# sangminwoo/SVOL

Measured on AMD Instinct MI355X. Metric: frames/sec (fwd+matcher+bwd), T=32·P=196·d=256, higher is better.
Workload: dtype bf16

## Files before the change

include/svol_hip.h:

```cpp
#ifndef SVOL_HIP_H
#define SVOL_HIP_H

#include <stdint.h>

#ifdef __cplusplus
extern "C" {
#endif

#define SVOL_F32 0
#define SVOL_BF16 1
#define SVOL_F16 2

#define SVOL_OK 0
#define SVOL_E_INVALID (-1)
#define SVOL_E_UNSUPPORTED (-2)
#define SVOL_E_LAUNCH (-3)

#define SVOL_ACT_NONE 0
#define SVOL_ACT_RELU 1
#define SVOL_ACT_GELU 2
#define SVOL_ACT_SIGMOID 3
#define SVOL_ACT_GELU_D 5
#define SVOL_ACT_RELU_RES 4

// ... 24 lines not shown
                   float weight_decay, int64_t step, float grad_scale, void* stream);
int svol_adam_flat_zero(float* p, float* g, float* m, float* v, int64_t n, float lr, float beta1, float beta2, float eps,
                        float weight_decay, int64_t step, float grad_scale, void* stream);
int svol_adam_flat_scaled(float* p, const float* g, float* m, float* v, int64_t n, float lr, float beta1, float beta2, float eps,
                          float weight_decay, float grad_mul, const float* scaler_state, void* stream);
int64_t svol_grad_sqnorm_ws_bytes(int64_t n);
int svol_grad_sqnorm(const float* g, int64_t n, float* ws, float* out, void* stream);
int svol_grad_clip_state(const float* sq, int32_t nb, float grad_mul, float max_norm, float loss_scale, int64_t steps_taken,
                         float* scaler_state, float* state_out, void* stream);
int svol_sgd_flat_grouped(float* p, float* g, float* buf, int64_t n, const int32_t* seg_end, const int32_t* seg_group, int32_t nseg,
                          const float* hyper, int32_t ngroups, const float* state, float grad_mul, int zero, void* stream);
int svol_adam_flat_grouped(float* p, float* g, float* m, float* v, int64_t n, const int32_t* seg_end, const int32_t* seg_group,
                           int32_t nseg, const float* hyper, int32_t ngroups, const float* state, const float* step_count,
                           float grad_mul, int zero, void* stream);
int svol_adamw_flat_grouped(float* p, float* g, float* m, float* v, int64_t n, const int32_t* seg_end, const int32_t* seg_group,
                            int32_t nseg, const float* hyper, int32_t ngroups, const float* state, const float* step_count,
                            float grad_mul, int zero, void* stream);
int svol_flat_step_advance(float* step_count, const float* state, void* stream);

int svol_gemm_nt(const void* A, int64_t lda, const void* A2, int64_t n_split, const void* B, int64_t ldb,
                 void* C, int64_t ldc, const float* bias, const float* colscale, int act, void* pre_act_out,
                 int64_t ldp, const void* residual, int64_t ldr, int out_f32, int64_t M, int64_t N, int64_t K,
                 int dtype, void* stream);
int svol_gemm_nt_split(const void* A, int64_t lda, const void* W_hilo, int64_t ldw, void* C, int64_t ldc, const float* bias,
                       int64_t M, int64_t N, int64_t K, void* stream);
int svol_gemm_nt_dgelu(const void* A, int64_t lda, const void* B, int64_t ldb, void* C, int64_t ldc,
                       const void* pre, int64_t ldp, float* colsum, int64_t M, int64_t N, int64_t K, int dtype,
                       void* stream);
int svol_gemm_nt_dact(const void* A, int64_t lda, const void* B, int64_t ldb, void* C, int64_t ldc,
                      const void* aux, int64_t ldaux, int act, float* colsum, int64_t M, int64_t N, int64_t K,
                      int dtype, void* stream);

int svol_gemm_tn(const void* A, int64_t lda, const void* B, int64_t ldb, float* C, int64_t ldc, float* colsum,
                 int64_t Mc, int64_t N, int64_t K, int dtype, void* stream);
#define SVOL_TN_GROUP_MAX 6
typedef struct svol_tn_problem {
    const void* A; int64_t lda;
    const void* B; int64_t ldb;
    float* C; int64_t ldc;
    float* colsum;
    int64_t Mc, N, K;
} svol_tn_problem;
int svol_gemm_tn_grouped(const svol_tn_problem* problems, int32_t n, int dtype, void* stream);
int svol_colsum(const void* X, int64_t ldx, float* out, int64_t M, int64_t N, int dtype, void* stream);
int svol_act_bwd(const void* dy, const void* aux, void* dpre, int act, int64_t n, int dtype, void* stream);

int svol_layernorm_fwd(const void* x, int x_f32, const float* gamma, const float* beta, float* y32, void* y,
                       void* ypos, const void* pos, int64_t pos_rows, float* mean, float* rstd, int64_t M, int64_t D,
                       float dropout_p, uint64_t seed, const int64_t* seed_offset_dev, int dtype, void* stream);
int svol_layernorm_bwd(const float* dy32, const void* dy, const void* dy2, const void* x, int x_f32,
                       const float* gamma, const float* mean, const float* rstd, float* dx32, void* dx,
                       float* dgamma, float* dbeta, float* dx_colsum, int64_t M, int64_t D, float dropout_p,
                       uint64_t seed, const int64_t* seed_offset_dev, int dtype, void* stream);

int svol_dropout(const void* x, void* y, int64_t n, int64_t row_len, float p, uint64_t seed, int dtype, void* stream);
int svol_dropout_add(const float* t32, const float* res32, float* out32, int64_t n, int64_t row_len, float p, uint64_t seed, void* stream);

int svol_posenc_sine(const float* mask, void* pos, int64_t B, int64_t L, int64_t D, int dtype, void* stream);

int64_t svol_attn_ws_bytes(int64_t B, int64_t H, int64_t Lq, int64_t Lk, int64_t dh);
int svol_attn_fwd(const void* q, int64_t ldq, const void* k, int64_t ldk, const void* v, int64_t ldv, void* o,
                  int64_t ldo, float* lse2, const float* kbias, int64_t B, int64_t H, int64_t Lq, int64_t Lk,
                  int64_t dh, float scale, float q_premul, void* ws, int64_t ws_bytes, int dtype, void* stream);
int svol_attn_bwd(const void* q, int64_t ldq, const void* k, int64_t ldk, const void* v, int64_t ldv, const void* o,
                  int64_t ldo, const void* d_o, int64_t lddo, const float* lse2, float* delta, const float* kbias,
                  void* dq, int64_t lddq, void* dk, int64_t lddk, void* dv, int64_t lddv, int64_t B, int64_t H,
                  int64_t Lq, int64_t Lk, int64_t dh, float scale, float q_premul, void* ws, int64_t ws_bytes,
                  int dtype, void* stream);

#define SVOL_ATTN_DQ_PREZEROED 1
int64_t svol_attn_bwd_sp_image_bytes(int64_t B, int64_t H, int64_t Lq, int64_t Lk, int64_t dh, int64_t ws_bytes, int dtype);
int svol_attn_bwd_zero_ws(void* ws, int64_t ws_bytes, int64_t B, int64_t H, int64_t Lq, int64_t Lk, int64_t dh, int dtype, void* stream);
int svol_attn_bwd_ex(const void* q, int64_t ldq, const void* k, int64_t ldk, const void* v, int64_t ldv, const void* o,
                     int64_t ldo, const void* d_o, int64_t lddo, const float* lse2, float* delta, const float* kbias,
                     void* dq, int64_t lddq, void* dk, int64_t lddk, void* dv, int64_t lddv, int64_t B, int64_t H,
                     int64_t Lq, int64_t Lk, int64_t dh, float scale, float q_premul, void* ws, int64_t ws_bytes,
                     int dtype, int flags, void* ev_prep, void* stream);

int svol_attn_fwd_dropout(const void* q, int64_t ldq, const void* k, int64_t ldk, const void* v, int64_t ldv, void* o,
                          int64_t ldo, float* lse2, const float* kbias, int64_t B, int64_t H, int64_t Lq, int64_t Lk,
                          int64_t dh, float scale, float q_premul, void* ws, int64_t ws_bytes, float dropout_p, uint64_t seed,
                          int dtype, void* stream);
int svol_attn_bwd_dropout(const void* q, int64_t ldq, const void* k, int64_t ldk, const void* v, int64_t ldv, const void* o,
                          int64_t ldo, const void* d_o, int64_t lddo, const float* lse2, float* delta, const float* kbias,
                          void* dq, int64_t lddq, void* dk, int64_t lddk, void* dv, int64_t lddv, int64_t B, int64_t H,
                          int64_t Lq, int64_t Lk, int64_t dh, float scale, float q_premul, void* ws, int64_t ws_bytes,
                          float dropout_p, uint64_t seed, int dtype, void* stream);

int svol_gate_fwd(const float* x32, const void* pos, const float* u, const float* gamma, const float* beta,
                  float* y32, void* y, void* ypos, float* a, float* mean, float* rstd, float* ws, int64_t B,
                  int64_t L, int64_t D, int64_t H, int dtype, void* stream);
int svol_gate_bwd(const float* dy32, const void* dy, const void* dy2, const float* x32, const void* pos,
                  const float* u, const float* gamma, const float* a, const float* mean, const float* rstd,
                  const float* ws, float* ws2, float* dx32, float* du, float* dgamma, float* dbeta, int64_t B,
                  int64_t L, int64_t D, int64_t H, int dtype, void* stream);

int svol_layernorm_gate_scores_fwd(const float* x32, const float* gamma, const float* beta, float* y32, void* y, void* ypos,
                                   const void* pos, float* mean, float* rstd, const float* u_next, float* scores_next,
                                   int64_t B, int64_t L, int64_t D, int64_t H, int dtype, void* stream);
int svol_gate_fwd_scored(const float* x32, const void* pos, const float* u, const float* gamma, const float* beta,
                         float* y32, void* y, void* ypos, float* a, float* mean, float* rstd, float* ws, int64_t B,
                         int64_t L, int64_t D, int64_t H, int dtype, void* stream);

int svol_gate_vectors_fwd(const float* skch, const float* W_in, const float* b_in, float* q_out, float* u_out, int64_t B, int64_t D,
                          int64_t H, void* stream);
int svol_gate_vectors_bwd(const float* du, const float* skch, const float* W_in, const float* q, float* dq_ws, float* dskch,
                          float* dW_in, float* db_in, int64_t B, int64_t D, int64_t H, void* stream);
#define SVOL_GATE_VEC_MAX_LAYERS 8
int svol_gate_vectors_fwd_multi(const float* skch, const float* const* W_in, const float* const* b_in, float* const* q_out,
                                float* const* u_out, int64_t n_layers, int64_t B, int64_t D, int64_t H, void* stream);
int svol_gate_vectors_bwd_multi(const float* const* du, const float* skch, const float* const* W_in, const float* const* q,
                                float* const* dq_ws, float* const* dskch, float* const* dW_in, float* const* db_in, int64_t n_layers,
                                int64_t B, int64_t D, int64_t H, void* stream);

int svol_match_cost(const float* logits, const float* boxes, const float* tgt_boxes, const int32_t* pred_off,
                    const int32_t* pred_cnt, const int32_t* tgt_off, const int32_t* tgt_cnt,
                    const int64_t* cost_off, float* cost, int32_t n_problems, float w_bbox, float w_giou,
                    float w_class, int32_t* box_status, void* stream);
int svol_lsap_batched(const float* cost, const int64_t* cost_off, const int32_t* pred_off, const int32_t* pred_cnt,
                      const int32_t* tgt_off, const int32_t* tgt_cnt, int32_t* match, int32_t* status,
                      int32_t n_problems, int32_t max_dim, void* stream);
int svol_heads_fwd(const float* hs, const float* Wc, const float* bc, const float* W0, const float* b0, const float* W1, const float* b1,
                   const float* W2, const float* b2, float* logits, float* h1, float* h2, float* boxes, int64_t R, int64_t D, void* stream);
int svol_heads_bwd(const float* dlogits, const float* dboxes, const float* hs, const float* h1, const float* h2, const float* boxes,
                   const float* Wc, const float* W0, const float* W1, const float* W2, float* dhs, float* gp0, float* gp1, float* dWc,
                   float* dbc, float* dW2, float* db2, int64_t R, int64_t D, void* stream);
int svol_set_loss_bwd(const float* g_label, const float* g_bbox, const float* g_giou, const float* dl, float* dlogits, float* dboxes,
                      int64_t n_layers, int64_t rows_per_layer, void* stream);
int svol_weighted_total(const float* x, const float* w, int64_t n, float* out, void* stream);
int svol_weighted_total_bwd(const float* w, const float* dout, int64_t n, float* dx, void* stream);
int svol_lsap_solve(const double* cost, int64_t nr, int64_t nc, int64_t* rows, int64_t* cols);
int svol_set_loss(const float* logits, const float* boxes, const float* tgt_boxes, const int32_t* match,
                  float* losses, float* g_label, float* g_bbox, float* g_giou, int32_t n_layers,
                  int32_t rows_per_layer, float eos_coef, const int32_t* rebase_vid_off, int32_t rows_per_video,
                  const int32_t* status, const int32_t* box_status, int32_t problems_per_layer, void* stream);

int svol_postprocess(const float* logits, const float* boxes, float* out, int64_t B, int64_t N, int64_t chunk, void* stream);
int svol_eval_max_iou(const double* pred_box, const int32_t* pred_off, const double* gt_box, const int32_t* gt_off,
                      const int32_t* gt_rec, double* out, int64_t n_gt, int32_t k, void* stream);
int svol_eval_ap(const double* pred_box, const double* pred_score, const int32_t* pred_frame, const int32_t* grp_pred_off,
                 const double* gt_box, const int32_t* gt_frame, const int32_t* grp_gt_off, const double* thresholds,
                 int32_t n_thresholds, int32_t* ws_order, unsigned char* ws_u8, double* ws_f64, double* ap, int64_t n_pred,
                 int64_t n_gt, int64_t n_groups, void* stream);

int svol_ingest_resize(const uint8_t* src, int64_t n, int64_t H, int64_t W, int64_t s_n, int64_t s_h, int64_t s_w,
                       const int32_t* xtab, int64_t kx, const int32_t* ytab, int64_t ky, const float* lut, const uint8_t* flip,
                       void* out, int64_t o_n, int64_t o_c, int64_t o_h, int64_t o_w, int64_t OH, int64_t OW, int out_dtype,
                       void* stream);
// ... 9 lines not shown
                   int64_t N, int64_t H, int64_t W, int64_t C, int64_t Cout, int64_t kh, int64_t kw, int64_t stride,
                   int64_t pad, int dtype, void* stream);
int svol_maxpool_nhwc(const void* x, void* y, int64_t N, int64_t H, int64_t W, int64_t C, int64_t k, int64_t stride,
                      int64_t pad, int dtype, void* stream);
int svol_avgpool_nhwc(const void* x, float* y, int64_t N, int64_t HW, int64_t C, int dtype, void* stream);
int svol_bn_colstats(const void* z, const float* shift, float shift_scale, float* sum, float* sumsq, int64_t M, int64_t C, int dtype,
                     void* stream);
int svol_bn_finalize(const float* sum, const float* sumsq_centered, const float* pivot, const float* gamma, const float* beta,
                     float* running_mean, float* running_var, float momentum, float eps, int64_t M, int64_t C, float* mean, float* rstd,
                     float* scale, float* shift, void* stream);
int svol_conv_weight_pack(const float* w, void* out, int64_t Cout, int64_t Cin, int64_t kh, int64_t kw, int64_t Kp, int flip, int dtype,
                          void* stream);
int svol_conv_weight_unpack_add(const float* dwp, float* grad, int64_t Cout, int64_t Cin, int64_t kh, int64_t kw, int64_t Kp, void* stream);
int svol_conv_wgrad_nhwc(const void* dz, const void* x, float* dwp, int64_t N, int64_t H, int64_t W, int64_t C, int64_t Cout, int64_t kh, int64_t kw,
                         int64_t stride, int64_t pad, int64_t Kp, int dtype, void* stream);
int svol_bn_apply(const void* z, const float* scale, const float* shift, const void* residual, int relu, void* y, int64_t M, int64_t C,
                  int dtype, void* stream);
int svol_bn_bwd_reduce(const void* dy, const void* y, const void* z, const float* mean, const float* rstd, float* sum_g, float* sum_gx,
                       int64_t M, int64_t C, int dtype, void* stream);
int svol_bn_bwd_apply(const void* dy, const void* y, const void* z, const float* mean, const float* rstd, const float* gamma,
                      const float* sum_g, const float* sum_gx, void* dz, void* dres, int64_t M, int64_t C, int dtype, void* stream);
int svol_col2im_nhwc(const void* dcols, int64_t ldcols, void* dx, int64_t N, int64_t H, int64_t W, int64_t C, int64_t kh, int64_t kw,
                     int64_t stride, int64_t pad, int dtype, void* stream);
int svol_maxpool_idx_nhwc(const void* x, void* y, uint8_t* idx, int64_t N, int64_t H, int64_t W, int64_t C, int64_t k, int64_t stride,
                          int64_t pad, int dtype, void* stream);
int svol_maxpool_bwd_nhwc(const void* dy, const uint8_t* idx, void* dx, int64_t N, int64_t H, int64_t W, int64_t C, int64_t k,
                          int64_t stride, int64_t pad, int dtype, void* stream);
int svol_attn_weights_mean(const void* q, int64_t ldq, const void* k, int64_t ldk, const float* lse2, const float* kbias,
                           float* att, int64_t B, int64_t H, int64_t Lq, int64_t Lk, int64_t dh, float scale,
                           float q_premul, int dtype, void* stream);
int svol_attn_small_fwd(const void* q, int64_t ldq, const void* k, int64_t ldk, const void* v, int64_t ldv, void* o, int64_t ldo,
                        int64_t n_seq, int64_t H, int64_t L, int64_t dh, float scale, int dtype, void* stream);
int svol_attn_small_fwd_lse(const void* q, int64_t ldq, const void* k, int64_t ldk, const void* v, int64_t ldv, void* o, int64_t ldo,
                            float* lse2, int64_t n_seq, int64_t H, int64_t L, int64_t dh, float scale, int dtype, void* stream);
int svol_attn_small_bwd(const void* q, int64_t ldq, const void* k, int64_t ldk, const void* v, int64_t ldv, const void* o, int64_t ldo,
                        const void* dout, int64_t lddo, const float* lse2, void* dq, int64_t lddq, void* dk, int64_t lddk, void* dv,
                        int64_t lddv, int64_t n_seq, int64_t H, int64_t L, int64_t dh, float scale, int dtype, void* stream);


#define SVOL_DIM_B 0
#define SVOL_DIM_L 1
#define SVOL_DIM_N 2
#define SVOL_DIM_D 3
#define SVOL_DIM_H 4
#define SVOL_DIM_F 5
#define SVOL_DIM_DTYPE 6
#define SVOL_DIM_QDTYPE 7
#define SVOL_DIM_ATTN_WS_BYTES 8
#define SVOL_DIM_COUNT 9

#define SVOL_BLK_VIDEO_HALF 0
#define SVOL_BLK_QUERY_SELF 1
#define SVOL_BLK_QUERY_CROSS 2
const char* svol_block_slot_names(int block);
int svol_block_trace_dump(char* buf, int64_t cap);
int svol_clock_probe(uint64_t* samples, int32_t* count, int32_t max_samples, const int32_t* stop, int64_t period_us,
                     int64_t max_ms, int32_t* wall_khz, void* stream);


#define SVOL_VH_SLOTS(X) \
    X(X32) X(POS) X(U) X(G1) X(BT1) X(G2) X(BT2) X(G3) X(BT3) X(B_IN) X(B_O) X(B_FC1) X(B_FC2) X(QSCALE) \
    X(W_IN) X(WV_HILO) X(W_O) X(W_FC1) X(W_FC2) X(W_IN_T) X(W_O_T) X(W_FC1_T) X(W_FC2_T) \
    X(Y1) X(Y1POS) X(A) X(MEAN1) X(RSTD1) X(GATE_WS) X(GATE_PRE) X(U_NEXT) X(GATE_WS_NEXT) \
    X(QKV) X(O) X(LSE) X(S2) X(Y2) X(MEAN2) X(RSTD2) X(PRE) X(HID) X(S3) \
    X(MEAN3) X(RSTD3) X(M32) X(M) X(MPOS) X(Y1_32) X(Y2_32) X(ATTN_WS) \
    X(DM32) X(DM) X(DMPOS) X(DS32_3) X(DS3) X(DPRE) X(DY2) X(DS32_2) X(G2D) X(DO) X(DQKV) X(DELTA) X(DXQP) X(DXQ) X(GATE_WS2) \
    X(DX32) X(DU) \
    X(DG1) X(DBT1) X(DG2) X(DBT2) X(DG3) X(DBT3) X(DW_IN) X(DB_IN) X(DW_O) X(DB_O) X(DW_FC1) X(DB_FC1) X(DW_FC2) X(DB_FC2) \
    X(EV_A0) X(EV_A1) X(EV_CLEAN_IN) X(EV_PREP) X(ATTN_WS_NEXT) X(ZERO_STREAM) X(EV_CLEAN_OUT)
#define SVOL_QS_SLOTS(X) \
    X(O32) X(O) X(OPOS) X(QPOS) X(B_IN) X(B_O) X(G4) X(BT4) X(QSCALE) X(W_IN) X(WV_HILO) X(W_O) X(W_IN_T) X(W_O_T) \
    X(QKV) X(OA) X(LSE) X(S4) X(MEAN4) X(RSTD4) X(Y32) X(Y) X(YPOS) X(ATTN_WS) \
    X(DY32) X(DY) X(DYPOS) X(G) X(DOA) X(DQKV) X(DELTA) X(DO32) X(DXQ) X(DXQP) X(DQPOS) \
    X(DW_IN) X(DB_IN) X(DW_O) X(DB_O) X(DG4) X(DBT4)
#define SVOL_QC_SLOTS(X) \
    X(O32) X(O) X(OPOS) X(MV) X(MPOS) X(KBIAS) X(QPOS) X(B_IN) X(B_O) X(G5) X(BT5) X(B_FC1) X(B_FC2) X(G6) X(BT6) X(QSCALE) \
    X(W_INQ) X(W_INQ_T) X(W_KV) X(W_KV_T) X(WV_HILO) X(W_O) X(W_O_T) X(W_FC1) X(W_FC1_T) X(W_FC2) X(W_FC2_T) \
    X(Q) X(QC) X(KV) X(OA) X(OAQ) X(LSE) X(S5) X(Y5_32) X(Y5) X(MEAN5) X(RSTD5) X(PRE) X(HID) X(S6) X(MEAN6) X(RSTD6) \
    X(Y32) X(Y) X(YPOS) X(ATTN_WS) \
    X(DY32) X(DY) X(DYPOS) X(DS32_6) X(DS6) X(DPRE) X(DY5) X(DS32_5) X(G5D) X(DOAQ) X(DOA) X(DQC) X(DQ) X(DKV) X(DELTA) \
    X(DO32) X(DXQP) X(DMPOS) X(DMV) X(DQPOS) \
    X(DW_IN) X(DB_IN) X(DW_O) X(DB_O) X(DG5) X(DBT5) X(DW_FC1) X(DB_FC1) X(DW_FC2) X(DB_FC2) X(DG6) X(DBT6)
#define SVOL_SLOT_ENUM_VH(n) SVOL_VH_##n,
#define SVOL_SLOT_ENUM_QS(n) SVOL_QS_##n,
#define SVOL_SLOT_ENUM_QC(n) SVOL_QC_##n,
enum { SVOL_VH_SLOTS(SVOL_SLOT_ENUM_VH) SVOL_VH_COUNT };
enum { SVOL_QS_SLOTS(SVOL_SLOT_ENUM_QS) SVOL_QS_COUNT };
enum { SVOL_QC_SLOTS(SVOL_SLOT_ENUM_QC) SVOL_QC_COUNT };

int svol_video_half_fwd(const int64_t* dims, void* const* slots, void* stream);
int svol_video_half_bwd(const int64_t* dims, void* const* slots, int phase, void* stream);
int svol_video_half_wgrad(const int64_t* dims, void* const* slots, void* stream);
int svol_video_half_wgrad_part(const int64_t* dims, void* const* slots, int part, void* stream);
int svol_query_self_fwd(const int64_t* dims, void* const* slots, void* stream);
int svol_query_self_bwd(const int64_t* dims, void* const* slots, void* stream);
int svol_query_self_wgrad(const int64_t* dims, void* const* slots, void* stream);
int svol_query_cross_fwd(const int64_t* dims, void* const* slots, void* stream);
int svol_query_cross_bwd(const int64_t* dims, void* const* slots, void* stream);
int svol_query_cross_wgrad(const int64_t* dims, void* const* slots, void* stream);

#ifdef __cplusplus
}
#endif
#endif
```

svol_amd/_lib.py:

```python
from __future__ import annotations

import ctypes
import os

_HERE = os.path.dirname(os.path.abspath(__file__))
LIB_PATH = os.path.join(_HERE, 'libsvol_hip.so')

_p = ctypes.c_void_p
_i64 = ctypes.c_int64
_i32 = ctypes.c_int32
_int = ctypes.c_int
_f32 = ctypes.c_float
_u64 = ctypes.c_uint64

SIGNATURES = {
    'svol_block_trace_dump': [ctypes.c_char_p, _i64],
    'svol_lsap_solve': [_p, _i64, _i64, _p, _p],
    'svol_heads_fwd': [_p] * 13 + [_i64, _i64, _p],
    'svol_heads_bwd': [_p] * 17 + [_i64, _i64, _p],
    'svol_set_loss_bwd': [_p] * 6 + [_i64, _i64, _p],
    'svol_weighted_total': [_p, _p, _i64, _p, _p],
    'svol_weighted_total_bwd': [_p, _p, _i64, _p, _p],
    'svol_cast': [_p, _int, _p, _int, _i64, _p],
    'svol_cast_transpose': [_p, _p, _p, _int, _i64, _i64, _p],
    'svol_cast_split': [_p, _i64, _p, _i64, _i64, _p],
    'svol_gemm_nt_split': [_p, _i64, _p, _i64, _p, _i64, _p, _i64, _i64, _i64, _p],
    'svol_gemm_nt': [_p, _i64, _p, _i64, _p, _i64, _p, _i64, _p, _p, _int, _p, _i64, _p, _i64, _int, _i64, _i64, _i64,
                     _int, _p],
    'svol_gemm_nt_dgelu': [_p, _i64, _p, _i64, _p, _i64, _p, _i64, _p, _i64, _i64, _i64, _int, _p],
    'svol_gemm_nt_dact': [_p, _i64, _p, _i64, _p, _i64, _p, _i64, _int, _p, _i64, _i64, _i64, _int, _p],
    'svol_gemm_tn': [_p, _i64, _p, _i64, _p, _i64, _p, _i64, _i64, _i64, _int, _p],
    'svol_gemm_tn_grouped': [_p, _i32, _int, _p],
    'svol_colsum': [_p, _i64, _p, _i64, _i64, _int, _p],
    'svol_act_bwd': [_p, _p, _p, _int, _i64, _int, _p],
    'svol_layernorm_fwd': [_p, _int, _p, _p, _p, _p, _p, _p, _i64, _p, _p, _i64, _i64, _f32, _u64, _p, _int, _p],
    'svol_layernorm_bwd': [_p, _p, _p, _p, _int, _p, _p, _p, _p, _p, _p, _p, _p, _i64, _i64, _f32, _u64, _p, _int, _p],
    'svol_cast_transpose_multi': [_p, _int, _i64, _int, _p],
    'svol_postprocess': [_p, _p, _p, _i64, _i64, _i64, _p],
    'svol_eval_max_iou': [_p, _p, _p, _p, _p, _p, _i64, _int, _p],
    'svol_eval_ap': [_p, _p, _p, _p, _p, _p, _p, _p, _int, _p, _p, _p, _p, _i64, _i64, _i64, _p],
    'svol_patchify': [_p, _p, _i64, _i64, _i64, _i64, _i64, _int, _p],
    'svol_vit_embed': [_p, _p, _p, _p, _p, _i64, _i64, _i64, _int, _p],
    'svol_ingest_resize': [_p, _i64, _i64, _i64, _i64, _i64, _i64, _p, _i64, _p, _i64, _p, _p, _p, _i64, _i64, _i64, _i64, _i64, _i64, _int, _p],
    'svol_adamw_flat': [_p, _p, _p, _p, _i64, _f32, _f32, _f32, _f32, _f32, _i64, _f32, _p],
    'svol_adamw_flat_zero': [_p, _p, _p, _p, _i64, _f32, _f32, _f32, _f32, _f32, _i64, _f32, _p],
    'svol_grad_finite': [_p, _i64, _p, _p],
    'svol_adamw_flat_scaled': [_p, _p, _p, _p, _i64, _f32, _f32, _f32, _f32, _f32, _f32, _p, _p],
    'svol_loss_scaler_update': [_p, _f32, _f32, _i64, _f32, _f32, _p],
    'svol_sgd_flat': [_p, _p, _p, _i64, _f32, _f32, _f32, _f32, _p],
    'svol_sgd_flat_zero': [_p, _p, _p, _i64, _f32, _f32, _f32, _f32, _p],
    'svol_sgd_flat_scaled': [_p, _p, _p, _i64, _f32, _f32, _f32, _f32, _p, _p],
    'svol_adam_flat': [_p, _p, _p, _p, _i64, _f32, _f32, _f32, _f32, _f32, _i64, _f32, _p],
    'svol_adam_flat_zero': [_p, _p, _p, _p, _i64, _f32, _f32, _f32, _f32, _f32, _i64, _f32, _p],
    'svol_adam_flat_scaled': [_p, _p, _p, _p, _i64, _f32, _f32, _f32, _f32, _f32, _f32, _p, _p],
    'svol_grad_sqnorm_ws_bytes': [_i64],
    'svol_grad_sqnorm': [_p, _i64, _p, _p, _p],
    'svol_grad_clip_state': [_p, _i32, _f32, _f32, _f32, _i64, _p, _p, _p],
    'svol_sgd_flat_grouped': [_p, _p, _p, _i64, _p, _p, _i32, _p, _i32, _p, _f32, _int, _p],
    'svol_adam_flat_grouped': [_p, _p, _p, _p, _i64, _p, _p, _i32, _p, _i32, _p, _p, _f32, _int, _p],
    'svol_adamw_flat_grouped': [_p, _p, _p, _p, _i64, _p, _p, _i32, _p, _i32, _p, _p, _f32, _int, _p],
    'svol_flat_step_advance': [_p, _p, _p],
    'svol_conv_nhwc': [_p, _p, _i64, _p, _p, _int, _p, _i64, _i64, _i64, _i64, _i64, _i64, _i64, _i64, _i64, _int, _p],
    'svol_im2col': [_p, _i64, _i64, _i64, _i64, _int, _p, _i64, _i64, _i64, _i64, _i64, _i64, _i64, _i64, _i64, _int, _p],
    'svol_maxpool_nhwc': [_p, _p, _i64, _i64, _i64, _i64, _i64, _i64, _i64, _int, _p],
    'svol_avgpool_nhwc': [_p, _p, _i64, _i64, _i64, _int, _p],
    'svol_bn_colstats': [_p, _p, _f32, _p, _p, _i64, _i64, _int, _p],
    'svol_bn_finalize': [_p, _p, _p, _p, _p, _p, _p, _f32, _f32, _i64, _i64, _p, _p, _p, _p, _p],
    'svol_conv_weight_pack': [_p, _p, _i64, _i64, _i64, _i64, _i64, _int, _int, _p],
    'svol_conv_weight_unpack_add': [_p, _p, _i64, _i64, _i64, _i64, _i64, _p],
    'svol_conv_wgrad_nhwc': [_p, _p, _p, _i64, _i64, _i64, _i64, _i64, _i64, _i64, _i64, _i64, _i64, _int, _p],
    'svol_bn_apply': [_p, _p, _p, _p, _int, _p, _i64, _i64, _int, _p],
    'svol_bn_bwd_reduce': [_p, _p, _p, _p, _p, _p, _p, _i64, _i64, _int, _p],
    'svol_bn_bwd_apply': [_p, _p, _p, _p, _p, _p, _p, _p, _p, _p, _i64, _i64, _int, _p],
    'svol_col2im_nhwc': [_p, _i64, _p, _i64, _i64, _i64, _i64, _i64, _i64, _i64, _i64, _int, _p],
    'svol_maxpool_idx_nhwc': [_p, _p, _p, _i64, _i64, _i64, _i64, _i64, _i64, _i64, _int, _p],
    'svol_maxpool_bwd_nhwc': [_p, _p, _p, _i64, _i64, _i64, _i64, _i64, _i64, _i64, _int, _p],
    'svol_attn_weights_mean': [_p, _i64, _p, _i64, _p, _p, _p, _i64, _i64, _i64, _i64, _i64, _f32, _f32, _int, _p],
    'svol_attn_small_fwd': [_p, _i64, _p, _i64, _p, _i64, _p, _i64, _i64, _i64, _i64, _i64, _f32, _int, _p],
    'svol_attn_small_fwd_lse': [_p, _i64, _p, _i64, _p, _i64, _p, _i64, _p, _i64, _i64, _i64, _i64, _f32, _int, _p],
    'svol_attn_small_bwd': [_p, _i64, _p, _i64, _p, _i64, _p, _i64, _p, _i64, _p, _p, _i64, _p, _i64, _p, _i64, _i64, _i64, _i64,
                            _i64, _f32, _int, _p],
    'svol_posenc_sine': [_p, _p, _i64, _i64, _i64, _int, _p],
    'svol_attn_ws_bytes': [_i64, _i64, _i64, _i64, _i64],
    'svol_attn_fwd': [_p, _i64, _p, _i64, _p, _i64, _p, _i64, _p, _p, _i64, _i64, _i64, _i64, _i64, _f32, _f32, _p, _i64,
                      _int, _p],
    'svol_attn_bwd': [_p, _i64, _p, _i64, _p, _i64, _p, _i64, _p, _i64, _p, _p, _p, _p, _i64, _p, _i64, _p, _i64,
                      _i64, _i64, _i64, _i64, _i64, _f32, _f32, _p, _i64, _int, _p],
    'svol_attn_bwd_ex': [_p, _i64, _p, _i64, _p, _i64, _p, _i64, _p, _i64, _p, _p, _p, _p, _i64, _p, _i64, _p, _i64,
                         _i64, _i64, _i64, _i64, _i64, _f32, _f32, _p, _i64, _int, _int, _p, _p],
    'svol_attn_bwd_sp_image_bytes': [_i64, _i64, _i64, _i64, _i64, _i64, _int],
    'svol_attn_bwd_zero_ws': [_p, _i64, _i64, _i64, _i64, _i64, _i64, _int, _p],
    'svol_attn_fwd_dropout': [_p, _i64, _p, _i64, _p, _i64, _p, _i64, _p, _p, _i64, _i64, _i64, _i64, _i64, _f32, _f32, _p, _i64,
                              _f32, _u64, _int, _p],
    'svol_attn_bwd_dropout': [_p, _i64, _p, _i64, _p, _i64, _p, _i64, _p, _i64, _p, _p, _p, _p, _i64, _p, _i64, _p, _i64,
                              _i64, _i64, _i64, _i64, _i64, _f32, _f32, _p, _i64, _f32, _u64, _int, _p],
    'svol_dropout': [_p, _p, _i64, _i64, _f32, _u64, _int, _p],
    'svol_dropout_add': [_p, _p, _p, _i64, _i64, _f32, _u64, _p],
    'svol_gate_fwd': [_p, _p, _p, _p, _p, _p, _p, _p, _p, _p, _p, _p, _i64, _i64, _i64, _i64, _int, _p],
    'svol_gate_bwd': [_p, _p, _p, _p, _p, _p, _p, _p, _p, _p, _p, _p, _p, _p, _p, _p, _i64, _i64, _i64, _i64, _int,
                      _p],
    'svol_clock_probe': [_p, _p, _int, _p, _i64, _i64, _p, _p],
    'svol_gate_fwd_scored': [_p, _p, _p, _p, _p, _p, _p, _p, _p, _p, _p, _p, _i64, _i64, _i64, _i64, _int, _p],
    'svol_layernorm_gate_scores_fwd': [_p, _p, _p, _p, _p, _p, _p, _p, _p, _p, _p, _i64, _i64, _i64, _i64, _int, _p],
    'svol_gate_vectors_fwd': [_p, _p, _p, _p, _p, _i64, _i64, _i64, _p],
    'svol_gate_vectors_bwd': [_p, _p, _p, _p, _p, _p, _p, _p, _i64, _i64, _i64, _p],
    'svol_gate_vectors_fwd_multi': [_p, _p, _p, _p, _p, _i64, _i64, _i64, _i64, _p],
    'svol_gate_vectors_bwd_multi': [_p, _p, _p, _p, _p, _p, _p, _p, _i64, _i64, _i64, _i64, _p],
    'svol_match_cost': [_p, _p, _p, _p, _p, _p, _p, _p, _p, _i32, _f32, _f32, _f32, _p, _p],
    'svol_lsap_batched': [_p, _p, _p, _p, _p, _p, _p, _p, _i32, _i32, _p],
    'svol_set_loss': [_p, _p, _p, _p, _p, _p, _p, _p, _i32, _i32, _f32, _p, _i32, _p, _p, _i32, _p],
    'svol_video_half_fwd': [_p, _p, _p],
    'svol_video_half_bwd': [_p, _p, _int, _p],
    'svol_video_half_wgrad': [_p, _p, _p],
    'svol_video_half_wgrad_part': [_p, _p, _int, _p],
    'svol_query_self_fwd': [_p, _p, _p],
    'svol_query_self_bwd': [_p, _p, _p],
    'svol_query_self_wgrad': [_p, _p, _p],
    'svol_query_cross_fwd': [_p, _p, _p],
    'svol_query_cross_bwd': [_p, _p, _p],
    'svol_query_cross_wgrad': [_p, _p, _p],
}



class TnProblem(ctypes.Structure):
    _fields_ = [('A', _p), ('lda', _i64), ('B', _p), ('ldb', _i64), ('C', _p), ('ldc', _i64), ('colsum', _p),
                ('Mc', _i64), ('N', _i64), ('K', _i64)]


_LIB = None


class SvolHipError(RuntimeError):
    pass


def lib():
    global _LIB
    if _LIB is None:
        if not os.path.exists(LIB_PATH):
            raise SvolHipError(
                f'{LIB_PATH} not found: the SVOL hot path has no CPU fallback. '
                'Build it with `python -m svol_amd.build` (hipcc, gfx950).')
        L = ctypes.CDLL(LIB_PATH)
        L.svol_abi_version.restype = _int
        L.svol_abi_version.argtypes = []
        L.svol_strerror.restype = ctypes.c_char_p
        L.svol_strerror.argtypes = [_int]
        for name, at in SIGNATURES.items():
            f = getattr(L, name)
            f.restype = _int
            f.argtypes = at
        L.svol_attn_ws_bytes.restype = _i64
        L.svol_attn_bwd_sp_image_bytes.restype = _i64
        L.svol_grad_sqnorm_ws_bytes.restype = _i64
        L.svol_block_slot_names.restype = ctypes.c_char_p
        L.svol_block_slot_names.argtypes = [_int]
        _LIB = L
    return _LIB


def check(rc: int, name: str):
    if rc != 0:
        msg = lib().svol_strerror(rc).decode()
        raise SvolHipError(f'{name} failed: {msg} (code {rc})')
```

svol_amd/blocks.py:

```python
from __future__ import annotations

import ctypes
import math
import os
import weakref

import torch

from . import _lib, ops

WGRAD_SPLIT = os.environ.get('SVOL_WGRAD_SPLIT') is not None
ENABLED = os.environ.get('SVOL_NO_BLOCKS') is None
GATE_SCORES_FUSE = os.environ.get('SVOL_GATE_SCORES_FUSE') is not None
VH, QS, QC = 0, 1, 2
_F32, _BF16 = 0, 1
_ESZ = {torch.float32: 4, torch.bfloat16: 2, torch.float16: 2}
_SLOTS = {}


def _slots(block):
    m = _SLOTS.get(block)
    if m is None:
        names = _lib.lib().svol_block_slot_names(block).decode().rstrip(',').split(',')
        m = _SLOTS[block] = {n: i for i, n in enumerate(names)}
    return m


class _Table:

    __slots__ = ('arr', 'idx', 'n')

    def __init__(self, block, template=None):
        self.idx = _slots(block)
        self.n = len(self.idx)
        self.arr = (ctypes.c_void_p * self.n)()
        if template is not None:
            ctypes.memmove(self.arr, template.arr, self.n * 8)

    def set(self, name, ptr):
        self.arr[self.idx[name]] = ptr

    def set_t(self, name, t):
        self.arr[self.idx[name]] = t.data_ptr() if t is not None else None


def _align(n, a=256):
    return (n + a - 1) // a * a


class _Layout:

    def __init__(self, items):
        self.off = {}
        n = 0
        for name, nbytes in items:
            self.off[name] = (n, nbytes)
            n += _align(nbytes)
        self.total = max(n, 256)

    def fill(self, tbl, base):
        for name, (o, _) in self.off.items():
            tbl.arr[tbl.idx[name]] = base + o

    def view(self, arena, name, dtype, shape):
        o, nb = self.off[name]
        return arena[o:o + nb].view(dtype).view(shape)


_LAYOUTS = {}


def _layout(key, make):
    lay = _LAYOUTS.get(key)
    if lay is None:
        lay = _LAYOUTS[key] = _Layout(make())
    return lay


_SCRATCH = {}


def _scratch(dev, nbytes):
    key = (dev, ops._stream())
    t = _SCRATCH.get(key)
    if t is None or t.numel() < nbytes:
        t = _SCRATCH[key] = torch.empty((_align(nbytes, 1 << 20),), dtype=torch.uint8, device=dev)
    return t


def _dims(B, L, N, D, H, F, dt, qdt, ws_bytes):
    return (ctypes.c_int64 * 9)(B, L, N, D, H, F, ops._DT[dt], ops._DT[qdt], ws_bytes)


def _attn_ws_bytes(B, H, Lq, Lk, dh, dt):
    n = _lib.lib().svol_attn_ws_bytes(B, H, Lq, Lk, dh) if dt != torch.float32 else 0
    return max(int(n), 0)


_VH_PARAMS = [
    ('DG1', lambda l: l.norm1.weight), ('DBT1', lambda l: l.norm1.bias),
    ('DW_IN', lambda l: l.content_self_attn.in_proj_weight), ('DB_IN', lambda l: l.content_self_attn.in_proj_bias),
    ('DW_O', lambda l: l.content_self_attn.out_proj.weight), ('DB_O', lambda l: l.content_self_attn.out_proj.bias),
    ('DG2', lambda l: l.norm2.weight), ('DBT2', lambda l: l.norm2.bias),
    ('DW_FC1', lambda l: l.mlp1.fc1.weight), ('DB_FC1', lambda l: l.mlp1.fc1.bias),
    ('DW_FC2', lambda l: l.mlp1.fc2.weight), ('DB_FC2', lambda l: l.mlp1.fc2.bias),
    ('DG3', lambda l: l.norm3.weight), ('DBT3', lambda l: l.norm3.bias)]
_QS_PARAMS = [
    ('DW_IN', lambda l: l.token_self_attn.in_proj_weight), ('DB_IN', lambda l: l.token_self_attn.in_proj_bias),
    ('DW_O', lambda l: l.token_self_attn.out_proj.weight), ('DB_O', lambda l: l.token_self_attn.out_proj.bias),
    ('DG4', lambda l: l.norm4.weight), ('DBT4', lambda l: l.norm4.bias)]
_QC_PARAMS = [
    ('DW_IN', lambda l: l.content_token_cross_attn.in_proj_weight), ('DB_IN', lambda l: l.content_token_cross_attn.in_proj_bias),
    ('DW_O', lambda l: l.content_token_cross_attn.out_proj.weight), ('DB_O', lambda l: l.content_token_cross_attn.out_proj.bias),
    ('DG5', lambda l: l.norm5.weight), ('DBT5', lambda l: l.norm5.bias),
    ('DW_FC1', lambda l: l.mlp2.fc1.weight), ('DB_FC1', lambda l: l.mlp2.fc1.bias),
    ('DW_FC2', lambda l: l.mlp2.fc2.weight), ('DB_FC2', lambda l: l.mlp2.fc2.bias),
    ('DG6', lambda l: l.norm6.weight), ('DBT6', lambda l: l.norm6.bias)]
_PARAMS = {VH: _VH_PARAMS, QS: _QS_PARAMS, QC: _QC_PARAMS}


class BlockPlan:

    def __init__(self, block, layer, dt, qdt):
        self.block, self.dt, self.qdt = block, dt, qdt
        self.layer = weakref.ref(layer)
        self.params = [g(layer) for _, g in _PARAMS[block]]
        self.grad_slots = [n for n, _ in _PARAMS[block]]
        self.tpl = _Table(block)
        self.keep = []
        D = layer.d_model
        self.split_v = ops.SPLIT_V and D % 32 == 0
        t = self.tpl
        W = ops.weights
        dev = self.params[0].device

        self.casts = []
        self.epoch = W.epoch

        def both(name, w, dtype, name_t=None):
            wc, wt = W.get(w, dtype)
            t.set_t(name, wc)
            t.set_t(name_t or (name + '_T'), wt)
            self.keep += [wc, wt]
            self.casts.append((w, dtype, wc, wt))

        def qscale(dtype, n):
            if dtype == torch.float32:
                return None
            q = ops._qscale(D, ops.LOG2E / math.sqrt(D // layer.nhead), dev)
            self.keep.append(q)
            return q

        if block == VH:
            m, mlp = layer.content_self_attn, layer.mlp1
            for n_, p_ in (('G1', layer.norm1.weight), ('BT1', layer.norm1.bias), ('G2', layer.norm2.weight), ('BT2', layer.norm2.bias),
                           ('G3', layer.norm3.weight), ('BT3', layer.norm3.bias), ('B_IN', m.in_proj_bias), ('B_O', m.out_proj.bias),
                           ('B_FC1', mlp.fc1.bias), ('B_FC2', mlp.fc2.bias)):
                t.set_t(n_, p_)
            both('W_IN', m.in_proj_weight, dt)
            both('W_O', m.out_proj.weight, dt)
            both('W_FC1', mlp.fc1.weight, dt)
            both('W_FC2', mlp.fc2.weight, dt)
            if dt == torch.bfloat16 and self.split_v:
                hl = W.get_split(m.in_proj_weight, 2 * D, D)
                t.set_t('WV_HILO', hl)
                self.keep.append(hl)
                self.casts.append((m.in_proj_weight, 2 * D, D, hl))
            t.set_t('QSCALE', qscale(dt, 2 * D))
        elif block == QS:
            m = layer.token_self_attn
            for n_, p_ in (('G4', layer.norm4.weight), ('BT4', layer.norm4.bias), ('B_IN', m.in_proj_bias), ('B_O', m.out_proj.bias)):
                t.set_t(n_, p_)
            both('W_IN', m.in_proj_weight, qdt)
            both('W_O', m.out_proj.weight, qdt)
            if qdt == torch.bfloat16 and self.split_v:
                hl = W.get_split(m.in_proj_weight, 2 * D, D)
                t.set_t('WV_HILO', hl)
                self.keep.append(hl)
                self.casts.append((m.in_proj_weight, 2 * D, D, hl))
            t.set_t('QSCALE', qscale(qdt, 2 * D))
        else:
            m, mlp = layer.content_token_cross_attn, layer.mlp2
            for n_, p_ in (('G5', layer.norm5.weight), ('BT5', layer.norm5.bias), ('G6', layer.norm6.weight), ('BT6', layer.norm6.bias),
                           ('B_IN', m.in_proj_bias), ('B_O', m.out_proj.bias), ('B_FC1', mlp.fc1.bias), ('B_FC2', mlp.fc2.bias)):
                t.set_t(n_, p_)
            both('W_INQ', m.in_proj_weight, qdt)
            both('W_KV', m.in_proj_weight, dt)
            both('W_O', m.out_proj.weight, qdt)
            both('W_FC1', mlp.fc1.weight, qdt)
            both('W_FC2', mlp.fc2.weight, qdt)
            if dt == torch.bfloat16 and self.split_v:
                hl = W.get_split(m.in_proj_weight, 2 * D, D)
                t.set_t('WV_HILO', hl)
                self.keep.append(hl)
                self.casts.append((m.in_proj_weight, 2 * D, D, hl))
            t.set_t('QSCALE', qscale(dt, D))
        self.sinks = [ops._claim(p, p.requires_grad) for p in self.params]
        self.nosink = [(i, p.numel()) for i, (p, s) in enumerate(zip(self.params, self.sinks)) if s is None]
        for name, s in zip(self.grad_slots, self.sinks):
            if s is not None:
                t.set_t(name, s.view)
        self.graph_params = self.params if (self.nosink or any(s.owner is None for s in self.sinks)) else []
        cnt = {}
        for s in self.sinks:
            if s is not None and s.owner is not None:
                cnt[(id(s.owner), s.bucket)] = (s.owner, s.bucket, cnt.get((id(s.owner), s.bucket), (None, None, 0))[2] + 1)
        self.notify = list(cnt.values())
        self.key = self._key()

    def _key(self):
        k = []
        for p in self.params:
            g = p.grad
            s = getattr(p, '_svol_sink', None)
            k.append((p.data_ptr(), g.data_ptr() if (g is not None and s is not None) else 0, p.requires_grad))
        return (ops.SPLIT_V, tuple(k))

    def valid(self):
        return self.layer() is not None and self._key() == self.key

    def fresh_copies(self):
        W = ops.weights
        for c in self.casts:
            if len(c) == 4 and isinstance(c[1], torch.dtype):
                wc, wt = W.get(c[0], c[1])
                if wc is not c[2] or wt is not c[3]:
                    return False
            else:
                if W.get_split(c[0], c[1], c[2]) is not c[3]:
                    return False
        return True

    def grad_buffers(self, tbl, dev):
        if not self.nosink:
            return None
        offs, n = [], 0
        for _, numel in self.nosink:
            offs.append(n)
            n += (numel + 3) // 4 * 4
        flat = torch.zeros((n,), dtype=torch.float32, device=dev)
        out = {}
        base = flat.data_ptr()
        for (i, numel), o in zip(self.nosink, offs):
            tbl.set(self.grad_slots[i], base + o * 4)
            out[i] = flat[o:o + numel].view_as(self.params[i])
        return out

    def inputs(self, *tensors):
        if self.graph_params or not any(t_.requires_grad for t_ in tensors):
            return self.params
        return ()

    def done(self, in_graph):
        if not in_graph:
            for owner, bi, n in self.notify:
                owner.params_done(bi, n)

    def grads_out(self, bufs, needs, in_graph):
        res = []
        if not in_graph:
            return res
# ... 56 lines not shown
    e0, e1 = torch.cuda.Event(enable_timing=True), torch.cuda.Event(enable_timing=True)
    e0.record()
    e1.record()
    tm.records.setdefault((name, meta), []).append((e0, e1))
    return e0, e1


DQ_PREZERO = os.environ.get('SVOL_DQ_PREZERO') is not None and os.environ.get('SVOL_NO_DQ_PREZERO') is None
_DQ_PREZERO = {}


class _DqPrezero:
    __slots__ = ('bufs', 'side', 'ev_prep', 'clean_ev', 'clean', 'nxt')

    def __init__(self, dev, wsb):
        self.bufs = [torch.empty((_align(wsb, 1 << 20),), dtype=torch.uint8, device=dev) for _ in range(2)]
        self.side = torch.cuda.Stream(device=dev)
        self.ev_prep = torch.cuda.Event()
        self.clean_ev = [torch.cuda.Event(), torch.cuda.Event()]
        for e_ in [self.ev_prep] + self.clean_ev:
            e_.record()
        self.clean = [False, False]
        self.nxt = 0

    def bind(self, tbl):
        i = self.nxt
        tbl.set('ATTN_WS', self.bufs[i].data_ptr())
        tbl.set('EV_CLEAN_IN', self.clean_ev[i].cuda_event if self.clean[i] else None)
        tbl.set('EV_PREP', self.ev_prep.cuda_event)
        tbl.set('ATTN_WS_NEXT', self.bufs[1 - i].data_ptr())
        tbl.set('ZERO_STREAM', self.side.cuda_stream)
        tbl.set('EV_CLEAN_OUT', self.clean_ev[1 - i].cuda_event)
        self.clean[i] = False

    def advance(self, tbl):
        i = self.nxt
        self.clean[1 - i] = True
        self.nxt = 1 - i
        for n_ in ('EV_CLEAN_IN', 'EV_PREP', 'ATTN_WS_NEXT', 'ZERO_STREAM', 'EV_CLEAN_OUT'):
            tbl.set(n_, None)


def _dq_prezero(dev, B, H, L, dh, dt, wsb):
    if not DQ_PREZERO or dt == torch.float32 or torch.cuda.is_current_stream_capturing():
        return None
    key = (dev, ops._stream(), B, H, L, dh, dt, wsb)
    st = _DQ_PREZERO.get(key)
    if st is None:
        img = _lib.lib().svol_attn_bwd_sp_image_bytes(B, H, L, L, dh, wsb, ops._DT[dt])
        st = _DQ_PREZERO[key] = _DqPrezero(dev, wsb) if img > 0 else False
    return st or None


def _vh_fwd_layout(B, L, D, H, F, e):
    M = B * L
    return [('Y1', M * D * e), ('Y1POS', M * D * e), ('A', M * 4), ('MEAN1', M * 4), ('RSTD1', M * 4), ('GATE_WS', B * H * (L + 2) * 4),
            ('QKV', M * 3 * D * e), ('O', M * D * e), ('LSE', B * H * L * 4), ('S2', M * D * 4), ('Y2', M * D * e), ('MEAN2', M * 4),
            ('RSTD2', M * 4), ('PRE', M * F * e), ('HID', M * F * e), ('S3', M * D * 4), ('MEAN3', M * 4), ('RSTD3', M * 4),
            ('M32', M * D * 4), ('M', M * D * e), ('MPOS', M * D * e)]


def _vh_bwd_layout(B, L, D, H, F, e):
    M = B * L
    return [('DS32_3', M * D * 4), ('DS3', M * D * e), ('DPRE', M * F * e), ('DY2', M * D * e), ('DS32_2', M * D * 4), ('G2D', M * D * e),
            ('DO', M * D * e), ('DQKV', M * 3 * D * e), ('DELTA', 3 * B * H * L * 4), ('DXQP', M * D * e), ('DXQ', M * D * e),
            ('GATE_WS2', (B * L + B * H) * 4), ('DX32', M * D * 4)]


class VideoHalfFn(torch.autograd.Function):

    @staticmethod
    def forward(ctx, pl, x32, pos, u, u_next, sc_in, *params):
        ctx.set_materialize_grads(False)
        B, L, D = x32.shape
        layer = pl.layer()
        H, F = layer.nhead, layer.mlp1.fc1.weight.shape[0]
        dt = pl.dt
        e = _ESZ[dt]
        dev = x32.device
        M = B * L
        x2 = x32.reshape(M, D)
        x2 = x2 if x2.is_contiguous() else x2.contiguous()
        pos2 = pos.reshape(M, D)
        pos2 = pos2 if pos2.is_contiguous() else pos2.contiguous()
        u = u.contiguous()
        assert x2.dtype == torch.float32 and pos2.dtype == dt and u.dtype == torch.float32
        wsb = _attn_ws_bytes(B, H, L, L, D // H, dt)
        key = (VH, B, L, D, H, F, dt)
        lay = _layout(('f',) + key, lambda: _vh_fwd_layout(B, L, D, H, F, e))
        slay = _layout(('s',) + key, lambda: [('Y1_32', M * D * 4), ('Y2_32', M * D * 4), ('ATTN_WS', max(wsb, 16))])
        arena = torch.empty((lay.total,), dtype=torch.uint8, device=dev)
        scr = _scratch(dev, slay.total)
        tbl = _Table(VH, pl.tpl)
        lay.fill(tbl, arena.data_ptr())
        slay.fill(tbl, scr.data_ptr())
        tbl.set('X32', x2.data_ptr())
        tbl.set('POS', pos2.data_ptr())
        tbl.set('U', u.data_ptr())
        if sc_in is not None:
            assert sc_in.dtype == torch.float32 and sc_in.numel() == B * H * (L + 2) and sc_in.is_contiguous()
            tbl.set('GATE_WS', sc_in.data_ptr())
            tbl.set('GATE_PRE', sc_in.data_ptr())
        if u_next is not None:
            u_next = u_next.contiguous()
            assert u_next.dtype == torch.float32 and u_next.shape == u.shape and L % 4 == 0
            sc_next = torch.empty((B * H * (L + 2),), dtype=torch.float32, device=dev)
            tbl.set('U_NEXT', u_next.data_ptr())
            tbl.set('GATE_WS_NEXT', sc_next.data_ptr())
        else:
            sc_next = torch.empty((0,), dtype=torch.float32, device=dev)
        dims = _dims(B, L, 0, D, H, F, dt, dt, wsb)
        big = B * H * L * L >= ops._WGRAD_FLUSH_MIN_SCORES
        if big:
            ops._BIG_ATTN['left'] += 1
        ev = _maybe_events('attn_fwd', (B, H, L, L, D // H))
        if ev:
            tbl.set('EV_A0', ev[0].cuda_event)
            tbl.set('EV_A1', ev[1].cuda_event)
        _lib.check(_lib.lib().svol_video_half_fwd(dims, tbl.arr, ops._stream()), 'svol_video_half_fwd')
        tbl.set('EV_A0', None)
        tbl.set('EV_A1', None)
        tbl.set('U_NEXT', None)
        tbl.set('GATE_WS_NEXT', None)
        ctx.pl, ctx.tbl, ctx.dims, ctx.arena, ctx.shape, ctx.big = pl, tbl, dims, arena, (B, L, D, H, F), big
        ctx.n_par = len(params)
        ctx.sc_in = sc_in
        ctx.save_for_backward(x2, pos2, u)
        ctx.mark_non_differentiable(sc_next)
        return (lay.view(arena, 'M32', torch.float32, (B, L, D)), lay.view(arena, 'M', dt, (B, L, D)),
                lay.view(arena, 'MPOS', dt, (B, L, D)), sc_next)

    @staticmethod
    def backward(ctx, dm32, dm, dmpos, _dsc=None):
        pl, tbl, dims = ctx.pl, ctx.tbl, ctx.dims
        B, L, D, H, F = ctx.shape
        x2, pos2, u = ctx.saved_tensors
        n_par = ctx.n_par
        if dm32 is None and dm is None and dmpos is None:
            pl.done(n_par > 0)
            return (None,) * (6 + n_par)
        dt = pl.dt
        e = _ESZ[dt]
        dev = x2.device
        M = B * L
        cont = lambda t_: None if t_ is None else (t_.reshape(M, D) if t_.is_contiguous() else t_.reshape(M, D).contiguous())
        dm32, dm, dmpos = cont(dm32), cont(dm), cont(dmpos)
        lay = _layout(('b', VH, B, L, D, H, F, dt), lambda: _vh_bwd_layout(B, L, D, H, F, e))
        tmp = torch.empty((lay.total,), dtype=torch.uint8, device=dev)
        lay.fill(tbl, tmp.data_ptr())
        du = torch.zeros((B, H, D), dtype=torch.float32, device=dev)
        tbl.set('DU', du.data_ptr())
        tbl.set_t('DM32', dm32)
        tbl.set_t('DM', dm)
        tbl.set_t('DMPOS', dmpos)
        slay = _layout(('s', VH, B, L, D, H, F, dt), None)
        scr = _scratch(dev, slay.total)
        slay.fill(tbl, scr.data_ptr())
        bufs = pl.grad_buffers(tbl, dev)
        L_ = _lib.lib()
        s = ops._stream()
        _lib.check(L_.svol_video_half_bwd(dims, tbl.arr, 1, s), 'svol_video_half_bwd')
        keep = [t_ for t_ in (ctx.arena, tmp, dm32, dm, dmpos) if t_ is not None]
        split = bufs is None and ctx.big and WGRAD_SPLIT
        if ctx.big:
            ops._BIG_ATTN['left'] -= 1
            if split:
                _issue_wgrad('svol_video_half_wgrad_part', dims, tbl, keep, dev, part=1)
            ops.flush_wgrad(gate=True)
        ev = _maybe_events('attn_bwd', (B, H, L, L, D // H))
        if ev:
            tbl.set('EV_A0', ev[0].cuda_event)
            tbl.set('EV_A1', ev[1].cuda_event)
        pz = _dq_prezero(dev, B, H, L, D // H, dt, dims[8]) if ctx.big else None
        if pz is not None:
            pz.bind(tbl)
        _lib.check(L_.svol_video_half_bwd(dims, tbl.arr, 2, s), 'svol_video_half_bwd')
        if pz is not None:
            pz.advance(tbl)
        tbl.set('EV_A0', None)
        tbl.set('EV_A1', None)
        if split:
            _issue_wgrad('svol_video_half_wgrad_part', dims, tbl, keep, dev, part=2)
        elif bufs is None:
            _issue_wgrad('svol_video_half_wgrad', dims, tbl, keep, dev)
        else:
            _lib.check(L_.svol_video_half_wgrad(dims, tbl.arr, s), 'svol_video_half_wgrad')
        pl.done(n_par > 0)
        dx32 = lay.view(tmp, 'DX32', torch.float32, (B, L, D))
        needs = ctx.needs_input_grad
        return (None, dx32, None, du if needs[3] else None, None, None) + tuple(pl.grads_out(bufs, needs[6:], n_par > 0))


def gate_scores_fusable(L, D, H):
    return GATE_SCORES_FUSE and L % 4 == 0 and D % 4 == 0 and D <= 256 and H <= 8


def video_half(layer, x32, pos, u, dt, u_next=None, sc_in=None):
    pl = plan(layer, VH, dt, dt)
    if u_next is not None and not gate_scores_fusable(x32.shape[1], x32.shape[2], layer.nhead):
        u_next = None
    m32, m, mpos, sc = VideoHalfFn.apply(pl, x32, pos, u, u_next, sc_in, *pl.inputs(x32, u))
    return m32, m, mpos, (sc if u_next is not None else None)


def _qpos_target(pl, qpos, tbl, dev, N, D):
    if not qpos.requires_grad:
        tbl.set('DQPOS', None)
        return None, False
    s = ops._claim(qpos, True) if (qpos.is_leaf and qpos.dtype == torch.float32) else None
    if s is not None:
        tbl.set_t('DQPOS', s.view)
        return None, True
    g = torch.zeros((N, D), dtype=torch.float32, device=dev)
    tbl.set('DQPOS', g.data_ptr())
    return g, False


class QuerySelfFn(torch.autograd.Function):

    @staticmethod
    def forward(ctx, pl, o32, o, opos, qpos, *params):
        ctx.set_materialize_grads(False)
        B, N, D = o.shape
        layer = pl.layer()
        H = layer.nhead
        qdt = pl.qdt
        e = _ESZ[qdt]
        dev = o.device
        R = B * N
        c = lambda t_: t_ if t_.is_contiguous() else t_.contiguous()
        o32_, o_, opos_, qpos_ = c(o32), c(o), c(opos), c(qpos)
        assert o32_.dtype == torch.float32 and o_.dtype == qdt and opos_.dtype == qdt and qpos_.dtype == qdt
        wsb = _attn_ws_bytes(B, H, N, N, D // H, qdt)
        key = (QS, B, N, D, H, qdt)
        lay = _layout(('f',) + key, lambda: [('QKV', R * 3 * D * e), ('OA', R * D * e), ('LSE', B * H * N * 4), ('S4', R * D * 4),
                                              ('MEAN4', R * 4), ('RSTD4', R * 4), ('Y32', R * D * 4), ('Y', R * D * e), ('YPOS', R * D * e)])
        slay = _layout(('s',) + key, lambda: [('ATTN_WS', max(wsb, 16))])
        arena = torch.empty((lay.total,), dtype=torch.uint8, device=dev)
        scr = _scratch(dev, slay.total)
        tbl = _Table(QS, pl.tpl)
        lay.fill(tbl, arena.data_ptr())
        slay.fill(tbl, scr.data_ptr())
        tbl.set('O32', o32_.data_ptr())
        tbl.set('O', o_.data_ptr())
        tbl.set('OPOS', opos_.data_ptr())
        tbl.set('QPOS', qpos_.data_ptr())
        dims = _dims(B, 0, N, D, H, 0, qdt, qdt, wsb)
        _lib.check(_lib.lib().svol_query_self_fwd(dims, tbl.arr, ops._stream()), 'svol_query_self_fwd')
        ctx.pl, ctx.tbl, ctx.dims, ctx.arena, ctx.shape = pl, tbl, dims, arena, (B, N, D, H)
        ctx.n_par = len(params)
        ctx.save_for_backward(o32_, o_, opos_, qpos)
        return (lay.view(arena, 'Y32', torch.float32, (B, N, D)), lay.view(arena, 'Y', qdt, (B, N, D)),
                lay.view(arena, 'YPOS', qdt, (B, N, D)))

    @staticmethod
# ... 6 lines not shown
            pl.done(n_par > 0)
            return (None,) * (5 + n_par)
        qdt = pl.qdt
        e = _ESZ[qdt]
        dev = o_.device
        R = B * N
        cont = lambda t_: None if t_ is None else (t_ if t_.is_contiguous() else t_.contiguous())
        dy32, dy, dypos = cont(dy32), cont(dy), cont(dypos)
        lay = _layout(('b', QS, B, N, D, H, qdt), lambda: [('G', R * D * e), ('DOA', R * D * e), ('DQKV', R * 3 * D * e),
                                                            ('DELTA', 3 * B * H * N * 4), ('DO32', R * D * 4), ('DXQ', R * D * e),
                                                            ('DXQP', R * D * e)])
        tmp = torch.empty((lay.total,), dtype=torch.uint8, device=dev)
        lay.fill(tbl, tmp.data_ptr())
        tbl.set_t('DY32', dy32)
        tbl.set_t('DY', dy)
        tbl.set_t('DYPOS', dypos)
        slay = _layout(('s', QS, B, N, D, H, qdt), None)
        scr = _scratch(dev, slay.total)
        slay.fill(tbl, scr.data_ptr())
        needs = ctx.needs_input_grad
        gq, _ = _qpos_target(pl, qpos, tbl, dev, N, D) if needs[4] else (None, False)
        if not needs[4]:
            tbl.set('DQPOS', None)
        bufs = pl.grad_buffers(tbl, dev)
        L_ = _lib.lib()
        s = ops._stream()
        _lib.check(L_.svol_query_self_bwd(dims, tbl.arr, s), 'svol_query_self_bwd')
        keep = (ctx.arena, tmp, o_, opos_)
        if bufs is None:
            _issue_wgrad('svol_query_self_wgrad', dims, tbl, list(keep), dev)
        else:
            _lib.check(L_.svol_query_self_wgrad(dims, tbl.arr, s), 'svol_query_self_wgrad')
        pl.done(n_par > 0)
        if gq is not None and qdt != torch.float32:
            gq = ops.cast(gq, qdt)
        v = lambda n_, dt_: lay.view(tmp, n_, dt_, (B, N, D))
        return (None, v('DO32', torch.float32), v('DXQ', qdt), v('DXQP', qdt), gq) + tuple(pl.grads_out(bufs, needs[5:], n_par > 0))


def query_self(layer, out, qpos, dt, qdt):
    pl = plan(layer, QS, dt, qdt)
    o32, o, opos = out
    return QuerySelfFn.apply(pl, o32, o, opos, qpos, *pl.inputs(o32, o, opos))


def _qc_fwd_layout(B, N, L, D, H, F, e, qe):
    R, M = B * N, B * L
    return [('Q', R * D * qe), ('QC', R * D * e), ('KV', M * 2 * D * e), ('OA', R * D * e), ('OAQ', R * D * qe), ('LSE', B * H * N * 4),
            ('S5', R * D * 4), ('Y5_32', R * D * 4), ('Y5', R * D * qe), ('MEAN5', R * 4), ('RSTD5', R * 4), ('PRE', R * F * qe),
            ('HID', R * F * qe), ('S6', R * D * 4), ('MEAN6', R * 4), ('RSTD6', R * 4), ('Y32', R * D * 4), ('Y', R * D * qe),
            ('YPOS', R * D * qe)]


def _qc_bwd_layout(B, N, L, D, H, F, e, qe):
    R, M = B * N, B * L
    return [('DS32_6', R * D * 4), ('DS6', R * D * qe), ('DPRE', R * F * qe), ('DY5', R * D * qe), ('G5D', R * D * qe), ('DOAQ', R * D * qe),
            ('DOA', R * D * e), ('DQC', R * D * e), ('DQ', R * D * qe), ('DKV', M * 2 * D * e), ('DELTA', 3 * B * H * N * 4),
            ('DO32', R * D * 4), ('DXQP', R * D * qe), ('DMPOS', M * D * e), ('DMV', M * D * e)]


class QueryCrossFn(torch.autograd.Function):

    @staticmethod
    def forward(ctx, pl, o32, o, opos, mv, mpos, kbias, qpos, *params):
        ctx.set_materialize_grads(False)
        B, N, D = o.shape
        L = mv.shape[1]
        layer = pl.layer()
        H, F = layer.nhead, layer.mlp2.fc1.weight.shape[0]
        dt, qdt = pl.dt, pl.qdt
        e, qe = _ESZ[dt], _ESZ[qdt]
        dev = o.device
        c = lambda t_: t_ if t_.is_contiguous() else t_.contiguous()
        o32_, o_, opos_, mv_, mpos_, kb_, qpos_ = c(o32), c(o), c(opos), c(mv), c(mpos), c(kbias), c(qpos)
        assert o32_.dtype == torch.float32 and o_.dtype == qdt and opos_.dtype == qdt and qpos_.dtype == qdt
        assert mv_.dtype == dt and mpos_.dtype == dt and kb_.dtype == torch.float32
        wsb = _attn_ws_bytes(B, H, N, L, D // H, dt)
        key = (QC, B, N, L, D, H, F, dt, qdt)
        lay = _layout(('f',) + key, lambda: _qc_fwd_layout(B, N, L, D, H, F, e, qe))
        slay = _layout(('s',) + key, lambda: [('ATTN_WS', max(wsb, 16))])
        arena = torch.empty((lay.total,), dtype=torch.uint8, device=dev)
        scr = _scratch(dev, slay.total)
        tbl = _Table(QC, pl.tpl)
        lay.fill(tbl, arena.data_ptr())
        slay.fill(tbl, scr.data_ptr())
        for n_, t_ in (('O32', o32_), ('O', o_), ('OPOS', opos_), ('MV', mv_), ('MPOS', mpos_), ('KBIAS', kb_), ('QPOS', qpos_)):
            tbl.set(n_, t_.data_ptr())
        dims = _dims(B, L, N, D, H, F, dt, qdt, wsb)
        _lib.check(_lib.lib().svol_query_cross_fwd(dims, tbl.arr, ops._stream()), 'svol_query_cross_fwd')
        ctx.pl, ctx.tbl, ctx.dims, ctx.arena, ctx.shape = pl, tbl, dims, arena, (B, N, L, D, H, F)
        ctx.n_par = len(params)
        ctx.save_for_backward(o32_, o_, opos_, mv_, mpos_, kb_, qpos)
        return (lay.view(arena, 'Y32', torch.float32, (B, N, D)), lay.view(arena, 'Y', qdt, (B, N, D)),
                lay.view(arena, 'YPOS', qdt, (B, N, D)))

    @staticmethod
    def backward(ctx, dy32, dy, dypos):
        pl, tbl, dims = ctx.pl, ctx.tbl, ctx.dims
        B, N, L, D, H, F = ctx.shape
        o32_, o_, opos_, mv_, mpos_, kb_, qpos = ctx.saved_tensors
        n_par = ctx.n_par
        if dy32 is None and dy is None and dypos is None:
            pl.done(n_par > 0)
            return (None,) * (8 + n_par)
        dt, qdt = pl.dt, pl.qdt
        e, qe = _ESZ[dt], _ESZ[qdt]
        dev = o_.device
        cont = lambda t_: None if t_ is None else (t_ if t_.is_contiguous() else t_.contiguous())
        dy32, dy, dypos = cont(dy32), cont(dy), cont(dypos)
        lay = _layout(('b', QC, B, N, L, D, H, F, dt, qdt), lambda: _qc_bwd_layout(B, N, L, D, H, F, e, qe))
        tmp = torch.empty((lay.total,), dtype=torch.uint8, device=dev)
        lay.fill(tbl, tmp.data_ptr())
        tbl.set_t('DY32', dy32)
        tbl.set_t('DY', dy)
        tbl.set_t('DYPOS', dypos)
        slay = _layout(('s', QC, B, N, L, D, H, F, dt, qdt), None)
        scr = _scratch(dev, slay.total)
        slay.fill(tbl, scr.data_ptr())
        needs = ctx.needs_input_grad
        gq = None
        if needs[7]:
            gq, _ = _qpos_target(pl, qpos, tbl, dev, N, D)
        else:
            tbl.set('DQPOS', None)
        bufs = pl.grad_buffers(tbl, dev)
        L_ = _lib.lib()
        s = ops._stream()
        _lib.check(L_.svol_query_cross_bwd(dims, tbl.arr, s), 'svol_query_cross_bwd')
        keep = (ctx.arena, tmp, opos_, mv_, mpos_)
        if bufs is None:
            _issue_wgrad('svol_query_cross_wgrad', dims, tbl, list(keep), dev)
        else:
            _lib.check(L_.svol_query_cross_wgrad(dims, tbl.arr, s), 'svol_query_cross_wgrad')
        pl.done(n_par > 0)
        if gq is not None and qdt != torch.float32:
            gq = ops.cast(gq, qdt)
        vq = lambda n_, dt_: lay.view(tmp, n_, dt_, (B, N, D))
        vm = lambda n_: lay.view(tmp, n_, dt, (B, L, D))
        return (None, vq('DO32', torch.float32), None, vq('DXQP', qdt), vm('DMV'), vm('DMPOS'), None, gq) + \
            tuple(pl.grads_out(bufs, needs[8:], n_par > 0))


def query_cross(layer, out, mv, mpos, kbias, qpos, dt, qdt):
    pl = plan(layer, QC, dt, qdt)
    o32, o, opos = out
    return QueryCrossFn.apply(pl, o32, o, opos, mv, mpos, kbias, qpos, *pl.inputs(o32, opos, mv, mpos))


def trace_dump() -> str:
    buf = ctypes.create_string_buffer(1 << 20)
    _lib.check(_lib.lib().svol_block_trace_dump(buf, len(buf)), 'svol_block_trace_dump')
    return buf.value.decode()
```

svol_amd/csrc/blocks.hip:

```cpp
#include <math.h>
#include <stdio.h>
#include <stdlib.h>
#include <string.h>

#include <map>
#include <mutex>
#include <string>
#include <vector>

#include "common.h"

namespace {

const bool kTrace = getenv("SVOL_BLOCK_TRACE") != nullptr;
struct TraceRec { const char* prog; const char* site; hipEvent_t e0, e1; };
std::mutex g_trace_mu;
std::vector<TraceRec> g_trace_log;
struct Trace {
    const char* prog;
    hipStream_t s;
    hipEvent_t last = nullptr;
    Trace* prev;
    static thread_local Trace* cur;
    Trace(const char* prog_, void* s_) : prog(prog_), s(static_cast<hipStream_t>(s_)), prev(cur) {
// ... 4 lines not shown
    void mark(const char* site) {
        if (!kTrace || !last) return;
        hipEvent_t e;
        if (hipEventCreate(&e) != hipSuccess) return;
        (void)hipEventRecord(e, s);
        std::lock_guard<std::mutex> lk(g_trace_mu);
        g_trace_log.push_back({prog, site, last, e});
        last = e;
    }
};
thread_local Trace* Trace::cur = nullptr;

struct Dims {
    int64_t B, L, N, D, H, F, ws_bytes;
    int dt, qdt;
    explicit Dims(const int64_t* d)
        : B(d[SVOL_DIM_B]), L(d[SVOL_DIM_L]), N(d[SVOL_DIM_N]), D(d[SVOL_DIM_D]), H(d[SVOL_DIM_H]), F(d[SVOL_DIM_F]),
          ws_bytes(d[SVOL_DIM_ATTN_WS_BYTES]), dt((int)d[SVOL_DIM_DTYPE]), qdt((int)d[SVOL_DIM_QDTYPE]) {}
    bool ok() const {
        return B > 0 && D > 0 && H > 0 && D % H == 0 && (dt == SVOL_F32 || svol_is16(dt)) && (qdt == SVOL_F32 || svol_is16(qdt));
    }
};

inline int esz(int dtype) { return svol_is16(dtype) ? 2 : 4; }
inline void* at(void* p, int64_t elems, int dtype) { return p ? static_cast<char*>(p) + elems * esz(dtype) : nullptr; }
inline const void* at(const void* p, int64_t elems, int dtype) { return p ? static_cast<const char*>(p) + elems * esz(dtype) : nullptr; }
inline float* f32(void* p) { return static_cast<float*>(p); }

inline float attn_scale(int64_t dh) { return (float)(1.0 / sqrt((double)dh)); }
inline float attn_premul(int64_t dh, int dtype) { return svol_is16(dtype) ? (float)(1.4426950408889634 / sqrt((double)dh)) : 0.f; }

inline int nt(const void* A, int64_t lda, const void* W, int64_t ldw, void* C, int64_t ldc, const void* bias, const void* colscale,
              int64_t M, int64_t N, int64_t K, int dtype, void* s) {
    return svol_gemm_nt(A, lda, nullptr, 0, W, ldw, C, ldc, static_cast<const float*>(bias), static_cast<const float*>(colscale),
                        SVOL_ACT_NONE, nullptr, 0, nullptr, 0, 0, M, N, K, dtype, s);
}
inline int nt_res(const void* A, int64_t lda, const void* W, int64_t ldw, void* C32, const void* bias, const void* res32, int64_t M,
                  int64_t N, int64_t K, int dtype, void* s) {
    return svol_gemm_nt(A, lda, nullptr, 0, W, ldw, C32, N, static_cast<const float*>(bias), nullptr, SVOL_ACT_NONE, nullptr, 0, res32, N,
                        1, M, N, K, dtype, s);
}

#define RUN(expr)                                 \
    do {                                          \
        const int rc_ = (expr);                   \
        if (rc_) return rc_;                      \
        if (kTrace && Trace::cur) Trace::cur->mark(#expr); \
    } while (0)

#define SLOT_NAME(n) #n ","
const char* const kVhNames = SVOL_VH_SLOTS(SLOT_NAME);
const char* const kQsNames = SVOL_QS_SLOTS(SLOT_NAME);
const char* const kQcNames = SVOL_QC_SLOTS(SLOT_NAME);

inline void record(void* ev, void* stream) {
    if (ev) (void)hipEventRecord(static_cast<hipEvent_t>(ev), static_cast<hipStream_t>(stream));
}

}


extern "C" {

int svol_block_trace_dump(char* buf, int64_t cap) {
    if (!buf || cap <= 0) return SVOL_E_INVALID;
    buf[0] = 0;
    if (!kTrace) return SVOL_OK;
    if (hipDeviceSynchronize() != hipSuccess) return SVOL_E_LAUNCH;
    std::lock_guard<std::mutex> lk(g_trace_mu);
    static const bool timeline = getenv("SVOL_BLOCK_TRACE") && atoi(getenv("SVOL_BLOCK_TRACE")) == 2;
    if (timeline && !g_trace_log.empty()) {
        std::string out;
        char line[256];
        const hipEvent_t ref = g_trace_log.front().e0;
        for (const TraceRec& r : g_trace_log) {
            float t0 = 0.f, t1 = 0.f;
            if (hipEventElapsedTime(&t0, ref, r.e0) != hipSuccess || hipEventElapsedTime(&t1, ref, r.e1) != hipSuccess) continue;
            std::string site(r.site);
            const size_t c = site.find(',');
            if (c != std::string::npos) site.resize(c);
            snprintf(line, sizeof line, "%9.3f %9.3f  %-20s %s\n", t0, t1, r.prog, site.c_str());
            out += line;
        }
        std::map<hipEvent_t, int> seen_;
        for (const TraceRec& r : g_trace_log) { seen_[r.e0] = 1; seen_[r.e1] = 1; }
        for (auto& kv : seen_) (void)hipEventDestroy(kv.first);
        g_trace_log.clear();
        strncpy(buf, out.c_str(), (size_t)cap - 1);
        buf[cap - 1] = 0;
        return SVOL_OK;
    }
    std::map<std::string, std::pair<double, int>> acc;
    std::vector<std::string> order;
    std::map<hipEvent_t, int> seen;
    for (const TraceRec& r : g_trace_log) {
        float ms = 0.f;
        if (hipEventElapsedTime(&ms, r.e0, r.e1) != hipSuccess) continue;
        std::string site(r.site);
        const size_t c = site.find(',');
        if (c != std::string::npos) site.resize(c);
        const std::string key = std::string(r.prog) + " | " + site;
        if (!acc.count(key)) order.push_back(key);
        acc[key].first += ms;
        acc[key].second += 1;
    }
    for (const TraceRec& r : g_trace_log) { seen[r.e0] = 1; seen[r.e1] = 1; }
    for (auto& kv : seen) (void)hipEventDestroy(kv.first);
    g_trace_log.clear();
    std::string out;
    char line[256];
    for (const std::string& k : order) {
        snprintf(line, sizeof line, "%-110s calls %6d  avg_us %9.1f  total_ms %9.3f\n", k.c_str(), acc[k].second,
                 acc[k].first / acc[k].second * 1e3, acc[k].first);
        out += line;
    }
    strncpy(buf, out.c_str(), (size_t)cap - 1);
    buf[cap - 1] = 0;
    return SVOL_OK;
}

const char* svol_block_slot_names(int block) {
    switch (block) {
        case SVOL_BLK_VIDEO_HALF: return kVhNames;
        case SVOL_BLK_QUERY_SELF: return kQsNames;
        case SVOL_BLK_QUERY_CROSS: return kQcNames;
        default: return "";
    }
}

int svol_video_half_fwd(const int64_t* dims, void* const* p, void* s) {
    if (!dims || !p) return SVOL_E_INVALID;
    Trace tr_("video_half_fwd", s);
    const Dims d(dims);
    if (!d.ok() || d.L <= 0 || d.F <= 0) return SVOL_E_INVALID;
    const int64_t M = d.B * d.L, D = d.D, F = d.F, dh = D / d.H;
    const int dt = d.dt, xf = dt != SVOL_F32;
#define P(n) p[SVOL_VH_##n]
    if (P(GATE_PRE))
        RUN(svol_gate_fwd_scored(f32(P(X32)), P(POS), f32(P(U)), f32(P(G1)), f32(P(BT1)), f32(P(Y1_32)), P(Y1), P(Y1POS), f32(P(A)),
                                 f32(P(MEAN1)), f32(P(RSTD1)), f32(P(GATE_WS)), d.B, d.L, D, d.H, dt, s));
    else
        RUN(svol_gate_fwd(f32(P(X32)), P(POS), f32(P(U)), f32(P(G1)), f32(P(BT1)), f32(P(Y1_32)), P(Y1), P(Y1POS), f32(P(A)), f32(P(MEAN1)),
                          f32(P(RSTD1)), f32(P(GATE_WS)), d.B, d.L, D, d.H, dt, s));
    RUN(nt(P(Y1POS), D, P(W_IN), D, P(QKV), 3 * D, P(B_IN), P(QSCALE), M, 2 * D, D, dt, s));
    if (P(WV_HILO))
        RUN(svol_gemm_nt_split(P(Y1), D, P(WV_HILO), 2 * D, at(P(QKV), 2 * D, dt), 3 * D, f32(P(B_IN)) + 2 * D, M, D, D, s));
    else
        RUN(nt(P(Y1), D, at(P(W_IN), 2 * D * D, dt), D, at(P(QKV), 2 * D, dt), 3 * D, f32(P(B_IN)) + 2 * D, nullptr, M, D, D, dt, s));
    record(P(EV_A0), s);
    RUN(svol_attn_fwd(P(QKV), 3 * D, at(P(QKV), D, dt), 3 * D, at(P(QKV), 2 * D, dt), 3 * D, P(O), D, f32(P(LSE)), nullptr, d.B, d.H, d.L,
                      d.L, dh, attn_scale(dh), attn_premul(dh, dt), P(ATTN_WS), d.ws_bytes, dt, s));
    record(P(EV_A1), s);
    RUN(nt_res(P(O), D, P(W_O), D, P(S2), P(B_O), P(Y1_32), M, D, D, dt, s));
    RUN(svol_layernorm_fwd(P(S2), xf, f32(P(G2)), f32(P(BT2)), f32(P(Y2_32)), P(Y2), nullptr, nullptr, 0, f32(P(MEAN2)), f32(P(RSTD2)), M,
                           D, 0.f, 0, nullptr, dt, s));
    RUN(svol_gemm_nt(P(Y2), D, nullptr, 0, P(W_FC1), D, P(HID), F, f32(P(B_FC1)), nullptr, SVOL_ACT_GELU_D, P(PRE), F, nullptr, 0, 0, M, F, D, dt, s));
    RUN(nt_res(P(HID), F, P(W_FC2), F, P(S3), P(B_FC2), P(Y2_32), M, D, F, dt, s));
    if (P(U_NEXT) && P(GATE_WS_NEXT))
        RUN(svol_layernorm_gate_scores_fwd(f32(P(S3)), f32(P(G3)), f32(P(BT3)), f32(P(M32)), P(M), P(MPOS), P(POS), f32(P(MEAN3)),
                                           f32(P(RSTD3)), f32(P(U_NEXT)), f32(P(GATE_WS_NEXT)), d.B, d.L, D, d.H, dt, s));
    else
        RUN(svol_layernorm_fwd(P(S3), xf, f32(P(G3)), f32(P(BT3)), f32(P(M32)), P(M), P(MPOS), P(POS), M, f32(P(MEAN3)), f32(P(RSTD3)), M, D,
                               0.f, 0, nullptr, dt, s));
    return SVOL_OK;
}

int svol_video_half_bwd(const int64_t* dims, void* const* p, int phase, void* s) {
    if (!dims || !p || phase < 0 || phase > 2) return SVOL_E_INVALID;
    Trace tr_(phase == 2 ? "video_half_bwd.2" : "video_half_bwd.1", s);
    const Dims d(dims);
    if (!d.ok() || d.L <= 0 || d.F <= 0) return SVOL_E_INVALID;
    const int64_t M = d.B * d.L, D = d.D, F = d.F, dh = D / d.H;
    const int dt = d.dt, xf = dt != SVOL_F32;
    if (phase != 2) {
        RUN(svol_layernorm_bwd(f32(P(DM32)), P(DM), P(DMPOS), P(S3), xf, f32(P(G3)), f32(P(MEAN3)), f32(P(RSTD3)), f32(P(DS32_3)), P(DS3),
                               f32(P(DG3)), f32(P(DBT3)), f32(P(DB_FC2)), M, D, 0.f, 0, nullptr, dt, s));
        RUN(svol_gemm_nt_dact(P(DS3), D, P(W_FC2_T), D, P(DPRE), F, P(PRE), F, SVOL_ACT_GELU_D, f32(P(DB_FC1)), M, F, D, dt, s));
        RUN(nt(P(DPRE), F, P(W_FC1_T), F, P(DY2), D, nullptr, nullptr, M, D, F, dt, s));
        RUN(svol_layernorm_bwd(f32(P(DS32_3)), P(DY2), nullptr, P(S2), xf, f32(P(G2)), f32(P(MEAN2)), f32(P(RSTD2)), f32(P(DS32_2)), P(G2D),
                               f32(P(DG2)), f32(P(DBT2)), f32(P(DB_O)), M, D, 0.f, 0, nullptr, dt, s));
        RUN(nt(P(G2D), D, P(W_O_T), D, P(DO), D, nullptr, nullptr, M, D, D, dt, s));
    }
    if (phase != 1) {
        int aflags = 0;
        if (P(EV_CLEAN_IN)) {
            if (hipStreamWaitEvent(static_cast<hipStream_t>(s), static_cast<hipEvent_t>(P(EV_CLEAN_IN)), 0) != hipSuccess) return SVOL_E_LAUNCH;
            aflags = SVOL_ATTN_DQ_PREZEROED;
        }
        record(P(EV_A0), s);
        RUN(svol_attn_bwd_ex(P(QKV), 3 * D, at(P(QKV), D, dt), 3 * D, at(P(QKV), 2 * D, dt), 3 * D, P(O), D, P(DO), D, f32(P(LSE)),
                             f32(P(DELTA)), nullptr, P(DQKV), 3 * D, at(P(DQKV), D, dt), 3 * D, at(P(DQKV), 2 * D, dt), 3 * D, d.B, d.H, d.L,
                             d.L, dh, attn_scale(dh), attn_premul(dh, dt), P(ATTN_WS), d.ws_bytes, dt, aflags, P(EV_PREP), s));
        record(P(EV_A1), s);
        if (P(ATTN_WS_NEXT) && P(ZERO_STREAM) && P(EV_PREP) && P(EV_CLEAN_OUT)) {
            hipStream_t zs = static_cast<hipStream_t>(P(ZERO_STREAM));
            if (hipStreamWaitEvent(zs, static_cast<hipEvent_t>(P(EV_PREP)), 0) != hipSuccess) return SVOL_E_LAUNCH;
            const int zrc = svol_attn_bwd_zero_ws(P(ATTN_WS_NEXT), d.ws_bytes, d.B, d.H, d.L, d.L, dh, dt, zs);
            if (zrc) return zrc;
            record(P(EV_CLEAN_OUT), zs);
        }
        RUN(nt(P(DQKV), 3 * D, P(W_IN_T), 3 * D, P(DXQP), D, nullptr, nullptr, M, D, 2 * D, dt, s));
        RUN(nt(at(P(DQKV), 2 * D, dt), 3 * D, at(P(W_IN_T), 2 * D, dt), 3 * D, P(DXQ), D, nullptr, nullptr, M, D, D, dt, s));
        RUN(svol_gate_bwd(f32(P(DS32_2)), P(DXQ), P(DXQP), f32(P(X32)), P(POS), f32(P(U)), f32(P(G1)), f32(P(A)), f32(P(MEAN1)),
                          f32(P(RSTD1)), f32(P(GATE_WS)), f32(P(GATE_WS2)), f32(P(DX32)), f32(P(DU)), f32(P(DG1)), f32(P(DBT1)), d.B, d.L,
                          D, d.H, dt, s));
    }
    return SVOL_OK;
}

int svol_video_half_wgrad_part(const int64_t* dims, void* const* p, int part, void* s) {
    if (!dims || !p || part < 0 || part > 2) return SVOL_E_INVALID;
    Trace tr_(part == 1 ? "video_half_wgrad.1" : part == 2 ? "video_half_wgrad.2" : "video_half_wgrad", s);
    const Dims d(dims);
    if (!d.ok()) return SVOL_E_INVALID;
    const int64_t M = d.B * d.L, D = d.D, F = d.F;
    const int dt = d.dt;
    const svol_tn_problem pr[5] = {
        {P(DS3), D, P(HID), F, f32(P(DW_FC2)), F, nullptr, M, D, F},
        {P(DPRE), F, P(Y2), D, f32(P(DW_FC1)), D, nullptr, M, F, D},
        {P(G2D), D, P(O), D, f32(P(DW_O)), D, nullptr, M, D, D},
        {P(DQKV), 3 * D, P(Y1POS), D, f32(P(DW_IN)), D, f32(P(DB_IN)), M, 2 * D, D},
        {at(P(DQKV), 2 * D, dt), 3 * D, P(Y1), D, f32(P(DW_IN)) + 2 * D * D, D, f32(P(DB_IN)) + 2 * D, M, D, D}};
    if (part == 1) RUN(svol_gemm_tn_grouped(pr, 3, dt, s));
    else if (part == 2) RUN(svol_gemm_tn_grouped(pr + 3, 2, dt, s));
    else RUN(svol_gemm_tn_grouped(pr, 5, dt, s));
    return SVOL_OK;
}

int svol_video_half_wgrad(const int64_t* dims, void* const* p, void* s) { return svol_video_half_wgrad_part(dims, p, 0, s); }
#undef P

int svol_query_self_fwd(const int64_t* dims, void* const* p, void* s) {
    if (!dims || !p) return SVOL_E_INVALID;
    Trace tr_("query_self_fwd", s);
    const Dims d(dims);
    if (!d.ok() || d.N <= 0) return SVOL_E_INVALID;
    const int64_t R = d.B * d.N, D = d.D, dh = D / d.H;
    const int qdt = d.qdt, xf = qdt != SVOL_F32;
#define P(n) p[SVOL_QS_##n]
    RUN(nt(P(OPOS), D, P(W_IN), D, P(QKV), 3 * D, P(B_IN), P(QSCALE), R, 2 * D, D, qdt, s));
    if (P(WV_HILO))
        RUN(svol_gemm_nt_split(P(O), D, P(WV_HILO), 2 * D, at(P(QKV), 2 * D, qdt), 3 * D, f32(P(B_IN)) + 2 * D, R, D, D, s));
    else
        RUN(nt(P(O), D, at(P(W_IN), 2 * D * D, qdt), D, at(P(QKV), 2 * D, qdt), 3 * D, f32(P(B_IN)) + 2 * D, nullptr, R, D, D, qdt, s));
    RUN(svol_attn_fwd(P(QKV), 3 * D, at(P(QKV), D, qdt), 3 * D, at(P(QKV), 2 * D, qdt), 3 * D, P(OA), D, f32(P(LSE)), nullptr, d.B, d.H,
                      d.N, d.N, dh, attn_scale(dh), attn_premul(dh, qdt), P(ATTN_WS), d.ws_bytes, qdt, s));
    RUN(nt_res(P(OA), D, P(W_O), D, P(S4), P(B_O), P(O32), R, D, D, qdt, s));
    RUN(svol_layernorm_fwd(P(S4), xf, f32(P(G4)), f32(P(BT4)), f32(P(Y32)), P(Y), P(YPOS), P(QPOS), d.N, f32(P(MEAN4)), f32(P(RSTD4)), R, D,
                           0.f, 0, nullptr, qdt, s));
    return SVOL_OK;
}

int svol_query_self_bwd(const int64_t* dims, void* const* p, void* s) {
    if (!dims || !p) return SVOL_E_INVALID;
    Trace tr_("query_self_bwd", s);
    const Dims d(dims);
    if (!d.ok() || d.N <= 0) return SVOL_E_INVALID;
    const int64_t R = d.B * d.N, D = d.D, dh = D / d.H;
// ... 39 lines not shown
    if (mixed) {
        RUN(nt(P(OPOS), D, P(W_INQ), D, P(Q), D, P(B_IN), P(QSCALE), R, D, D, qdt, s));
        RUN(svol_cast(P(Q), qdt, P(QC), dt, R * D, s));
    } else {
        RUN(nt(P(OPOS), D, P(W_KV), D, P(QC), D, P(B_IN), P(QSCALE), R, D, D, dt, s));
    }
    RUN(nt(P(MPOS), D, at(P(W_KV), D * D, dt), D, P(KV), 2 * D, f32(P(B_IN)) + D, nullptr, M, D, D, dt, s));
    if (P(WV_HILO))
        RUN(svol_gemm_nt_split(P(MV), D, P(WV_HILO), 2 * D, at(P(KV), D, dt), 2 * D, f32(P(B_IN)) + 2 * D, M, D, D, s));
    else
        RUN(nt(P(MV), D, at(P(W_KV), 2 * D * D, dt), D, at(P(KV), D, dt), 2 * D, f32(P(B_IN)) + 2 * D, nullptr, M, D, D, dt, s));
    RUN(svol_attn_fwd(P(QC), D, P(KV), 2 * D, at(P(KV), D, dt), 2 * D, P(OA), D, f32(P(LSE)), f32(P(KBIAS)), d.B, d.H, d.N, d.L, dh,
                      attn_scale(dh), attn_premul(dh, dt), P(ATTN_WS), d.ws_bytes, dt, s));
    const void* oq = P(OA);
    if (mixed) {
        RUN(svol_cast(P(OA), dt, P(OAQ), qdt, R * D, s));
        oq = P(OAQ);
    }
    RUN(nt_res(oq, D, P(W_O), D, P(S5), P(B_O), P(O32), R, D, D, qdt, s));
    RUN(svol_layernorm_fwd(P(S5), xf, f32(P(G5)), f32(P(BT5)), f32(P(Y5_32)), P(Y5), nullptr, nullptr, 0, f32(P(MEAN5)), f32(P(RSTD5)), R,
                           D, 0.f, 0, nullptr, qdt, s));
    RUN(svol_gemm_nt(P(Y5), D, nullptr, 0, P(W_FC1), D, P(HID), F, f32(P(B_FC1)), nullptr, SVOL_ACT_GELU, P(PRE), F, nullptr, 0, 0, R, F, D,
                     qdt, s));
    RUN(nt_res(P(HID), F, P(W_FC2), F, P(S6), P(B_FC2), P(Y5_32), R, D, F, qdt, s));
    RUN(svol_layernorm_fwd(P(S6), xf, f32(P(G6)), f32(P(BT6)), f32(P(Y32)), P(Y), P(YPOS), P(QPOS), d.N, f32(P(MEAN6)), f32(P(RSTD6)), R, D,
                           0.f, 0, nullptr, qdt, s));
    return SVOL_OK;
}

int svol_query_cross_bwd(const int64_t* dims, void* const* p, void* s) {
    if (!dims || !p) return SVOL_E_INVALID;
    Trace tr_("query_cross_bwd", s);
    const Dims d(dims);
    if (!d.ok() || d.N <= 0 || d.L <= 0 || d.F <= 0) return SVOL_E_INVALID;
    const int64_t R = d.B * d.N, M = d.B * d.L, D = d.D, F = d.F, dh = D / d.H;
    const int dt = d.dt, qdt = d.qdt, xf = qdt != SVOL_F32;
    const bool mixed = qdt != dt;
    RUN(svol_layernorm_bwd(f32(P(DY32)), P(DY), P(DYPOS), P(S6), xf, f32(P(G6)), f32(P(MEAN6)), f32(P(RSTD6)), f32(P(DS32_6)), P(DS6),
                           f32(P(DG6)), f32(P(DBT6)), f32(P(DB_FC2)), R, D, 0.f, 0, nullptr, qdt, s));
    if (P(DQPOS) && P(DYPOS)) RUN(svol_colsum(P(DYPOS), d.N * D, f32(P(DQPOS)), d.B, d.N * D, qdt, s));
    RUN(svol_gemm_nt_dact(P(DS6), D, P(W_FC2_T), D, P(DPRE), F, P(PRE), F, SVOL_ACT_GELU, f32(P(DB_FC1)), R, F, D, qdt, s));
    RUN(nt(P(DPRE), F, P(W_FC1_T), F, P(DY5), D, nullptr, nullptr, R, D, F, qdt, s));
    RUN(svol_layernorm_bwd(f32(P(DS32_6)), P(DY5), nullptr, P(S5), xf, f32(P(G5)), f32(P(MEAN5)), f32(P(RSTD5)), f32(P(DO32)), P(G5D),
                           f32(P(DG5)), f32(P(DBT5)), f32(P(DB_O)), R, D, 0.f, 0, nullptr, qdt, s));
    RUN(nt(P(G5D), D, P(W_O_T), D, P(DOAQ), D, nullptr, nullptr, R, D, D, qdt, s));
    const void* d_o = P(DOAQ);
    if (mixed) {
        RUN(svol_cast(P(DOAQ), qdt, P(DOA), dt, R * D, s));
        d_o = P(DOA);
    }
    RUN(svol_attn_bwd(P(QC), D, P(KV), 2 * D, at(P(KV), D, dt), 2 * D, P(OA), D, d_o, D, f32(P(LSE)), f32(P(DELTA)), f32(P(KBIAS)), P(DQC), D,
                      P(DKV), 2 * D, at(P(DKV), D, dt), 2 * D, d.B, d.H, d.N, d.L, dh, attn_scale(dh), attn_premul(dh, dt), P(ATTN_WS),
                      d.ws_bytes, dt, s));
    RUN(nt(P(DKV), 2 * D, at(P(W_KV_T), D, dt), 3 * D, P(DMPOS), D, nullptr, nullptr, M, D, D, dt, s));
    RUN(nt(at(P(DKV), D, dt), 2 * D, at(P(W_KV_T), 2 * D, dt), 3 * D, P(DMV), D, nullptr, nullptr, M, D, D, dt, s));
    const void* dq = P(DQC);
    if (mixed) {
        RUN(svol_cast(P(DQC), dt, P(DQ), qdt, R * D, s));
        dq = P(DQ);
    }
    RUN(nt(dq, D, mixed ? P(W_INQ_T) : P(W_KV_T), 3 * D, P(DXQP), D, nullptr, nullptr, R, D, D, qdt, s));
    return SVOL_OK;
}

int svol_query_cross_wgrad(const int64_t* dims, void* const* p, void* s) {
    if (!dims || !p) return SVOL_E_INVALID;
    Trace tr_("query_cross_wgrad", s);
    const Dims d(dims);
    if (!d.ok()) return SVOL_E_INVALID;
    const int64_t R = d.B * d.N, M = d.B * d.L, D = d.D, F = d.F;
    const int dt = d.dt, qdt = d.qdt;
    const bool mixed = qdt != dt;
    const svol_tn_problem pv[2] = {
        {P(DKV), 2 * D, P(MPOS), D, f32(P(DW_IN)) + D * D, D, f32(P(DB_IN)) + D, M, D, D},
        {at(P(DKV), D, dt), 2 * D, P(MV), D, f32(P(DW_IN)) + 2 * D * D, D, f32(P(DB_IN)) + 2 * D, M, D, D}};
    RUN(svol_gemm_tn_grouped(pv, 2, dt, s));
    const svol_tn_problem pq[4] = {
        {P(DS6), D, P(HID), F, f32(P(DW_FC2)), F, nullptr, R, D, F},
        {P(DPRE), F, P(Y5), D, f32(P(DW_FC1)), D, nullptr, R, F, D},
        {P(G5D), D, mixed ? P(OAQ) : P(OA), D, f32(P(DW_O)), D, nullptr, R, D, D},
        {mixed ? P(DQ) : P(DQC), D, P(OPOS), D, f32(P(DW_IN)), D, f32(P(DB_IN)), R, D, D}};
    RUN(svol_gemm_tn_grouped(pq, 4, qdt, s));
    return SVOL_OK;
#undef P
}

}
```

svol_amd/csrc/gate.hip:

```cpp
#include <cstdlib>

#include "common.h"

namespace {

constexpr int GP = 4;
constexpr int GH = 8;

__device__ __forceinline__ void store_head_sums(const float (&part)[GH], float* __restrict__ scores, int b, int l, int L, int H, int lane) {
    const bool b0 = lane & 1, b1 = lane & 2;
    float h4[4], h2[2];
#pragma unroll
    for (int i = 0; i < 4; ++i) {
        const float send = b0 ? part[i] : part[4 + i], keep = b0 ? part[4 + i] : part[i];
        h4[i] = keep + dpp_f32<0xB1>(send);
    }
#pragma unroll
    for (int i = 0; i < 2; ++i) {
        const float send = b1 ? h4[i] : h4[2 + i], keep = b1 ? h4[2 + i] : h4[i];
        h2[i] = keep + dpp_f32<0x4E>(send);
    }
#pragma unroll
    for (int i = 0; i < 2; ++i) {
        float v = h2[i];
// ... 352 lines not shown
                o.store(dx + row * D + c);
            }
        }
        dacc = wave_sum(dacc);
        if (lane == 0) da[row] = dacc;
        cacc += __expf(cur.sc - mxl) * isl * dacc;
        if (bn != bcur || row + 1 == rend) {
            if (lane < H) {
                if (det_cc) det_cc[(((int64_t)blockIdx.x * 4 + (threadIdx.x >> 6)) * (M / L) + bcur) * H + lane] = cacc / (float)H;
                else atomicAdd(cc + bcur * H + lane, cacc / (float)H);
                cacc = 0.f;
                if (row + 1 < rend) { mxl = mx[bn * H + lane]; isl = 1.f / sm[bn * H + lane]; }
            }
        }
        bcur = bn;
        lcur = ln;
        cur = nxt;
    }
    __shared__ float red[2][NP * 256];
    const int wave = threadIdx.x >> 6;
    for (int w = 0; w < 4; ++w) {
        if (wave == w) {
#pragma unroll
            for (int j = 0; j < NP; ++j) {
                const int c = (lane + 64 * j) * 4;
                if (c < D) {
#pragma unroll
                    for (int e = 0; e < 4; ++e) {
                        if (w == 0) { red[0][c + e] = dg[j][e]; red[1][c + e] = db[j][e]; }
                        else { red[0][c + e] += dg[j][e]; red[1][c + e] += db[j][e]; }
                    }
                }
            }
        }
        __syncthreads();
    }
    if (det_gb) {
        float* row = det_gb + (int64_t)blockIdx.x * 2 * D;
        for (int c = threadIdx.x; c < D; c += 256) { row[c] = red[0][c]; row[D + c] = red[1][c]; }
        return;
    }
    for (int c = threadIdx.x; c < D; c += 256) {
        atomicAdd(dgamma + c, red[0][c]);
        atomicAdd(dbeta + c, red[1][c]);
    }
}

template <typename T, int NP>
__global__ __launch_bounds__(256) void gate_bwd_apply_kernel(const float* __restrict__ x, const T* __restrict__ pos,
                                                             const float* __restrict__ u, const float* __restrict__ scores,
                                                             const float* __restrict__ mx, const float* __restrict__ sm,
                                                             const float* __restrict__ da, const float* __restrict__ cc,
                                                             float* __restrict__ dx, float* __restrict__ du, int L, int D,
                                                             int H, int rpw, float* __restrict__ det_du) {
    const int lane = threadIdx.x & 63, wave = threadIdx.x >> 6;
    const int b = blockIdx.y;
    const int l0 = (blockIdx.x * 4 + wave) * rpw;
    float ur[GH][NP][4], dur[GH][NP][4];
#pragma unroll
    for (int hh = 0; hh < GH; ++hh)
#pragma unroll
        for (int j = 0; j < NP; ++j) {
            const int c = (lane + 64 * j) * 4;
#pragma unroll
            for (int e = 0; e < 4; ++e) {
                ur[hh][j][e] = (hh < H && c < D) ? u[((int64_t)b * H + hh) * D + c + e] : 0.f;
                dur[hh][j][e] = 0.f;
            }
        }
    const int lend = min(l0 + rpw, L);
    Vec4<float> xv[NP], dv[NP], nxv[NP], ndv[NP];
    Vec4<T> pv[NP], npv[NP];
    float mxr[GH], isr[GH], ccr[GH], sc[GH], nsc[GH], dar = 0.f, ndar = 0.f;
#pragma unroll
    for (int hh = 0; hh < GH; ++hh) {
        mxr[hh] = hh < H ? mx[b * H + hh] : 0.f;
        isr[hh] = hh < H ? 1.f / sm[b * H + hh] : 0.f;
        ccr[hh] = hh < H ? cc[b * H + hh] : 0.f;
        sc[hh] = nsc[hh] = 0.f;
    }
    auto fetch = [&](int l, Vec4<float> (&xr)[NP], Vec4<T> (&pr)[NP], Vec4<float> (&dr)[NP], float (&sr)[GH], float& dr1) {
        const int64_t row = (int64_t)b * L + l;
#pragma unroll
        for (int j = 0; j < NP; ++j) {
            const int c = (lane + 64 * j) * 4;
            if (c < D) {
                xr[j].load(x + row * D + c);
                pr[j].load(pos + row * D + c);
                dr[j].load(dx + row * D + c);
            }
        }
#pragma unroll
        for (int hh = 0; hh < GH; ++hh)
            if (hh < H) sr[hh] = scores[((int64_t)b * H + hh) * L + l];
        dr1 = da[row];
    };
    if (l0 < lend) fetch(l0, xv, pv, dv, sc, dar);
    for (int l = l0; l < lend; ++l) {
        const int64_t row = (int64_t)b * L + l;
        if (l + 1 < lend) fetch(l + 1, nxv, npv, ndv, nsc, ndar);
        float ds[GH];
        const float dal = dar / (float)H;
#pragma unroll
        for (int hh = 0; hh < GH; ++hh) {
            if (hh < H) {
                const float pp = __expf(sc[hh] - mxr[hh]) * isr[hh];
                ds[hh] = pp * (dal - ccr[hh]);
            } else ds[hh] = 0.f;
        }
#pragma unroll
        for (int j = 0; j < NP; ++j) {
            const int c = (lane + 64 * j) * 4;
            if (c < D) {
#pragma unroll
                for (int e = 0; e < 4; ++e) {
                    const float t = xv[j].get(e) + pv[j].get(e);
                    float add = 0.f;
#pragma unroll
                    for (int hh = 0; hh < GH; ++hh) {
                        add += ds[hh] * ur[hh][j][e];
                        dur[hh][j][e] += ds[hh] * t;
                    }
                    dv[j].set(e, dv[j].get(e) + add);
                }
                dv[j].store(dx + row * D + c);
            }
        }
#pragma unroll
        for (int j = 0; j < NP; ++j) { xv[j] = nxv[j]; pv[j] = npv[j]; dv[j] = ndv[j]; }
#pragma unroll
        for (int hh = 0; hh < GH; ++hh) sc[hh] = nsc[hh];
        dar = ndar;
    }
    __shared__ float red[GH * NP * 256];
    for (int w = 0; w < 4; ++w) {
        if (wave == w) {
#pragma unroll
            for (int hh = 0; hh < GH; ++hh)
#pragma unroll
                for (int j = 0; j < NP; ++j) {
                    const int c = (lane + 64 * j) * 4;
#pragma unroll
                    for (int e = 0; e < 4; ++e) {
                        float* r = red + hh * NP * 256 + c + e;
                        if (w == 0) *r = dur[hh][j][e];
                        else *r += dur[hh][j][e];
                    }
                }
        }
        __syncthreads();
    }
    for (int i = threadIdx.x; i < GH * NP * 256; i += 256) {
        const int hh = i / (NP * 256), c = i % (NP * 256);
        if (hh < H && c < D) {
            if (det_du) det_du[(((int64_t)b * gridDim.x + blockIdx.x) * H + hh) * D + c] = red[i];
            else atomicAdd(du + ((int64_t)b * H + hh) * D + c, red[i]);
        }
    }
}

__device__ __forceinline__ void gate_vec_fwd_body(const float* __restrict__ skch, const float* __restrict__ W,
                                                  const float* __restrict__ bias, float* __restrict__ q_out,
                                                  float* __restrict__ u_out, int D, int H) {
    __shared__ float s_q[GP * 256];
    const int hh = blockIdx.x, b = blockIdx.y, tid = threadIdx.x, lane = tid & 63, wave = tid >> 6, dh = D / H;
    float sv[GP][4];
#pragma unroll
    for (int j = 0; j < GP; ++j) {
        const int c = (lane + 64 * j) * 4;
#pragma unroll
        for (int e = 0; e < 4; ++e) sv[j][e] = c < D ? skch[(int64_t)b * D + c + e] : 0.f;
    }
    for (int e = wave; e < dh; e += 4) {
        const int row = hh * dh + e;
        const float* w = W + (int64_t)row * D;
        float acc = 0.f;
#pragma unroll
        for (int j = 0; j < GP; ++j) {
// ... 162 lines not shown
#define SVOL_GATE_FWD(TT)                                                                                                   \
    do {                                                                                                                    \
        if (scored) { }                                                                                                      \
        else if (np_ == 1) hipLaunchKernelGGL((gate_scores_kernel<TT, 1>), g1, dim3(256), 0, s, x32, (const TT*)pos, u, scores, (int)L, (int)D, (int)H, rpw); \
        else if (np_ == 2) hipLaunchKernelGGL((gate_scores_kernel<TT, 2>), g1, dim3(256), 0, s, x32, (const TT*)pos, u, scores, (int)L, (int)D, (int)H, rpw); \
        else hipLaunchKernelGGL((gate_scores_kernel<TT, 4>), g1, dim3(256), 0, s, x32, (const TT*)pos, u, scores, (int)L, (int)D, (int)H, rpw); \
        hipLaunchKernelGGL(gate_stats_kernel, dim3((unsigned)(B * H)), dim3(256), 0, s, scores, mx, sm, (int)L);            \
        if (np_ == 1) hipLaunchKernelGGL((gate_apply_kernel<TT, 1>), dim3(g3), dim3(256), 0, s, x32, (const TT*)pos, scores, mx, sm, gamma, beta, y32, (TT*)y, (TT*)ypos, a, mean, rstd, (int)L, (int)D, (int)H, M); \
        else if (np_ == 2) hipLaunchKernelGGL((gate_apply_kernel<TT, 2>), dim3(g3), dim3(256), 0, s, x32, (const TT*)pos, scores, mx, sm, gamma, beta, y32, (TT*)y, (TT*)ypos, a, mean, rstd, (int)L, (int)D, (int)H, M); \
        else hipLaunchKernelGGL((gate_apply_kernel<TT, 4>), dim3(g3), dim3(256), 0, s, x32, (const TT*)pos, scores, mx, sm, gamma, beta, y32, (TT*)y, (TT*)ypos, a, mean, rstd, (int)L, (int)D, (int)H, M); \
    } while (0)
    if (dtype == SVOL_BF16) SVOL_GATE_FWD(bf16_t);
    else if (dtype == SVOL_F16) SVOL_GATE_FWD(f16_t);
    else SVOL_GATE_FWD(float);
#undef SVOL_GATE_FWD
    SVOL_CHECK_LAUNCH();
    return SVOL_OK;
}

int svol_gate_fwd(const float* x32, const void* pos, const float* u, const float* gamma, const float* beta, float* y32,
                  void* y, void* ypos, float* a, float* mean, float* rstd, float* ws, int64_t B, int64_t L, int64_t D, int64_t H,
                  int dtype, void* stream) {
    return gate_fwd_impl(x32, pos, u, gamma, beta, y32, y, ypos, a, mean, rstd, ws, B, L, D, H, dtype, stream, false);
}

int svol_gate_fwd_scored(const float* x32, const void* pos, const float* u, const float* gamma, const float* beta, float* y32,
                         void* y, void* ypos, float* a, float* mean, float* rstd, float* ws, int64_t B, int64_t L, int64_t D,
                         int64_t H, int dtype, void* stream) {
    return gate_fwd_impl(x32, pos, u, gamma, beta, y32, y, ypos, a, mean, rstd, ws, B, L, D, H, dtype, stream, true);
}

int svol_layernorm_gate_scores_fwd(const float* x32, const float* gamma, const float* beta, float* y32, void* y, void* ypos,
                                   const void* pos, float* mean, float* rstd, const float* u_next, float* scores_next, int64_t B,
                                   int64_t L, int64_t D, int64_t H, int dtype, void* stream) {
    if (!x32 || !gamma || !beta || (!y && !y32 && !ypos) || !pos || !mean || !rstd || !u_next || !scores_next) return SVOL_E_INVALID;
    if (!aligned16(gamma) || !aligned16(beta) || !aligned16(u_next)) return SVOL_E_INVALID;
    if (B <= 0 || L <= 0 || D <= 0 || H <= 0) return SVOL_E_INVALID;
    if (D % 4 || D > 256 || H > GH || L % 4 || L > (1 << 24) || B > 65535) return SVOL_E_UNSUPPORTED;
    if (!svol_is16(dtype) && dtype != SVOL_F32) return SVOL_E_INVALID;
    hipStream_t s = reinterpret_cast<hipStream_t>(stream);
    const dim3 grid((unsigned)(L / 4), (unsigned)B);
    const size_t lds = (size_t)GH * D * sizeof(float);
#define SVOL_LNS(TT)                                                                                                          \
    hipLaunchKernelGGL((ln_scores_kernel<TT, 1>), grid, dim3(256), lds, s, x32, gamma, beta, y32, (TT*)y, (TT*)ypos,               \
                       (const TT*)pos, mean, rstd, u_next, scores_next, (int)L, (int)D, (int)H)
    if (dtype == SVOL_BF16) SVOL_LNS(bf16_t);
    else if (dtype == SVOL_F16) SVOL_LNS(f16_t);
    else SVOL_LNS(float);
#undef SVOL_LNS
    SVOL_CHECK_LAUNCH();
    return SVOL_OK;
}

int svol_gate_bwd(const float* dy32, const void* dy, const void* dy2, const float* x32, const void* pos, const float* u,
                  const float* gamma, const float* a, const float* mean, const float* rstd, const float* ws, float* ws2,
                  float* dx32, float* du, float* dgamma, float* dbeta, int64_t B, int64_t L, int64_t D, int64_t H, int dtype,
                  void* stream) {
    if ((!dy32 && !dy && !dy2) || !x32 || !pos || !u || !gamma || !a || !mean || !rstd || !ws || !ws2 || !dx32 || !du ||
        !dgamma || !dbeta)
        return SVOL_E_INVALID;
    if (B <= 0 || L <= 0 || D <= 0 || H <= 0) return SVOL_E_INVALID;
    if (D % 4 || D > GP * 256 || H > GH || B > 65535 || L > (1 << 24)) return SVOL_E_UNSUPPORTED;
    if (!svol_is16(dtype) && dtype != SVOL_F32) return SVOL_E_INVALID;
    hipStream_t s = reinterpret_cast<hipStream_t>(stream);
    const int np_ = D <= 256 ? 1 : (D <= 512 ? 2 : 4);
    const float* scores = ws;
    const float* mx = ws + B * H * L;
    const float* sm = mx + B * H;
    float* da = ws2;
    float* cc = ws2 + B * L;
    const int64_t M = B * L;
    const int rpw1 = rows_per_wave(M, gate_waves(1));
    const unsigned g1 = (unsigned)(((M + rpw1 - 1) / rpw1 + 3) / 4);
    const int rpw3 = rows_per_wave(L, gate_waves(2) / B + 1);
    dim3 g3((unsigned)((L + 4 * rpw3 - 1) / (4 * rpw3)), (unsigned)B);
    if (hipMemsetAsync(cc, 0, sizeof(float) * (size_t)(B * H), s) != hipSuccess) return SVOL_E_LAUNCH;
    const bool det_mode = svol_deterministic();
    const size_t n_cc = (size_t)g1 * 4 * (size_t)(B * H), n_gb = (size_t)g1 * 2 * (size_t)D, n_du = (size_t)B * g3.x * (size_t)(H * D);
    DetScratch det(det_mode ? n_cc + n_gb + n_du : 0, s, true);
    if (det_mode && !det.p) return SVOL_E_LAUNCH;
    float* det_cc = det_mode ? det.p : nullptr;
    float* det_gb = det_mode ? det.p + n_cc : nullptr;
    float* det_du = det_mode ? det.p + n_cc + n_gb : nullptr;
#define SVOL_GATE_BWD(TT)                                                                                                   \
    do {                                                                                                                    \
        if (np_ == 1) hipLaunchKernelGGL((gate_bwd_ln_kernel<TT, 1>), dim3(g1), dim3(256), 0, s, dy32, (const TT*)dy, (const TT*)dy2, x32, a, gamma, mean, rstd, dx32, da, dgamma, dbeta, scores, mx, sm, cc, (int)L, (int)H, M, (int)D, rpw1, det_cc, det_gb); \
        else if (np_ == 2) hipLaunchKernelGGL((gate_bwd_ln_kernel<TT, 2>), dim3(g1), dim3(256), 0, s, dy32, (const TT*)dy, (const TT*)dy2, x32, a, gamma, mean, rstd, dx32, da, dgamma, dbeta, scores, mx, sm, cc, (int)L, (int)H, M, (int)D, rpw1, det_cc, det_gb); \
        else hipLaunchKernelGGL((gate_bwd_ln_kernel<TT, 4>), dim3(g1), dim3(256), 0, s, dy32, (const TT*)dy, (const TT*)dy2, x32, a, gamma, mean, rstd, dx32, da, dgamma, dbeta, scores, mx, sm, cc, (int)L, (int)H, M, (int)D, rpw1, det_cc, det_gb); \
        if (det_mode) {                                                                                                     \
            det_fold(det_cc, (int)(g1 * 4), B * H, cc, B * H, s);                                                           \
            det_fold(det_gb, (int)g1, 2 * D, dgamma, D, s);                                                                 \
            det_fold(det_gb + D, (int)g1, 2 * D, dbeta, D, s);                                                              \
        }                                                                                                                   \
        if (np_ == 1) hipLaunchKernelGGL((gate_bwd_apply_kernel<TT, 1>), g3, dim3(256), 0, s, x32, (const TT*)pos, u, scores, mx, sm, da, cc, dx32, du, (int)L, (int)D, (int)H, rpw3, det_du); \
        else if (np_ == 2) hipLaunchKernelGGL((gate_bwd_apply_kernel<TT, 2>), g3, dim3(256), 0, s, x32, (const TT*)pos, u, scores, mx, sm, da, cc, dx32, du, (int)L, (int)D, (int)H, rpw3, det_du); \
        else hipLaunchKernelGGL((gate_bwd_apply_kernel<TT, 4>), g3, dim3(256), 0, s, x32, (const TT*)pos, u, scores, mx, sm, da, cc, dx32, du, (int)L, (int)D, (int)H, rpw3, det_du); \
    } while (0)
    if (dtype == SVOL_BF16) SVOL_GATE_BWD(bf16_t);
    else if (dtype == SVOL_F16) SVOL_GATE_BWD(f16_t);
    else SVOL_GATE_BWD(float);
#undef SVOL_GATE_BWD
    if (det_mode) det_fold(det_du, (int)g3.x, H * D, du, H * D, s, (int)B, (int64_t)g3.x * H * D, H * D);
    SVOL_CHECK_LAUNCH();
    return SVOL_OK;
}

int svol_gate_vectors_fwd(const float* skch, const float* W_in, const float* b_in, float* q_out, float* u_out, int64_t B, int64_t D,
                          int64_t H, void* stream) {
    if (!skch || !W_in || !b_in || !q_out || !u_out || B <= 0 || D <= 0 || H <= 0) return SVOL_E_INVALID;
    if (D % 4 || D > GP * 256 || H > GH || D % H || B > 65535) return SVOL_E_UNSUPPORTED;
    if (!aligned16(W_in)) return SVOL_E_INVALID;
    hipLaunchKernelGGL(gate_vec_fwd_kernel, dim3((unsigned)H, (unsigned)B), dim3(256), 0, reinterpret_cast<hipStream_t>(stream), skch,
                       W_in, b_in, q_out, u_out, (int)D, (int)H);
    SVOL_CHECK_LAUNCH();
    return SVOL_OK;
}

int svol_gate_vectors_bwd(const float* du, const float* skch, const float* W_in, const float* q, float* dq_ws, float* dskch,
                          float* dW_in, float* db_in, int64_t B, int64_t D, int64_t H, void* stream) {
    if (!du || !skch || !W_in || !q || !dq_ws || !dW_in || !db_in || B <= 0 || D <= 0 || H <= 0) return SVOL_E_INVALID;
    if (D % 4 || D > GP * 256 || H > GH || D % H || B > 65535) return SVOL_E_UNSUPPORTED;
    if (!aligned16(W_in)) return SVOL_E_INVALID;
    hipStream_t s = reinterpret_cast<hipStream_t>(stream);
    hipLaunchKernelGGL(gate_vec_bwd_a_kernel, dim3((unsigned)H, (unsigned)B), dim3(256), 0, s, du, W_in, dq_ws, (int)D, (int)H);
    hipLaunchKernelGGL(gate_vec_bwd_b_kernel, dim3((unsigned)(D + B)), dim3(256), 0, s, du, skch, q, dq_ws, W_in, dW_in, db_in, dskch,
                       (int)B, (int)D, (int)H);
    SVOL_CHECK_LAUNCH();
    return SVOL_OK;
}

int svol_gate_vectors_fwd_multi(const float* skch, const float* const* W_in, const float* const* b_in, float* const* q_out,
                                float* const* u_out, int64_t n_layers, int64_t B, int64_t D, int64_t H, void* stream) {
    if (!skch || !W_in || !b_in || !q_out || !u_out || B <= 0 || D <= 0 || H <= 0 || n_layers <= 0) return SVOL_E_INVALID;
    if (D % 4 || D > GP * 256 || H > GH || D % H || B > 65535 || n_layers > SVOL_GATE_VEC_MAX_LAYERS) return SVOL_E_UNSUPPORTED;
    GateVecMulti g{};
    for (int l = 0; l < n_layers; ++l) {
        if (!W_in[l] || !b_in[l] || !q_out[l] || !u_out[l] || !aligned16(W_in[l])) return SVOL_E_INVALID;
        g.W[l] = W_in[l]; g.bias[l] = b_in[l]; g.q[l] = q_out[l]; g.u[l] = u_out[l];
    }
    hipLaunchKernelGGL(gate_vec_fwd_multi_kernel, dim3((unsigned)H, (unsigned)B, (unsigned)n_layers), dim3(256), 0,
                       reinterpret_cast<hipStream_t>(stream), skch, g, (int)D, (int)H);
    SVOL_CHECK_LAUNCH();
    return SVOL_OK;
}

int svol_gate_vectors_bwd_multi(const float* const* du, const float* skch, const float* const* W_in, const float* const* q,
                                float* const* dq_ws, float* const* dskch, float* const* dW_in, float* const* db_in, int64_t n_layers,
                                int64_t B, int64_t D, int64_t H, void* stream) {
    if (!du || !skch || !W_in || !q || !dq_ws || !dW_in || !db_in || B <= 0 || D <= 0 || H <= 0 || n_layers <= 0) return SVOL_E_INVALID;
    if (D % 4 || D > GP * 256 || H > GH || D % H || B > 65535 || n_layers > SVOL_GATE_VEC_MAX_LAYERS) return SVOL_E_UNSUPPORTED;
    GateVecMulti g{};
    for (int l = 0; l < n_layers; ++l) {
        if (!du[l] || !W_in[l] || !q[l] || !dq_ws[l] || !dW_in[l] || !db_in[l] || !aligned16(W_in[l])) return SVOL_E_INVALID;
        g.du[l] = du[l]; g.W[l] = W_in[l]; g.q[l] = const_cast<float*>(q[l]); g.dq[l] = dq_ws[l]; g.dW[l] = dW_in[l]; g.db[l] = db_in[l];
        g.dskch[l] = dskch ? dskch[l] : nullptr;
    }
    hipStream_t s = reinterpret_cast<hipStream_t>(stream);
// ... 9 lines not shown
```

svol_amd/csrc/norm.hip:

```cpp
#include "common.h"

namespace {

constexpr int LN_MAX_PASSES = 4;

template <typename T, typename TX, int NP>
__global__ __launch_bounds__(256) void ln_fwd_kernel(const TX* __restrict__ x, const float* __restrict__ gamma,
                                                     const float* __restrict__ beta, float* __restrict__ y32,
                                                     T* __restrict__ y, T* __restrict__ ypos, const T* __restrict__ pos,
                                                     int64_t pos_rows, float* __restrict__ mean, float* __restrict__ rstd,
                                                     int64_t M, int D, float p, float inv_keep, uint64_t seed0,
                                                     const int64_t* __restrict__ soff) {
    const uint64_t seed = seed0 + (soff ? ((uint64_t)soff[0] << 8) : 0ull);
    const int lane = threadIdx.x & 63;
    const int64_t row = (int64_t)blockIdx.x * 4 + (threadIdx.x >> 6);
    if (row >= M) return;
    const TX* xr = x + row * D;
    float v[NP][4];
    float s = 0.f;
    const T* pr = pos ? pos + (row % pos_rows) * D : nullptr;
    Vec4<TX> t[NP];
    Vec4<T> pv[NP];
    Vec4<float> gv[NP], bv[NP];
#pragma unroll
// ... 6 lines not shown
            bv[j].load(beta + c);
        }
    }
#pragma unroll
    for (int j = 0; j < NP; ++j) {
        const int c = (lane + 64 * j) * 4;
#pragma unroll
        for (int e = 0; e < 4; ++e) {
            v[j][e] = c < D ? t[j].get(e) : 0.f;
            s += v[j][e];
        }
    }
    const float mu = wave_sum(s) / (float)D;
    float q = 0.f;
#pragma unroll
    for (int j = 0; j < NP; ++j) {
        const int c = (lane + 64 * j) * 4;
        if (c < D) {
#pragma unroll
            for (int e = 0; e < 4; ++e) { const float d = v[j][e] - mu; q += d * d; }
        }
    }
    const float rs = rsqrtf(wave_sum(q) / (float)D + 1e-5f);
    if (lane == 0) { mean[row] = mu; rstd[row] = rs; }
#pragma unroll
    for (int j = 0; j < NP; ++j) {
        const int c = (lane + 64 * j) * 4;
        if (c < D) {
            Vec4<T> o, op;
            Vec4<float> o32;
#pragma unroll
            for (int e = 0; e < 4; ++e) {
                float r = (v[j][e] - mu) * rs * gv[j].get(e) + bv[j].get(e);
                if (p > 0.f) r *= dropout_scale(seed, (uint64_t)row, (uint32_t)(c + e), p, inv_keep);
                o.set(e, r);
                o32.set(e, r);
                if (pr) op.set(e, r + pv[j].get(e));
            }
            if (y32) o32.store(y32 + row * D + c);
            if (y) o.store(y + row * D + c);
            if (ypos) op.store(ypos + row * D + c);
        }
    }
}

template <typename T, typename TX, int NP>
__global__ __launch_bounds__(256) void ln_bwd_kernel(const float* __restrict__ dy32, const T* __restrict__ dy,
                                                     const T* __restrict__ dy2, const TX* __restrict__ x,
                                                     const float* __restrict__ gamma, const float* __restrict__ mean,
                                                     const float* __restrict__ rstd, float* __restrict__ dx32,
                                                     T* __restrict__ dx, float* __restrict__ dgamma,
                                                     float* __restrict__ dbeta, float* __restrict__ dxsum, int64_t M, int D,
                                                     float p, float inv_keep, uint64_t seed0, const int64_t* __restrict__ soff, int rows_per_wave,
                                                     float* __restrict__ det_part) {
    const uint64_t seed = seed0 + (soff ? ((uint64_t)soff[0] << 8) : 0ull);
    const int lane = threadIdx.x & 63;
    const int64_t wave_id = (int64_t)blockIdx.x * 4 + (threadIdx.x >> 6);
    const int64_t r0 = wave_id * rows_per_wave;
    float dg[NP][4], db[NP][4], dxs[NP][4], gm[NP][4];
#pragma unroll
    for (int j = 0; j < NP; ++j) {
        const int c = (lane + 64 * j) * 4;
#pragma unroll
        for (int e = 0; e < 4; ++e) { dg[j][e] = 0.f; db[j][e] = 0.f; dxs[j][e] = 0.f; gm[j][e] = c < D ? gamma[c + e] : 0.f; }
    }
    struct Row { Vec4<float> a32[NP]; Vec4<T> a[NP], b[NP]; Vec4<TX> xv[NP]; float mu, rs; };
    auto fetch = [&](int64_t row, Row& r) {
#pragma unroll
        for (int j = 0; j < NP; ++j) {
            const int c = (lane + 64 * j) * 4;
            if (c < D) {
                if (dy32) r.a32[j].load(dy32 + row * D + c);
                if (dy) r.a[j].load(dy + row * D + c);
                if (dy2) r.b[j].load(dy2 + row * D + c);
                r.xv[j].load(x + row * D + c);
            }
        }
        r.mu = mean[row];
        r.rs = rstd[row];
    };
    const int64_t rend = (r0 + rows_per_wave < M) ? r0 + rows_per_wave : M;
    Row cur, nxt;
    if (r0 < rend) fetch(r0, cur);
    for (int64_t row = r0; row < rend; ++row) {
        if (row + 1 < rend) fetch(row + 1, nxt);
        const float mu = cur.mu, rs = cur.rs;
        float g[NP][4], xh[NP][4];
        float s1 = 0.f, s2 = 0.f;
#pragma unroll
        for (int j = 0; j < NP; ++j) {
            const int c = (lane + 64 * j) * 4;
            if (c < D) {
#pragma unroll
                for (int e = 0; e < 4; ++e) {
                    float d = (dy32 ? cur.a32[j].get(e) : 0.f) + (dy ? cur.a[j].get(e) : 0.f) + (dy2 ? cur.b[j].get(e) : 0.f);
                    if (p > 0.f) d *= dropout_scale(seed, (uint64_t)row, (uint32_t)(c + e), p, inv_keep);
                    const float h = (cur.xv[j].get(e) - mu) * rs;
                    xh[j][e] = h;
                    dg[j][e] += d * h;
                    db[j][e] += d;
                    const float gg = d * gm[j][e];
                    g[j][e] = gg;
                    s1 += gg;
                    s2 += gg * h;
                }
            }
        }
        s1 = wave_sum(s1) / (float)D;
        s2 = wave_sum(s2) / (float)D;
#pragma unroll
        for (int j = 0; j < NP; ++j) {
            const int c = (lane + 64 * j) * 4;
            if (c < D) {
                Vec4<T> o;
                Vec4<float> o32;
#pragma unroll
                for (int e = 0; e < 4; ++e) {
                    const float r = rs * (g[j][e] - s1 - xh[j][e] * s2);
                    dxs[j][e] += r;
                    o.set(e, r);
                    o32.set(e, r);
                }
                if (dx32) o32.store(dx32 + row * D + c);
                if (dx) o.store(dx + row * D + c);
            }
        }
        cur = nxt;
    }
    __shared__ float red[3][NP * 256];
    const int wave = threadIdx.x >> 6;
    for (int w = 0; w < 4; ++w) {
        if (wave == w) {
#pragma unroll
            for (int j = 0; j < NP; ++j) {
                const int c = (lane + 64 * j) * 4;
                if (c < D) {
#pragma unroll
                    for (int e = 0; e < 4; ++e) {
                        if (w == 0) { red[0][c + e] = dg[j][e]; red[1][c + e] = db[j][e]; red[2][c + e] = dxs[j][e]; }
                        else { red[0][c + e] += dg[j][e]; red[1][c + e] += db[j][e]; red[2][c + e] += dxs[j][e]; }
                    }
                }
            }
        }
        __syncthreads();
    }
    if (det_part) {
        float* row = det_part + (int64_t)blockIdx.x * 3 * D;
        for (int c = threadIdx.x; c < D; c += 256) { row[c] = red[0][c]; row[D + c] = red[1][c]; row[2 * D + c] = red[2][c]; }
        return;
    }
    for (int c = threadIdx.x; c < D; c += 256) {
        atomicAdd(dgamma + c, red[0][c]);
        atomicAdd(dbeta + c, red[1][c]);
        if (dxsum) atomicAdd(dxsum + c, red[2][c]);
    }
}

template <typename T>
__global__ __launch_bounds__(256) void posenc_kernel(const float* __restrict__ mask, T* __restrict__ pos, int L, int D) {
    __shared__ float red[2][4];
    __shared__ float xe[64];
    const int b = blockIdx.y, tid = threadIdx.x, lane = tid & 63, wave = tid >> 6;
    const float* mr = mask + (int64_t)b * L;
    const int l0 = blockIdx.x * 64;
    float before = 0.f, all = 0.f;
    for (int l = tid; l < L; l += 256) {
        const float v = (mr[l] != 0.f) ? 1.f : 0.f;
        all += v;
        if (l < l0) before += v;
    }
// ... 54 lines not shown
    const uint32_t s0 = drop_seed32(seed);
    int64_t i = ((int64_t)blockIdx.x * blockDim.x + threadIdx.x) * 4;
    const int64_t stride = (int64_t)gridDim.x * blockDim.x * 4;
    for (; i < n; i += stride) {
        int64_t r = i / row_len;
        int64_t k = i - r * row_len;
        uint32_t rm = drop_row(s0, (uint64_t)r);
#pragma unroll
        for (int e = 0; e < 4; ++e) {
            if (i + e >= n) break;
            out[i + e] = res[i + e] + t[i + e] * drop_scale_rk(rm, (uint32_t)k, p, inv_keep);
            if (++k == row_len) { k = 0; ++r; rm = drop_row(s0, (uint64_t)r); }
        }
    }
}
}

extern "C" {

int svol_layernorm_fwd(const void* x, int x_f32, const float* gamma, const float* beta, float* y32, void* y,
                       void* ypos, const void* pos, int64_t pos_rows, float* mean, float* rstd, int64_t M, int64_t D,
                       float dropout_p, uint64_t seed, const int64_t* seed_offset_dev, int dtype, void* stream) {
    if (!x || !gamma || !beta || (!y && !y32) || !mean || !rstd || M < 0 || D <= 0) return SVOL_E_INVALID;
    if (!aligned16(gamma) || !aligned16(beta)) return SVOL_E_INVALID;
    if ((ypos != nullptr) != (pos != nullptr)) return SVOL_E_INVALID;
    if (pos && pos_rows <= 0) return SVOL_E_INVALID;
    if (D % 4 || D > LN_MAX_PASSES * 256) return SVOL_E_UNSUPPORTED;
    if (dropout_p < 0.f || dropout_p >= 1.f) return SVOL_E_INVALID;
    if (!svol_is16(dtype) && dtype != SVOL_F32) return SVOL_E_INVALID;
    if (M == 0) return SVOL_OK;
    const float inv_keep = 1.f / (1.f - dropout_p);
    const unsigned grid = (unsigned)((M + 3) / 4);
    hipStream_t s = reinterpret_cast<hipStream_t>(stream);
#define SVOL_LNF(TT, TXX, NPP)                                                                                              \
    hipLaunchKernelGGL((ln_fwd_kernel<TT, TXX, NPP>), dim3(grid), dim3(256), 0, s, (const TXX*)x, gamma, beta, y32, (TT*)y,      \
                       (TT*)ypos, (const TT*)pos, pos_rows, mean, rstd, M, (int)D, dropout_p, inv_keep, seed, seed_offset_dev)
#define SVOL_LNF_NP(TT, TXX)                     \
    do {                                         \
        if (D <= 256) SVOL_LNF(TT, TXX, 1);      \
        else if (D <= 512) SVOL_LNF(TT, TXX, 2); \
        else SVOL_LNF(TT, TXX, 4);               \
    } while (0)
    if (dtype == SVOL_BF16 && x_f32) SVOL_LNF_NP(bf16_t, float);
    else if (dtype == SVOL_BF16) SVOL_LNF_NP(bf16_t, bf16_t);
    else if (dtype == SVOL_F16 && x_f32) SVOL_LNF_NP(f16_t, float);
    else if (dtype == SVOL_F16) SVOL_LNF_NP(f16_t, f16_t);
    else SVOL_LNF_NP(float, float);
#undef SVOL_LNF_NP
#undef SVOL_LNF
    SVOL_CHECK_LAUNCH();
    return SVOL_OK;
}

int svol_layernorm_bwd(const float* dy32, const void* dy, const void* dy2, const void* x, int x_f32, const float* gamma,
                       const float* mean, const float* rstd, float* dx32, void* dx, float* dgamma, float* dbeta,
                       float* dx_colsum, int64_t M, int64_t D, float dropout_p, uint64_t seed, const int64_t* seed_offset_dev,
                       int dtype, void* stream) {
    if ((!dy32 && !dy && !dy2) || !x || !gamma || !mean || !rstd || (!dx && !dx32) || !dgamma || !dbeta || M < 0 || D <= 0)
        return SVOL_E_INVALID;
    if (D % 4 || D > LN_MAX_PASSES * 256) return SVOL_E_UNSUPPORTED;
    if (dropout_p < 0.f || dropout_p >= 1.f) return SVOL_E_INVALID;
    if (!svol_is16(dtype) && dtype != SVOL_F32) return SVOL_E_INVALID;
    if (M == 0) return SVOL_OK;
    const float inv_keep = 1.f / (1.f - dropout_p);
    int64_t rpw = (M + 2047) / 2048;
    if (rpw < 1) rpw = 1;
    const int64_t waves = (M + rpw - 1) / rpw;
    const unsigned grid = (unsigned)((waves + 3) / 4);
    hipStream_t s = reinterpret_cast<hipStream_t>(stream);
    const bool det_mode = svol_deterministic();
    DetScratch det(det_mode ? (size_t)grid * 3 * (size_t)D : 0, s);
    if (det_mode && !det.p) return SVOL_E_LAUNCH;
#define SVOL_LNB(TT, TXX, NPP)                                                                                                      \
    hipLaunchKernelGGL((ln_bwd_kernel<TT, TXX, NPP>), dim3(grid), dim3(256), 0, s, dy32, (const TT*)dy, (const TT*)dy2, (const TXX*)x, \
                       gamma, mean, rstd, dx32, (TT*)dx, dgamma, dbeta, dx_colsum, M, (int)D, dropout_p, inv_keep, seed,              \
                       seed_offset_dev, (int)rpw, det.p)
#define SVOL_LNB_NP(TT, TXX)                  \
    do {                                      \
        if (D <= 256) SVOL_LNB(TT, TXX, 1);   \
        else if (D <= 512) SVOL_LNB(TT, TXX, 2); \
        else SVOL_LNB(TT, TXX, 4);            \
    } while (0)
    if (dtype == SVOL_BF16 && x_f32) SVOL_LNB_NP(bf16_t, float);
    else if (dtype == SVOL_BF16) SVOL_LNB_NP(bf16_t, bf16_t);
    else if (dtype == SVOL_F16 && x_f32) SVOL_LNB_NP(f16_t, float);
    else if (dtype == SVOL_F16) SVOL_LNB_NP(f16_t, f16_t);
    else SVOL_LNB_NP(float, float);
#undef SVOL_LNB_NP
#undef SVOL_LNB
    if (det_mode) {
        det_fold(det.p, (int)grid, 3 * D, dgamma, D, s);
        det_fold(det.p + D, (int)grid, 3 * D, dbeta, D, s);
        det_fold(det.p + 2 * D, (int)grid, 3 * D, dx_colsum, D, s);
    }
    SVOL_CHECK_LAUNCH();
    return SVOL_OK;
}

int svol_dropout(const void* x, void* y, int64_t n, int64_t row_len, float p, uint64_t seed, int dtype, void* stream) {
    if (!x || !y || n < 0 || row_len <= 0 || row_len > 0xffffffffll || !(p >= 0.f && p < 1.f)) return SVOL_E_INVALID;
    if (n == 0) return SVOL_OK;
    const float inv = 1.f / (1.f - p);
    int64_t g = (n + 1023) / 1024;
    if (g > 8192) g = 8192;
    hipStream_t s = reinterpret_cast<hipStream_t>(stream);
    if (dtype == SVOL_F32) hipLaunchKernelGGL(dropout_kernel<float>, dim3((unsigned)g), dim3(256), 0, s, (const float*)x, (float*)y, n, row_len, p, inv, seed);
    else if (dtype == SVOL_BF16) hipLaunchKernelGGL(dropout_kernel<bf16_t>, dim3((unsigned)g), dim3(256), 0, s, (const bf16_t*)x, (bf16_t*)y, n, row_len, p, inv, seed);
    else if (dtype == SVOL_F16) hipLaunchKernelGGL(dropout_kernel<f16_t>, dim3((unsigned)g), dim3(256), 0, s, (const f16_t*)x, (f16_t*)y, n, row_len, p, inv, seed);
    else return SVOL_E_INVALID;
    SVOL_CHECK_LAUNCH();
    return SVOL_OK;
}

int svol_dropout_add(const float* t32, const float* res32, float* out32, int64_t n, int64_t row_len, float p, uint64_t seed, void* stream) {
    if (!t32 || !res32 || !out32 || n < 0 || row_len <= 0 || row_len > 0xffffffffll || !(p >= 0.f && p < 1.f)) return SVOL_E_INVALID;
    if (n == 0) return SVOL_OK;
    int64_t g = (n + 1023) / 1024;
    if (g > 8192) g = 8192;
    hipLaunchKernelGGL(dropout_add_kernel, dim3((unsigned)g), dim3(256), 0, reinterpret_cast<hipStream_t>(stream), t32, res32, out32, n,
                       row_len, p, 1.f / (1.f - p), seed);
    SVOL_CHECK_LAUNCH();
    return SVOL_OK;
}

int svol_posenc_sine(const float* mask, void* pos, int64_t B, int64_t L, int64_t D, int dtype, void* stream) {
    if (!mask || !pos || B <= 0 || L <= 0 || D <= 0) return SVOL_E_INVALID;
    if (L > (1 << 24) || D > 4096) return SVOL_E_UNSUPPORTED;
    hipStream_t s = reinterpret_cast<hipStream_t>(stream);
    if (B > 65535) return SVOL_E_UNSUPPORTED;
    dim3 grid((unsigned)((L + 63) / 64), (unsigned)B);
    if (dtype == SVOL_BF16)
        hipLaunchKernelGGL(posenc_kernel<bf16_t>, grid, dim3(256), 0, s, mask, (bf16_t*)pos, (int)L, (int)D);
    else if (dtype == SVOL_F16)
        hipLaunchKernelGGL(posenc_kernel<f16_t>, grid, dim3(256), 0, s, mask, (f16_t*)pos, (int)L, (int)D);
    else if (dtype == SVOL_F32)
        hipLaunchKernelGGL(posenc_kernel<float>, grid, dim3(256), 0, s, mask, (float*)pos, (int)L, (int)D);
    else return SVOL_E_INVALID;
    SVOL_CHECK_LAUNCH();
    return SVOL_OK;
}

}
```

svol_amd/modeling/cross_modal_transformer.py:

```python
from __future__ import annotations

import copy
import os

import torch
from torch import nn

from .. import blocks, ops

D_FF = 2048


class MLP(nn.Module):

    def __init__(self, in_features, hidden_features):
        super().__init__()
        self.fc1 = nn.Linear(in_features, hidden_features)
        self.fc2 = nn.Linear(hidden_features, in_features)


OVERLAP_QUERY_STREAM = os.environ.get('SVOL_NO_STREAM_OVERLAP') is None
QUERY_FP32 = os.environ.get('SVOL_QUERY_BF16') is None
_SIDE = {}

# ... 87 lines not shown
        dbs = [sb.view if sb is not None else torch.zeros((3 * d,), dtype=torch.float32, device=dev) for _, sb in ctx.sinks]
        ws = torch.empty((n, B, d), dtype=torch.float32, device=dev)
        dsk = torch.empty((n, B, d), dtype=torch.float32, device=dev) if ctx.needs_input_grad[0] else None
        rc = _lib.lib().svol_gate_vectors_bwd_multi(_ptr_array(dus), ops._ptr(skch), _ptr_array([w.detach() for w in Ws]),
                                                    _ptr_array(list(q.unbind(0))), _ptr_array(list(ws.unbind(0))),
                                                    None if dsk is None else _ptr_array(list(dsk.unbind(0))), _ptr_array(dWs),
                                                    _ptr_array(dbs), n, B, d, h, ops._stream())
        _lib.check(rc, 'svol_gate_vectors_bwd_multi')
        grads = [None if dsk is None else dsk.sum(0), None]
        for l, (sW, sb) in enumerate(ctx.sinks):
            grads += [None if sW is not None else dWs[l], None if sb is not None else dbs[l]]
        return tuple(grads)


GATE_VECTORS_MULTI_MAX = 8


def all_gate_vectors(layers, skch):
    import os
    if len(layers) > GATE_VECTORS_MULTI_MAX or len(layers) < 2 or os.environ.get('SVOL_GATE_VEC_PER_LAYER') is not None:
        return [layer.gate_vectors(skch) for layer in layers]
    params = []
    for layer in layers:
        a = layer.sketch_video_cross_attn
        params += [a.in_proj_weight, a.in_proj_bias]
    return list(_GateVectorsAllFn.apply(skch, layers[0].nhead, *params))


class CrossModalTransformerLayer(nn.Module):
    def __init__(self, d_model=512, nhead=8, dim_feedforward=D_FF):
        super().__init__()
        self.sketch_video_cross_attn = nn.MultiheadAttention(d_model, nhead)
        self.norm1 = nn.LayerNorm(d_model)
        self.content_self_attn = nn.MultiheadAttention(d_model, nhead)
        self.norm2 = nn.LayerNorm(d_model)
        self.mlp1 = MLP(d_model, dim_feedforward)
        self.norm3 = nn.LayerNorm(d_model)
        self.token_self_attn = nn.MultiheadAttention(d_model, nhead)
        self.norm4 = nn.LayerNorm(d_model)
        self.content_token_cross_attn = nn.MultiheadAttention(d_model, nhead)
        self.norm5 = nn.LayerNorm(d_model)
        self.mlp2 = MLP(d_model, dim_feedforward)
        self.norm6 = nn.LayerNorm(d_model)
        self.d_model, self.nhead = d_model, nhead

    def gate_vectors(self, skch):
        m = self.sketch_video_cross_attn
        return _GateVectorsFn.apply(skch, m.in_proj_weight, m.in_proj_bias, self.nhead)

    def forward(self, mem32, skch32, out, pos, qpos, kbias, u=None):
        m32, m, mpos = self.video_half(mem32, skch32, pos, u)
        return m32, self.query_half(out, m, mpos, qpos, kbias)

    def video_half(self, mem32, skch32, pos, u=None, u_next=None, sc_in=None):
        if blocks.ENABLED:
            uu = self.gate_vectors(skch32) if u is None else u
            m32, m, mpos, sc = blocks.video_half(self, mem32, pos, uu, pos.dtype, u_next, sc_in)
            return (m32, m, mpos) if u_next is None else (m32, m, mpos, sc)
        assert sc_in is None
        h = self.nhead
        n = lambda m: (m.weight, m.bias)
        mha = lambda m: (m.in_proj_weight, m.in_proj_bias, m.out_proj.weight, m.out_proj.bias)
        mlp = lambda m: (m.fc1.weight, m.fc1.bias, m.fc2.weight, m.fc2.bias)
        m32, m, mpos = ops.gate(mem32, pos, self.gate_vectors(skch32) if u is None else u, *n(self.norm1), h)
        m32, m = ops.self_attn_ln(m32, m, mpos, *mha(self.content_self_attn), *n(self.norm2), None, h)
        return ops.mlp_ln(m32, m, *mlp(self.mlp1), *n(self.norm3), pos)

    def query_half(self, out, m, mpos, qpos, kbias):
        return self.query_cross(self.query_self(out, qpos, m.dtype), m, mpos, qpos, kbias)

    def query_self(self, out, qpos, dt=None):
        if blocks.ENABLED:
            return blocks.query_self(self, out, qpos, dt if dt is not None else qpos.dtype, qpos.dtype)
        n = lambda m_: (m_.weight, m_.bias)
        mha = lambda m_: (m_.in_proj_weight, m_.in_proj_bias, m_.out_proj.weight, m_.out_proj.bias)
        o32, o, opos = out
        return ops.self_attn_ln(o32, o, opos, *mha(self.token_self_attn), *n(self.norm4), qpos, self.nhead)

    def query_cross(self, out, m, mpos, qpos, kbias):
        n = lambda m_: (m_.weight, m_.bias)
        mha = lambda m_: (m_.in_proj_weight, m_.in_proj_bias, m_.out_proj.weight, m_.out_proj.bias)
        mlp = lambda m_: (m_.fc1.weight, m_.fc1.bias, m_.fc2.weight, m_.fc2.bias)
        if blocks.ENABLED:
            return blocks.query_cross(self, out, m, mpos, kbias, qpos, m.dtype, qpos.dtype)
        o32, o, opos = out
        o32, o = ops.cross_attn_ln(o32, o, opos, mpos, m, *mha(self.content_token_cross_attn), *n(self.norm5), None, self.nhead,
                                   kbias)
        return ops.mlp_ln(o32, o, *mlp(self.mlp2), *n(self.norm6), qpos)


class CrossModalTransformer(nn.Module):
    def __init__(self, d_model=512, nhead=8, num_layers=6, dim_feedforward=D_FF):
        super().__init__()
        layer = CrossModalTransformerLayer(d_model, nhead, dim_feedforward)
        self.layers = nn.ModuleList([copy.deepcopy(layer) for _ in range(num_layers)])
        for p in self.parameters():
            if p.dim() > 1:
                nn.init.xavier_uniform_(p)
        self.d_model, self.nhead, self.num_layers = d_model, nhead, num_layers
        self._epoch_seen = -1

    def forward(self, src_vid32, src_skch32, kbias, vid_pos, query_embed, us=None):
        if ops.weights.epoch == self._epoch_seen:
            ops.weights.new_epoch()
        self._epoch_seen = ops.weights.epoch
        B = src_vid32.shape[0]
        dt = torch.float32 if QUERY_FP32 else vid_pos.dtype
        qpos = ops.cast_ag(query_embed, dt)
        N, d = qpos.shape
        def initial_queries():
            return (torch.zeros((B, N, d), dtype=torch.float32, device=vid_pos.device),
                    torch.zeros((B, N, d), dtype=dt, device=vid_pos.device),
                    qpos.unsqueeze(0).expand(B, -1, -1).contiguous())
        mem32 = src_vid32
        outputs = []
        if us is None:
            us = all_gate_vectors(list(self.layers), src_skch32)
        if not OVERLAP_QUERY_STREAM:
            out = initial_queries()
            for layer, u in zip(self.layers, us):
                mem32, out = layer(mem32, src_skch32, out, vid_pos, qpos, kbias, u)
                outputs.append(out[0])
            return torch.stack(outputs)
        main = torch.cuda.current_stream()
        side = _side_stream(main.device)
        side.wait_stream(main)
        qpos.record_stream(side)
        kbias.record_stream(side)
        with torch.cuda.stream(side):
            out = initial_queries()
        sc = None
        for li, (layer, u) in enumerate(zip(self.layers, us)):
            with torch.cuda.stream(side):
                out_sa = layer.query_self(out, qpos, vid_pos.dtype)
            if blocks.ENABLED and blocks.GATE_SCORES_FUSE and li + 1 < len(us):
                m32, m, mpos, sc = layer.video_half(mem32, src_skch32, vid_pos, u, us[li + 1], sc)
            elif sc is not None:
                m32, m, mpos = layer.video_half(mem32, src_skch32, vid_pos, u, None, sc)
            else:
                m32, m, mpos = layer.video_half(mem32, src_skch32, vid_pos, u)
            side.wait_stream(main)
            m.record_stream(side)
            mpos.record_stream(side)
            with torch.cuda.stream(side):
                out = layer.query_cross(out_sa, m, mpos, qpos, kbias)
                outputs.append(out[0])
            mem32 = m32
        main.wait_stream(side)
        for t in outputs:
            t.record_stream(main)
        return torch.stack(outputs)


def build_cross_modal_transformer(args):
    return CrossModalTransformer(d_model=args.hidden_dim, nhead=args.nheads, num_layers=args.num_layers,
                                 dim_feedforward=D_FF)
```

svol_amd/modeling/svanet.py:

```python
from __future__ import annotations

import os

import torch
from torch import nn

from .. import ops
from . import cross_modal_transformer as cmt
from .cross_modal_transformer import build_cross_modal_transformer
from .position_encoding import build_position_encoding

INPUT_OVERLAP = os.environ.get('SVOL_NO_INPUT_OVERLAP') is None

_DTYPES = {'bf16': torch.bfloat16, 'fp32': torch.float32, 'fp16': torch.float16, torch.float16: torch.float16, torch.bfloat16: torch.bfloat16,
           torch.float32: torch.float32}


class MLP(nn.Module):

    def __init__(self, input_dim, hidden_dim, output_dim, num_layers):
        super().__init__()
        self.num_layers = num_layers
        h = [hidden_dim] * (num_layers - 1)
        self.layers = nn.ModuleList(nn.Linear(n, k) for n, k in zip([input_dim] + h, h + [output_dim]))

    def forward(self, x, last_act=ops.ACT_NONE):
        for i, layer in enumerate(self.layers):
            act = ops.ACT_RELU if i < self.num_layers - 1 else last_act
            x = ops.linear(x, layer.weight, layer.bias, act)
        return x


class LinearLayer(nn.Module):

    def __init__(self, in_hsz, out_hsz, layer_norm=True, dropout=0.1, relu=True):
        super().__init__()
        self.relu = relu
        self.layer_norm = layer_norm
        self.p = dropout
        if layer_norm:
            self.LayerNorm = nn.LayerNorm(in_hsz)
        self.net = nn.Sequential(nn.Dropout(dropout), nn.Linear(in_hsz, out_hsz))

    def forward(self, x, seed=0, out_f32=False, seed_dev=None):
        p = self.p if self.training else 0.0
        if self.layer_norm:
            x = ops.layer_norm(x, self.LayerNorm.weight, self.LayerNorm.bias, p, seed, seed_dev)
        elif p > 0.0:
            raise NotImplementedError('dropout without LayerNorm is not on the reference path')
        lin = self.net[1]
        return ops.linear(x, lin.weight, lin.bias, ops.ACT_RELU if self.relu else ops.ACT_NONE, out_f32)


class SVANet(nn.Module):
    def __init__(self, transformer, sketch_position_embed, video_position_embed, input_vid_dim, input_skch_dim,
                 num_queries, input_dropout=0.1, aux_loss=True, use_sketch_pos=True, n_input_proj=2, num_classes=2,
                 vis_mode=None, compute_dtype='bf16'):
        super().__init__()
        self.num_queries = num_queries
        self.num_classes = num_classes
        self.transformer = transformer
        self.sketch_position_embed = sketch_position_embed
        self.video_position_embed = video_position_embed
        hidden_dim = transformer.d_model
        self.bbox_embed = MLP(hidden_dim, hidden_dim, 4, 3)
        self.use_sketch_pos = use_sketch_pos
        self.class_embed = nn.Linear(hidden_dim, 2)
        self.n_input_proj = n_input_proj
        self.class_head = nn.Linear(hidden_dim, num_classes)
        self.query_embed = nn.Embedding(num_queries, hidden_dim)
        relu_args = [True] * 3
        relu_args[n_input_proj - 1] = False
        self.input_video_proj = nn.Sequential(*[
            LinearLayer(input_vid_dim, hidden_dim, dropout=input_dropout, relu=relu_args[0]),
            LinearLayer(hidden_dim, hidden_dim, dropout=input_dropout, relu=relu_args[1]),
            LinearLayer(hidden_dim, hidden_dim, dropout=input_dropout, relu=relu_args[2])][:n_input_proj])
        self.input_sketch_proj = nn.Sequential(*[
            LinearLayer(input_skch_dim, hidden_dim, dropout=input_dropout, relu=relu_args[0]),
            LinearLayer(hidden_dim, hidden_dim, dropout=input_dropout, relu=relu_args[1]),
            LinearLayer(hidden_dim, hidden_dim, dropout=input_dropout, relu=relu_args[2])][:n_input_proj])
        self.vis_mode = vis_mode
        self.aux_loss = aux_loss
        self.compute_dtype = _DTYPES[compute_dtype]
        self._step = 0
        self.base_seed = 1
        self.step_dev = None

    def _proj(self, seq, x, salt):
        n = len(seq)
        for j, layer in enumerate(seq):
            x = layer(x, seed=(self.base_seed << 32) + (self._step << 8) + salt * 16 + j, out_f32=(j == n - 1),
                      seed_dev=self.step_dev)
        return x

    def forward(self, src_sketch, src_sketch_mask, src_video, src_video_mask):
        if not src_video.is_cuda:
            raise RuntimeError('svol_amd.SVANet runs on the MI355X HIP kernels only; move the module and its '
                               'inputs to cuda (there is no CPU path — the CPU oracle lives under oracle/).')
        dt = self.compute_dtype
        d = self.transformer.d_model
        overlap = INPUT_OVERLAP and cmt.OVERLAP_QUERY_STREAM and isinstance(self.transformer, cmt.CrossModalTransformer)
        if not overlap:
            ops.weights.new_epoch()
        if self.training:
            self._step += 1
        def mask_side(with_us):
            mask_f = src_video_mask.to(torch.float32)
            pos_video = self.video_position_embed(mask_f, d, dt)
            skch = self._proj(self.input_sketch_proj, ops.cast_ag(src_sketch.float(), dt), 1)
            skch = skch.reshape(skch.shape[0], -1)
            kbias = torch.zeros_like(mask_f).masked_fill_(mask_f == 0, float('-inf'))
            us = cmt.all_gate_vectors(list(self.transformer.layers), skch) if with_us else None
            return pos_video, skch, kbias, us

        if overlap:
            main = torch.cuda.current_stream()
            side = cmt._side_stream(main.device)
            side.wait_stream(main)
            with torch.cuda.stream(side):
                ops.weights.new_epoch()
                casts_done = side.record_event()
            xv = ops.cast_ag(src_video.float(), dt)
            with torch.cuda.stream(side):
                pos_video, skch, kbias, us = mask_side(True)
            main.wait_event(casts_done)
            vid = self._proj(self.input_video_proj, xv, 0)
            main.wait_stream(side)
            for t in [pos_video, skch, kbias] + list(us or []):
                t.record_stream(main)
        else:
            vid = self._proj(self.input_video_proj, ops.cast_ag(src_video.float(), dt), 0)
            pos_video, skch, kbias, us = mask_side(False)
        hs = (self.transformer(vid, skch, kbias, pos_video, self.query_embed.weight, us) if us is not None else
              self.transformer(vid, skch, kbias, pos_video, self.query_embed.weight))
        if ops.heads_fusable(hs, self.class_embed, self.bbox_embed):
            outputs_class, outputs_coord = ops.heads(hs, self.class_embed, self.bbox_embed)
        else:
            outputs_class = ops.linear(hs, self.class_embed.weight, self.class_embed.bias)
            outputs_coord = self.bbox_embed(hs, last_act=ops.ACT_SIGMOID)
        out = {'pred_logits': outputs_class[-1], 'pred_boxes': outputs_coord[-1]}
        if self.aux_loss:
            out['aux_outputs'] = [{'pred_logits': a, 'pred_boxes': b}
                                  for a, b in zip(outputs_class[:-1], outputs_coord[:-1])]
        out['_svol_stacked'] = (outputs_class, outputs_coord)
        if self.vis_mode is not None:
            return out, hs
        return out


def build_svanet(args):
    transformer = build_cross_modal_transformer(args)
    sketch_position_embed, video_position_embed = build_position_encoding(args)
    return SVANet(transformer, sketch_position_embed, video_position_embed, input_vid_dim=args.input_vid_dim,
                  input_skch_dim=args.input_skch_dim, num_queries=args.num_queries,
                  input_dropout=args.input_dropout, aux_loss=args.aux_loss, use_sketch_pos=args.use_sketch_pos,
                  n_input_proj=args.n_input_proj, vis_mode=args.vis_mode,
                  compute_dtype=getattr(args, 'compute_dtype', 'bf16'))
```

Before: 15130.

## Fuse input projection into a block, skip the last-layer fp32 output, merge position grads, twin bf16 dx

Adds a fused input-projection block (LayerNorm, dropout, linear, ReLU stack) with its own fwd/bwd/wgrad kernels and slot table, replacing the separate cast and per-op projection calls. The video-half block can now skip writing the fp32 M32 output for the last layer and skip a separate DXQ buffer when the position input needs no grad. The query-cross DMPOS buffer is likewise dropped in that case. A bf16 twin of dx is also emitted and handed off to later consumers. The aim is fewer launches and less memory traffic, at the cost of more code paths and cached twin-gradient state that must stay consistent.

```diff
diff --git a/include/svol_hip.h b/include/svol_hip.h
--- a/include/svol_hip.h
+++ b/include/svol_hip.h
@@ -100,6 +100,10 @@
                        const float* gamma, const float* mean, const float* rstd, float* dx32, void* dx,
                        float* dgamma, float* dbeta, float* dx_colsum, int64_t M, int64_t D, float dropout_p,
                        uint64_t seed, const int64_t* seed_offset_dev, int dtype, void* stream);
+enum { SVOL_LN_RELU_MASK = 1, SVOL_LN_NO_DX = 2 };
+int svol_layernorm_bwd_ex(const float* dy32, const void* dy, const void* dy2, const void* x, int x_f32, const float* gamma,
+                          const float* mean, const float* rstd, float* dx32, void* dx, float* dgamma, float* dbeta, int64_t M, int64_t D,
+                          float dropout_p, uint64_t seed, const int64_t* seed_offset_dev, int flags, int dtype, void* stream);
 
 int svol_dropout(const void* x, void* y, int64_t n, int64_t row_len, float p, uint64_t seed, int dtype, void* stream);
 int svol_dropout_add(const float* t32, const float* res32, float* out32, int64_t n, int64_t row_len, float p, uint64_t seed, void* stream);
@@ -142,6 +146,10 @@
                   const float* u, const float* gamma, const float* a, const float* mean, const float* rstd,
                   const float* ws, float* ws2, float* dx32, float* du, float* dgamma, float* dbeta, int64_t B,
                   int64_t L, int64_t D, int64_t H, int dtype, void* stream);
+int svol_gate_bwd_twin(const float* dy32, const void* dy, const void* dy2, const float* x32, const void* pos, const float* u,
+                       const float* gamma, const float* a, const float* mean, const float* rstd, const float* ws, float* ws2,
+                       float* dx32, void* dx16, float* du, float* dgamma, float* dbeta, int64_t B, int64_t L, int64_t D, int64_t H,
+                       int dtype, void* stream);
 
 int svol_layernorm_gate_scores_fwd(const float* x32, const float* gamma, const float* beta, float* y32, void* y, void* ypos,
                                    const void* pos, float* mean, float* rstd, const float* u_next, float* scores_next,
@@ -257,6 +265,7 @@
 #define SVOL_BLK_VIDEO_HALF 0
 #define SVOL_BLK_QUERY_SELF 1
 #define SVOL_BLK_QUERY_CROSS 2
+#define SVOL_BLK_INPUT_PROJ 3
 const char* svol_block_slot_names(int block);
 int svol_block_trace_dump(char* buf, int64_t cap);
 int svol_clock_probe(uint64_t* samples, int32_t* count, int32_t max_samples, const int32_t* stop, int64_t period_us,
@@ -272,7 +281,7 @@
     X(DM32) X(DM) X(DMPOS) X(DS32_3) X(DS3) X(DPRE) X(DY2) X(DS32_2) X(G2D) X(DO) X(DQKV) X(DELTA) X(DXQP) X(DXQ) X(GATE_WS2) \
     X(DX32) X(DU) \
     X(DG1) X(DBT1) X(DG2) X(DBT2) X(DG3) X(DBT3) X(DW_IN) X(DB_IN) X(DW_O) X(DB_O) X(DW_FC1) X(DB_FC1) X(DW_FC2) X(DB_FC2) \
-    X(EV_A0) X(EV_A1) X(EV_CLEAN_IN) X(EV_PREP) X(ATTN_WS_NEXT) X(ZERO_STREAM) X(EV_CLEAN_OUT)
+    X(EV_A0) X(EV_A1) X(EV_CLEAN_IN) X(EV_PREP) X(ATTN_WS_NEXT) X(ZERO_STREAM) X(EV_CLEAN_OUT) X(DX16)
 #define SVOL_QS_SLOTS(X) \
     X(O32) X(O) X(OPOS) X(QPOS) X(B_IN) X(B_O) X(G4) X(BT4) X(QSCALE) X(W_IN) X(WV_HILO) X(W_O) X(W_IN_T) X(W_O_T) \
     X(QKV) X(OA) X(LSE) X(S4) X(MEAN4) X(RSTD4) X(Y32) X(Y) X(YPOS) X(ATTN_WS) \
@@ -286,12 +295,19 @@
     X(DY32) X(DY) X(DYPOS) X(DS32_6) X(DS6) X(DPRE) X(DY5) X(DS32_5) X(G5D) X(DOAQ) X(DOA) X(DQC) X(DQ) X(DKV) X(DELTA) \
     X(DO32) X(DXQP) X(DMPOS) X(DMV) X(DQPOS) \
     X(DW_IN) X(DB_IN) X(DW_O) X(DB_O) X(DG5) X(DBT5) X(DW_FC1) X(DB_FC1) X(DW_FC2) X(DB_FC2) X(DG6) X(DBT6)
+#define SVOL_IP_SLOTS(X) \
+    X(X32) X(XC) X(G1) X(BT1) X(B1) X(G2) X(BT2) X(B2) X(SEED_DEV) X(W1) X(W1_T) X(W2) X(W2_T) \
+    X(H1) X(MEAN1) X(RSTD1) X(Y1) X(H2) X(MEAN2) X(RSTD2) X(OUT32) \
+    X(DOUT32) X(DOUT) X(DH2) X(DY1) X(DH1) X(DX) \
+    X(DG1) X(DBT1) X(DW1) X(DB1) X(DG2) X(DBT2) X(DW2) X(DB2)
 #define SVOL_SLOT_ENUM_VH(n) SVOL_VH_##n,
 #define SVOL_SLOT_ENUM_QS(n) SVOL_QS_##n,
 #define SVOL_SLOT_ENUM_QC(n) SVOL_QC_##n,
+#define SVOL_SLOT_ENUM_IP(n) SVOL_IP_##n,
 enum { SVOL_VH_SLOTS(SVOL_SLOT_ENUM_VH) SVOL_VH_COUNT };
 enum { SVOL_QS_SLOTS(SVOL_SLOT_ENUM_QS) SVOL_QS_COUNT };
 enum { SVOL_QC_SLOTS(SVOL_SLOT_ENUM_QC) SVOL_QC_COUNT };
+enum { SVOL_IP_SLOTS(SVOL_SLOT_ENUM_IP) SVOL_IP_COUNT };
 
 int svol_video_half_fwd(const int64_t* dims, void* const* slots, void* stream);
 int svol_video_half_bwd(const int64_t* dims, void* const* slots, int phase, void* stream);
@@ -303,6 +319,9 @@
 int svol_query_cross_fwd(const int64_t* dims, void* const* slots, void* stream);
 int svol_query_cross_bwd(const int64_t* dims, void* const* slots, void* stream);
 int svol_query_cross_wgrad(const int64_t* dims, void* const* slots, void* stream);
+int svol_input_proj_fwd(const int64_t* dims, void* const* slots, float p1, uint64_t seed1, float p2, uint64_t seed2, void* stream);
+int svol_input_proj_bwd(const int64_t* dims, void* const* slots, float p1, uint64_t seed1, float p2, uint64_t seed2, void* stream);
+int svol_input_proj_wgrad(const int64_t* dims, void* const* slots, void* stream);
 
 #ifdef __cplusplus
 }
diff --git a/svol_amd/_lib.py b/svol_amd/_lib.py
--- a/svol_amd/_lib.py
+++ b/svol_amd/_lib.py
@@ -34,6 +34,7 @@
     'svol_colsum': [_p, _i64, _p, _i64, _i64, _int, _p],
     'svol_act_bwd': [_p, _p, _p, _int, _i64, _int, _p],
     'svol_layernorm_fwd': [_p, _int, _p, _p, _p, _p, _p, _p, _i64, _p, _p, _i64, _i64, _f32, _u64, _p, _int, _p],
+    'svol_layernorm_bwd_ex': [_p, _p, _p, _p, _int, _p, _p, _p, _p, _p, _p, _p, _i64, _i64, _f32, _u64, _p, _int, _int, _p],
     'svol_layernorm_bwd': [_p, _p, _p, _p, _int, _p, _p, _p, _p, _p, _p, _p, _p, _i64, _i64, _f32, _u64, _p, _int, _p],
     'svol_cast_transpose_multi': [_p, _int, _i64, _int, _p],
     'svol_postprocess': [_p, _p, _p, _i64, _i64, _i64, _p],
@@ -99,6 +100,7 @@
     'svol_gate_fwd': [_p, _p, _p, _p, _p, _p, _p, _p, _p, _p, _p, _p, _i64, _i64, _i64, _i64, _int, _p],
     'svol_gate_bwd': [_p, _p, _p, _p, _p, _p, _p, _p, _p, _p, _p, _p, _p, _p, _p, _p, _i64, _i64, _i64, _i64, _int,
                       _p],
+    'svol_gate_bwd_twin': [_p, _p, _p, _p, _p, _p, _p, _p, _p, _p, _p, _p, _p, _p, _p, _p, _p, _i64, _i64, _i64, _i64, _int, _p],
     'svol_clock_probe': [_p, _p, _int, _p, _i64, _i64, _p, _p],
     'svol_gate_fwd_scored': [_p, _p, _p, _p, _p, _p, _p, _p, _p, _p, _p, _p, _i64, _i64, _i64, _i64, _int, _p],
     'svol_layernorm_gate_scores_fwd': [_p, _p, _p, _p, _p, _p, _p, _p, _p, _p, _p, _i64, _i64, _i64, _i64, _int, _p],
@@ -119,6 +121,9 @@
     'svol_query_cross_fwd': [_p, _p, _p],
     'svol_query_cross_bwd': [_p, _p, _p],
     'svol_query_cross_wgrad': [_p, _p, _p],
+    'svol_input_proj_fwd': [_p, _p, _f32, _u64, _f32, _u64, _p],
+    'svol_input_proj_bwd': [_p, _p, _f32, _u64, _f32, _u64, _p],
+    'svol_input_proj_wgrad': [_p, _p, _p],
 }
 
 
diff --git a/svol_amd/blocks.py b/svol_amd/blocks.py
--- a/svol_amd/blocks.py
+++ b/svol_amd/blocks.py
@@ -1,5 +1,6 @@
 from __future__ import annotations
 
+import copy
 import ctypes
 import math
 import os
@@ -12,7 +13,7 @@
 WGRAD_SPLIT = os.environ.get('SVOL_WGRAD_SPLIT') is not None
 ENABLED = os.environ.get('SVOL_NO_BLOCKS') is None
 GATE_SCORES_FUSE = os.environ.get('SVOL_GATE_SCORES_FUSE') is not None
-VH, QS, QC = 0, 1, 2
+VH, QS, QC, IP = 0, 1, 2, 3
 _F32, _BF16 = 0, 1
 _ESZ = {torch.float32: 4, torch.bfloat16: 2, torch.float16: 2}
 _SLOTS = {}
@@ -116,7 +117,12 @@
     ('DW_FC1', lambda l: l.mlp2.fc1.weight), ('DB_FC1', lambda l: l.mlp2.fc1.bias),
     ('DW_FC2', lambda l: l.mlp2.fc2.weight), ('DB_FC2', lambda l: l.mlp2.fc2.bias),
     ('DG6', lambda l: l.norm6.weight), ('DBT6', lambda l: l.norm6.bias)]
-_PARAMS = {VH: _VH_PARAMS, QS: _QS_PARAMS, QC: _QC_PARAMS}
+_IP_PARAMS = [
+    ('DG1', lambda l: l[0].LayerNorm.weight), ('DBT1', lambda l: l[0].LayerNorm.bias),
+    ('DW1', lambda l: l[0].net[1].weight), ('DB1', lambda l: l[0].net[1].bias),
+    ('DG2', lambda l: l[1].LayerNorm.weight), ('DBT2', lambda l: l[1].LayerNorm.bias),
+    ('DW2', lambda l: l[1].net[1].weight), ('DB2', lambda l: l[1].net[1].bias)]
+_PARAMS = {VH: _VH_PARAMS, QS: _QS_PARAMS, QC: _QC_PARAMS, IP: _IP_PARAMS}
 
 
 class BlockPlan:
@@ -128,7 +134,7 @@
         self.grad_slots = [n for n, _ in _PARAMS[block]]
         self.tpl = _Table(block)
         self.keep = []
-        D = layer.d_model
+        D = layer.d_model if block != IP else layer[1].net[1].weight.shape[0]
         self.split_v = ops.SPLIT_V and D % 32 == 0
         t = self.tpl
         W = ops.weights
@@ -179,6 +185,12 @@
                 self.keep.append(hl)
                 self.casts.append((m.in_proj_weight, 2 * D, D, hl))
             t.set_t('QSCALE', qscale(qdt, 2 * D))
+        elif block == IP:
+            for n_, p_ in zip(('G1', 'BT1', 'W1', 'B1', 'G2', 'BT2', 'W2', 'B2'), self.params):
+                if n_ in ('W1', 'W2'):
+                    both(n_, p_, dt)
+                else:
+                    t.set_t(n_, p_)
         else:
             m, mlp = layer.content_token_cross_attn, layer.mlp2
             for n_, p_ in (('G5', layer.norm5.weight), ('BT5', layer.norm5.bias), ('G6', layer.norm6.weight), ('BT6', layer.norm6.bias),
@@ -207,6 +219,17 @@
                 cnt[(id(s.owner), s.bucket)] = (s.owner, s.bucket, cnt.get((id(s.owner), s.bucket), (None, None, 0))[2] + 1)
         self.notify = list(cnt.values())
         self.key = self._key()
+        self.m32, self.twin = True, False
+        self._variants = {}
+
+    def variant(self, m32=True, twin=False):
+        if m32 and not twin:
+            return self
+        v = self._variants.get((m32, twin))
+        if v is None:
+            v = self._variants[(m32, twin)] = copy.copy(self)
+            v.m32, v.twin = m32, twin
+        return v
 
     def _key(self):
         k = []
@@ -369,19 +392,22 @@
     return st or None
 
 
-def _vh_fwd_layout(B, L, D, H, F, e):
+def _vh_fwd_layout(B, L, D, H, F, e, m32=True):
     M = B * L
+    out = [('M32', M * D * 4)] if m32 else []
     return [('Y1', M * D * e), ('Y1POS', M * D * e), ('A', M * 4), ('MEAN1', M * 4), ('RSTD1', M * 4), ('GATE_WS', B * H * (L + 2) * 4),
             ('QKV', M * 3 * D * e), ('O', M * D * e), ('LSE', B * H * L * 4), ('S2', M * D * 4), ('Y2', M * D * e), ('MEAN2', M * 4),
             ('RSTD2', M * 4), ('PRE', M * F * e), ('HID', M * F * e), ('S3', M * D * 4), ('MEAN3', M * 4), ('RSTD3', M * 4),
-            ('M32', M * D * 4), ('M', M * D * e), ('MPOS', M * D * e)]
-
-
-def _vh_bwd_layout(B, L, D, H, F, e):
+            ('M', M * D * e), ('MPOS', M * D * e)] + out
+
+
+def _vh_bwd_layout(B, L, D, H, F, e, merged=False, twin=False):
     M = B * L
+    dxq = [] if merged else [('DXQ', M * D * e)]
+    dxq += [('DX16', M * D * e)] if twin else []
     return [('DS32_3', M * D * 4), ('DS3', M * D * e), ('DPRE', M * F * e), ('DY2', M * D * e), ('DS32_2', M * D * 4), ('G2D', M * D * e),
-            ('DO', M * D * e), ('DQKV', M * 3 * D * e), ('DELTA', 3 * B * H * L * 4), ('DXQP', M * D * e), ('DXQ', M * D * e),
-            ('GATE_WS2', (B * L + B * H) * 4), ('DX32', M * D * 4)]
+            ('DO', M * D * e), ('DQKV', M * 3 * D * e), ('DELTA', 3 * B * H * L * 4), ('DXQP', M * D * e),
+            ('GATE_WS2', (B * L + B * H) * 4), ('DX32', M * D * 4)] + dxq
 
 
 class VideoHalfFn(torch.autograd.Function):
@@ -404,7 +430,7 @@
         assert x2.dtype == torch.float32 and pos2.dtype == dt and u.dtype == torch.float32
         wsb = _attn_ws_bytes(B, H, L, L, D // H, dt)
         key = (VH, B, L, D, H, F, dt)
-        lay = _layout(('f',) + key, lambda: _vh_fwd_layout(B, L, D, H, F, e))
+        lay = _layout(('f', pl.m32) + key, lambda: _vh_fwd_layout(B, L, D, H, F, e, pl.m32))
         slay = _layout(('s',) + key, lambda: [('Y1_32', M * D * 4), ('Y2_32', M * D * 4), ('ATTN_WS', max(wsb, 16))])
         arena = torch.empty((lay.total,), dtype=torch.uint8, device=dev)
         scr = _scratch(dev, slay.total)
@@ -443,9 +469,13 @@
         ctx.n_par = len(params)
         ctx.sc_in = sc_in
         ctx.save_for_backward(x2, pos2, u)
-        ctx.mark_non_differentiable(sc_next)
-        return (lay.view(arena, 'M32', torch.float32, (B, L, D)), lay.view(arena, 'M', dt, (B, L, D)),
-                lay.view(arena, 'MPOS', dt, (B, L, D)), sc_next)
+        if pl.m32:
+            m32 = lay.view(arena, 'M32', torch.float32, (B, L, D))
+            ctx.mark_non_differentiable(sc_next)
+        else:
+            m32 = torch.empty((0,), dtype=torch.float32, device=dev)
+            ctx.mark_non_differentiable(m32, sc_next)
+        return m32, lay.view(arena, 'M', dt, (B, L, D)), lay.view(arena, 'MPOS', dt, (B, L, D)), sc_next
 
     @staticmethod
     def backward(ctx, dm32, dm, dmpos, _dsc=None):
@@ -462,7 +492,10 @@
         M = B * L
         cont = lambda t_: None if t_ is None else (t_.reshape(M, D) if t_.is_contiguous() else t_.reshape(M, D).contiguous())
         dm32, dm, dmpos = cont(dm32), cont(dm), cont(dmpos)
-        lay = _layout(('b', VH, B, L, D, H, F, dt), lambda: _vh_bwd_layout(B, L, D, H, F, e))
+        merged = not ctx.needs_input_grad[2]
+        twin = pl.twin and dt != torch.float32
+        lay = _layout(('b', merged, VH, B, L, D, H, F, dt) + (('twin',) if twin else ()),
+                      lambda: _vh_bwd_layout(B, L, D, H, F, e, merged, twin))
         tmp = torch.empty((lay.total,), dtype=torch.uint8, device=dev)
         lay.fill(tbl, tmp.data_ptr())
         du = torch.zeros((B, H, D), dtype=torch.float32, device=dev)
@@ -504,20 +537,43 @@
             _lib.check(L_.svol_video_half_wgrad(dims, tbl.arr, s), 'svol_video_half_wgrad')
         pl.done(n_par > 0)
         dx32 = lay.view(tmp, 'DX32', torch.float32, (B, L, D))
+        if twin:
+            _twin_put(dx32, lay.view(tmp, 'DX16', dt, (B, L, D)))
         needs = ctx.needs_input_grad
         return (None, dx32, None, du if needs[3] else None, None, None) + tuple(pl.grads_out(bufs, needs[6:], n_par > 0))
 
 
+_TWINS = {}
+
+
+def _twin_put(dx32, dx16):
+    _TWINS.clear()
+    _TWINS[dx32.data_ptr()] = (dx32, dx32._version, dx16)
+
+
+def _twin_take(g32):
+    ent = _TWINS.pop(g32.data_ptr(), None)
+    if ent is None:
+        return None
+    dx32, version, dx16 = ent
+    if g32.shape != dx32.shape or g32.dtype != dx32.dtype or not g32.is_contiguous() or g32._version != version or \
+            dx32._version != version:
+        return None
+    return dx16
+
+
 def gate_scores_fusable(L, D, H):
     return GATE_SCORES_FUSE and L % 4 == 0 and D % 4 == 0 and D <= 256 and H <= 8
 
 
-def video_half(layer, x32, pos, u, dt, u_next=None, sc_in=None):
-    pl = plan(layer, VH, dt, dt)
+def video_half(layer, x32, pos, u, dt, u_next=None, sc_in=None, m32=True):
+    pl = plan(layer, VH, dt, dt).variant(m32, bool(getattr(x32, '_svol_twin', False)) and dt != torch.float32)
     if u_next is not None and not gate_scores_fusable(x32.shape[1], x32.shape[2], layer.nhead):
         u_next = None
-    m32, m, mpos, sc = VideoHalfFn.apply(pl, x32, pos, u, u_next, sc_in, *pl.inputs(x32, u))
-    return m32, m, mpos, (sc if u_next is not None else None)
+    m32_, m, mpos, sc = VideoHalfFn.apply(pl, x32, pos, u, u_next, sc_in, *pl.inputs(x32, u))
+    if not pos.requires_grad:
+        mpos._svol_m = weakref.ref(m)
+    return (m32_ if m32 else None), m, mpos, (sc if u_next is not None else None)
 
 
 def _qpos_target(pl, qpos, tbl, dev, N, D):
@@ -630,18 +686,20 @@
             ('YPOS', R * D * qe)]
 
 
-def _qc_bwd_layout(B, N, L, D, H, F, e, qe):
+def _qc_bwd_layout(B, N, L, D, H, F, e, qe, merged=False):
     R, M = B * N, B * L
+    dmpos = [] if merged else [('DMPOS', M * D * e)]
     return [('DS32_6', R * D * 4), ('DS6', R * D * qe), ('DPRE', R * F * qe), ('DY5', R * D * qe), ('G5D', R * D * qe), ('DOAQ', R * D * qe),
             ('DOA', R * D * e), ('DQC', R * D * e), ('DQ', R * D * qe), ('DKV', M * 2 * D * e), ('DELTA', 3 * B * H * N * 4),
-            ('DO32', R * D * 4), ('DXQP', R * D * qe), ('DMPOS', M * D * e), ('DMV', M * D * e)]
+            ('DO32', R * D * 4), ('DXQP', R * D * qe), ('DMV', M * D * e)] + dmpos
 
 
 class QueryCrossFn(torch.autograd.Function):
 
     @staticmethod
-    def forward(ctx, pl, o32, o, opos, mv, mpos, kbias, qpos, *params):
+    def forward(ctx, pl, merged, o32, o, opos, mv, mpos, kbias, qpos, *params):
         ctx.set_materialize_grads(False)
+        ctx.merged = bool(merged)
         B, N, D = o.shape
         L = mv.shape[1]
         layer = pl.layer()
@@ -680,13 +738,14 @@
         n_par = ctx.n_par
         if dy32 is None and dy is None and dypos is None:
             pl.done(n_par > 0)
-            return (None,) * (8 + n_par)
+            return (None,) * (9 + n_par)
         dt, qdt = pl.dt, pl.qdt
         e, qe = _ESZ[dt], _ESZ[qdt]
         dev = o_.device
         cont = lambda t_: None if t_ is None else (t_ if t_.is_contiguous() else t_.contiguous())
         dy32, dy, dypos = cont(dy32), cont(dy), cont(dypos)
-        lay = _layout(('b', QC, B, N, L, D, H, F, dt, qdt), lambda: _qc_bwd_layout(B, N, L, D, H, F, e, qe))
+        merged = ctx.merged
+        lay = _layout(('b', merged, QC, B, N, L, D, H, F, dt, qdt), lambda: _qc_bwd_layout(B, N, L, D, H, F, e, qe, merged))
         tmp = torch.empty((lay.total,), dtype=torch.uint8, device=dev)
         lay.fill(tbl, tmp.data_ptr())
         tbl.set_t('DY32', dy32)
@@ -697,7 +756,7 @@
         slay.fill(tbl, scr.data_ptr())
         needs = ctx.needs_input_grad
         gq = None
-        if needs[7]:
+        if needs[8]:
             gq, _ = _qpos_target(pl, qpos, tbl, dev, N, D)
         else:
             tbl.set('DQPOS', None)
@@ -715,14 +774,110 @@
             gq = ops.cast(gq, qdt)
         vq = lambda n_, dt_: lay.view(tmp, n_, dt_, (B, N, D))
         vm = lambda n_: lay.view(tmp, n_, dt, (B, L, D))
-        return (None, vq('DO32', torch.float32), None, vq('DXQP', qdt), vm('DMV'), vm('DMPOS'), None, gq) + \
-            tuple(pl.grads_out(bufs, needs[8:], n_par > 0))
+        return (None, None, vq('DO32', torch.float32), None, vq('DXQP', qdt), vm('DMV'), None if merged else vm('DMPOS'), None, gq) + \
+            tuple(pl.grads_out(bufs, needs[9:], n_par > 0))
 
 
 def query_cross(layer, out, mv, mpos, kbias, qpos, dt, qdt):
     pl = plan(layer, QC, dt, qdt)
     o32, o, opos = out
-    return QueryCrossFn.apply(pl, o32, o, opos, mv, mpos, kbias, qpos, *pl.inputs(o32, opos, mv, mpos))
+    of = getattr(mpos, '_svol_m', None)
+    merged = of is not None and of() is mv
+    return QueryCrossFn.apply(pl, merged, o32, o, opos, mv, mpos, kbias, qpos, *pl.inputs(o32, opos, mv, mpos))
+
+
+class InputProjFn(torch.autograd.Function):
+
+    @staticmethod
+    def forward(ctx, pl, x, p1, seed1, p2, seed2, seed_dev, *params):
+        ctx.set_materialize_grads(False)
+        seq = pl.layer()
+        D, Din = seq[1].net[1].weight.shape[0], x.shape[-1]
+        dt = pl.dt
+        e = _ESZ[dt]
+        dev = x.device
+        x2 = x.reshape(-1, Din)
+        x2 = x2 if x2.is_contiguous() else x2.contiguous()
+        assert x2.dtype == torch.float32
+        M = x2.shape[0]
+        xc = [] if dt == torch.float32 else [('XC', M * Din * e)]
+        lay = _layout(('f', IP, M, D, Din, dt), lambda: xc + [('H1', M * Din * e), ('MEAN1', M * 4), ('RSTD1', M * 4), ('Y1', M * D * e),
+                                                               ('H2', M * D * e), ('MEAN2', M * 4), ('RSTD2', M * 4),
+                                                               ('OUT32', M * D * 4)])
+        arena = torch.empty((lay.total,), dtype=torch.uint8, device=dev)
+        tbl = _Table(IP, pl.tpl)
+        lay.fill(tbl, arena.data_ptr())
+        tbl.set('X32' if dt != torch.float32 else 'XC', x2.data_ptr())
+        tbl.set_t('SEED_DEV', seed_dev)
+        dims = _dims(M, 0, 0, D, 1, Din, dt, dt, 0)
+        ctx.drop = (float(p1), int(seed1), float(p2), int(seed2))
+        _TWINS.clear()
+        _lib.check(_lib.lib().svol_input_proj_fwd(dims, tbl.arr, *ctx.drop, ops._stream()), 'svol_input_proj_fwd')
+        ctx.pl, ctx.tbl, ctx.dims, ctx.arena, ctx.shape, ctx.n_par = pl, tbl, dims, arena, (M, D, Din, x.shape), len(params)
+        ctx.save_for_backward(x2, seed_dev)
+        return lay.view(arena, 'OUT32', torch.float32, x.shape[:-1] + (D,))
+
+    @staticmethod
+    def backward(ctx, dout32):
+        pl, tbl, dims = ctx.pl, ctx.tbl, ctx.dims
+        M, D, Din, xshape = ctx.shape
+        x2, _ = ctx.saved_tensors
+        n_par = ctx.n_par
+        if dout32 is None:
+            pl.done(n_par > 0)
+            return (None,) * (7 + n_par)
+        dt = pl.dt
+        e = _ESZ[dt]
+        dev = x2.device
+        needs = ctx.needs_input_grad
+        f32 = dt == torch.float32
+        d16 = None if f32 else _twin_take(dout32)
+        d32 = dout32.reshape(M, D)
+        d32 = d32 if d32.is_contiguous() else d32.contiguous()
+        assert d32.dtype == torch.float32
+        have = f32 or d16 is not None
+        items = ([] if have else [('DOUT', M * D * e)]) + [('DH2', M * D * e), ('DY1', M * D * e), ('DH1', M * Din * e)] + \
+            ([('DX', M * Din * e)] if needs[1] else [])
+        lay = _layout(('b', IP, M, D, Din, dt, needs[1], have), lambda: items)
+        tmp = torch.empty((lay.total,), dtype=torch.uint8, device=dev)
+        lay.fill(tbl, tmp.data_ptr())
+        if have:
+            tbl.set('DOUT', (d32 if f32 else d16).data_ptr())
+            tbl.set('DOUT32', None)
+        else:
+            tbl.set('DOUT32', d32.data_ptr())
+        if not needs[1]:
+            tbl.set('DX', None)
+        bufs = pl.grad_buffers(tbl, dev)
+        L_ = _lib.lib()
+        s = ops._stream()
+        _lib.check(L_.svol_input_proj_bwd(dims, tbl.arr, *ctx.drop, s), 'svol_input_proj_bwd')
+        if bufs is None:
+            _issue_wgrad('svol_input_proj_wgrad', dims, tbl, [ctx.arena, tmp, d32] + ([d16] if d16 is not None else []), dev)
+        else:
+            _lib.check(L_.svol_input_proj_wgrad(dims, tbl.arr, s), 'svol_input_proj_wgrad')
+        pl.done(n_par > 0)
+        dx = None
+        if needs[1]:
+            dx = ops.cast(lay.view(tmp, 'DX', dt, (M, Din)), torch.float32).view(xshape)
+        return (None, dx, None, None, None, None, None) + tuple(pl.grads_out(bufs, needs[7:], n_par > 0))
+
+
+def input_proj_fusable(seq, x, dt):
+    if len(seq) != 2 or not all(getattr(l, 'layer_norm', False) for l in seq) or not seq[0].relu or seq[1].relu:
+        return False
+    w1, w2 = seq[0].net[1].weight, seq[1].net[1].weight
+    D, Din = w2.shape[0], w1.shape[1]
+    return (x.dtype == torch.float32 and x.shape[-1] == Din and w1.shape[0] == D and w2.shape[1] == D and D % 8 == 0 and Din % 8 == 0
+            and D <= 1024 and Din <= 1024 and seq[0].net[1].bias is not None and seq[1].net[1].bias is not None)
+
+
+def input_proj(seq, x, dt, p1, seed1, p2, seed2, seed_dev=None):
+    pl = plan(seq, IP, dt, dt)
+    out = InputProjFn.apply(pl, x, p1, seed1, p2, seed2, seed_dev, *pl.inputs(x))
+    if dt != torch.float32:
+        out._svol_twin = True
+    return out
 
 
 def trace_dump() -> str:
diff --git a/svol_amd/csrc/blocks.hip b/svol_amd/csrc/blocks.hip
--- a/svol_amd/csrc/blocks.hip
+++ b/svol_amd/csrc/blocks.hip
@@ -80,6 +80,7 @@
 const char* const kVhNames = SVOL_VH_SLOTS(SLOT_NAME);
 const char* const kQsNames = SVOL_QS_SLOTS(SLOT_NAME);
 const char* const kQcNames = SVOL_QC_SLOTS(SLOT_NAME);
+const char* const kIpNames = SVOL_IP_SLOTS(SLOT_NAME);
 
 inline void record(void* ev, void* stream) {
     if (ev) (void)hipEventRecord(static_cast<hipEvent_t>(ev), static_cast<hipStream_t>(stream));
@@ -152,6 +153,7 @@
         case SVOL_BLK_VIDEO_HALF: return kVhNames;
         case SVOL_BLK_QUERY_SELF: return kQsNames;
         case SVOL_BLK_QUERY_CROSS: return kQcNames;
+        case SVOL_BLK_INPUT_PROJ: return kIpNames;
         default: return "";
     }
 }
@@ -227,11 +229,18 @@
             if (zrc) return zrc;
             record(P(EV_CLEAN_OUT), zs);
         }
-        RUN(nt(P(DQKV), 3 * D, P(W_IN_T), 3 * D, P(DXQP), D, nullptr, nullptr, M, D, 2 * D, dt, s));
-        RUN(nt(at(P(DQKV), 2 * D, dt), 3 * D, at(P(W_IN_T), 2 * D, dt), 3 * D, P(DXQ), D, nullptr, nullptr, M, D, D, dt, s));
-        RUN(svol_gate_bwd(f32(P(DS32_2)), P(DXQ), P(DXQP), f32(P(X32)), P(POS), f32(P(U)), f32(P(G1)), f32(P(A)), f32(P(MEAN1)),
-                          f32(P(RSTD1)), f32(P(GATE_WS)), f32(P(GATE_WS2)), f32(P(DX32)), f32(P(DU)), f32(P(DG1)), f32(P(DBT1)), d.B, d.L,
-                          D, d.H, dt, s));
+        if (P(DXQ)) {
+            RUN(nt(P(DQKV), 3 * D, P(W_IN_T), 3 * D, P(DXQP), D, nullptr, nullptr, M, D, 2 * D, dt, s));
+            RUN(nt(at(P(DQKV), 2 * D, dt), 3 * D, at(P(W_IN_T), 2 * D, dt), 3 * D, P(DXQ), D, nullptr, nullptr, M, D, D, dt, s));
+            RUN(svol_gate_bwd_twin(f32(P(DS32_2)), P(DXQ), P(DXQP), f32(P(X32)), P(POS), f32(P(U)), f32(P(G1)), f32(P(A)), f32(P(MEAN1)),
+                                   f32(P(RSTD1)), f32(P(GATE_WS)), f32(P(GATE_WS2)), f32(P(DX32)), P(DX16), f32(P(DU)), f32(P(DG1)),
+                                   f32(P(DBT1)), d.B, d.L, D, d.H, dt, s));
+        } else {
+            RUN(nt(P(DQKV), 3 * D, P(W_IN_T), 3 * D, P(DXQP), D, nullptr, nullptr, M, D, 3 * D, dt, s));
+            RUN(svol_gate_bwd_twin(f32(P(DS32_2)), P(DXQP), nullptr, f32(P(X32)), P(POS), f32(P(U)), f32(P(G1)), f32(P(A)), f32(P(MEAN1)),
+                                   f32(P(RSTD1)), f32(P(GATE_WS)), f32(P(GATE_WS2)), f32(P(DX32)), P(DX16), f32(P(DU)), f32(P(DG1)),
+                                   f32(P(DBT1)), d.B, d.L, D, d.H, dt, s));
+        }
     }
     return SVOL_OK;
 }
@@ -377,8 +386,12 @@
     RUN(svol_attn_bwd(P(QC), D, P(KV), 2 * D, at(P(KV), D, dt), 2 * D, P(OA), D, d_o, D, f32(P(LSE)), f32(P(DELTA)), f32(P(KBIAS)), P(DQC), D,
                       P(DKV), 2 * D, at(P(DKV), D, dt), 2 * D, d.B, d.H, d.N, d.L, dh, attn_scale(dh), attn_premul(dh, dt), P(ATTN_WS),
                       d.ws_bytes, dt, s));
-    RUN(nt(P(DKV), 2 * D, at(P(W_KV_T), D, dt), 3 * D, P(DMPOS), D, nullptr, nullptr, M, D, D, dt, s));
-    RUN(nt(at(P(DKV), D, dt), 2 * D, at(P(W_KV_T), 2 * D, dt), 3 * D, P(DMV), D, nullptr, nullptr, M, D, D, dt, s));
+    if (P(DMPOS)) {
+        RUN(nt(P(DKV), 2 * D, at(P(W_KV_T), D, dt), 3 * D, P(DMPOS), D, nullptr, nullptr, M, D, D, dt, s));
+        RUN(nt(at(P(DKV), D, dt), 2 * D, at(P(W_KV_T), 2 * D, dt), 3 * D, P(DMV), D, nullptr, nullptr, M, D, D, dt, s));
+    } else {
+        RUN(nt(P(DKV), 2 * D, at(P(W_KV_T), D, dt), 3 * D, P(DMV), D, nullptr, nullptr, M, D, 2 * D, dt, s));
+    }
     const void* dq = P(DQC);
     if (mixed) {
         RUN(svol_cast(P(DQC), dt, P(DQ), qdt, R * D, s));
@@ -410,4 +423,57 @@
 #undef P
 }
 
-}
+#define P(n) p[SVOL_IP_##n]
+int svol_input_proj_fwd(const int64_t* dims, void* const* p, float p1, uint64_t seed1, float p2, uint64_t seed2, void* s) {
+    if (!dims || !p) return SVOL_E_INVALID;
+    Trace tr_("input_proj_fwd", s);
+    const Dims d(dims);
+    if (!d.ok() || d.F <= 0 || !P(XC)) return SVOL_E_INVALID;
+    const int64_t M = d.B, D = d.D, Din = d.F;
+    const int dt = d.dt;
+    const int64_t* sd = static_cast<const int64_t*>(P(SEED_DEV));
+    if (P(X32)) RUN(svol_cast(P(X32), SVOL_F32, P(XC), dt, M * Din, s));
+    RUN(svol_layernorm_fwd(P(XC), 0, f32(P(G1)), f32(P(BT1)), nullptr, P(H1), nullptr, nullptr, 0, f32(P(MEAN1)), f32(P(RSTD1)), M, Din, p1,
+                           seed1, sd, dt, s));
+    RUN(svol_gemm_nt(P(H1), Din, nullptr, 0, P(W1), Din, P(Y1), D, f32(P(B1)), nullptr, SVOL_ACT_RELU, nullptr, 0, nullptr, 0, 0, M, D, Din,
+                     dt, s));
+    RUN(svol_layernorm_fwd(P(Y1), 0, f32(P(G2)), f32(P(BT2)), nullptr, P(H2), nullptr, nullptr, 0, f32(P(MEAN2)), f32(P(RSTD2)), M, D, p2,
+                           seed2, sd, dt, s));
+    RUN(svol_gemm_nt(P(H2), D, nullptr, 0, P(W2), D, P(OUT32), D, f32(P(B2)), nullptr, SVOL_ACT_NONE, nullptr, 0, nullptr, 0, 1, M, D, D, dt,
+                     s));
+    return SVOL_OK;
+}
+
+int svol_input_proj_bwd(const int64_t* dims, void* const* p, float p1, uint64_t seed1, float p2, uint64_t seed2, void* s) {
+    if (!dims || !p) return SVOL_E_INVALID;
+    Trace tr_("input_proj_bwd", s);
+    const Dims d(dims);
+    if (!d.ok() || d.F <= 0 || !P(XC) || !P(DOUT)) return SVOL_E_INVALID;
+    const int64_t M = d.B, D = d.D, Din = d.F;
+    const int dt = d.dt;
+    const int64_t* sd = static_cast<const int64_t*>(P(SEED_DEV));
+    if (P(DOUT32)) RUN(svol_cast(P(DOUT32), SVOL_F32, P(DOUT), dt, M * D, s));
+    RUN(nt(P(DOUT), D, P(W2_T), D, P(DH2), D, nullptr, nullptr, M, D, D, dt, s));
+    RUN(svol_layernorm_bwd_ex(nullptr, P(DH2), nullptr, P(Y1), 0, f32(P(G2)), f32(P(MEAN2)), f32(P(RSTD2)), nullptr, P(DY1), f32(P(DG2)),
+                              f32(P(DBT2)), M, D, p2, seed2, sd, SVOL_LN_RELU_MASK, dt, s));
+    RUN(nt(P(DY1), D, P(W1_T), D, P(DH1), Din, nullptr, nullptr, M, Din, D, dt, s));
+    RUN(svol_layernorm_bwd_ex(nullptr, P(DH1), nullptr, P(XC), 0, f32(P(G1)), f32(P(MEAN1)), f32(P(RSTD1)), nullptr, P(DX), f32(P(DG1)),
+                              f32(P(DBT1)), M, Din, p1, seed1, sd, P(DX) ? 0 : SVOL_LN_NO_DX, dt, s));
+    return SVOL_OK;
+}
+
+int svol_input_proj_wgrad(const int64_t* dims, void* const* p, void* s) {
+    if (!dims || !p) return SVOL_E_INVALID;
+    Trace tr_("input_proj_wgrad", s);
+    const Dims d(dims);
+    if (!d.ok() || d.F <= 0) return SVOL_E_INVALID;
+    const int64_t M = d.B, D = d.D, Din = d.F;
+    const svol_tn_problem pr[2] = {
+        {P(DOUT), D, P(H2), D, f32(P(DW2)), D, f32(P(DB2)), M, D, D},
+        {P(DY1), D, P(H1), Din, f32(P(DW1)), Din, f32(P(DB1)), M, D, Din}};
+    RUN(svol_gemm_tn_grouped(pr, 2, d.dt, s));
+    return SVOL_OK;
+}
+#undef P
+
+}
diff --git a/svol_amd/csrc/gate.hip b/svol_amd/csrc/gate.hip
--- a/svol_amd/csrc/gate.hip
+++ b/svol_amd/csrc/gate.hip
@@ -428,7 +428,8 @@
                                                              const float* __restrict__ mx, const float* __restrict__ sm,
                                                              const float* __restrict__ da, const float* __restrict__ cc,
                                                              float* __restrict__ dx, float* __restrict__ du, int L, int D,
-                                                             int H, int rpw, float* __restrict__ det_du) {
+                                                             int H, int rpw, float* __restrict__ det_du,
+                                                             T* __restrict__ dx16) {
     const int lane = threadIdx.x & 63, wave = threadIdx.x >> 6;
     const int b = blockIdx.y;
     const int l0 = (blockIdx.x * 4 + wave) * rpw;
@@ -500,6 +501,12 @@
                     dv[j].set(e, dv[j].get(e) + add);
                 }
                 dv[j].store(dx + row * D + c);
+                if (dx16) {
+                    Vec4<T> o;
+#pragma unroll
+                    for (int e = 0; e < 4; ++e) o.set(e, dv[j].get(e));
+                    o.store(dx16 + row * D + c);
+                }
             }
         }
 #pragma unroll
@@ -768,10 +775,12 @@
     return SVOL_OK;
 }
 
-int svol_gate_bwd(const float* dy32, const void* dy, const void* dy2, const float* x32, const void* pos, const float* u,
-                  const float* gamma, const float* a, const float* mean, const float* rstd, const float* ws, float* ws2,
-                  float* dx32, float* du, float* dgamma, float* dbeta, int64_t B, int64_t L, int64_t D, int64_t H, int dtype,
-                  void* stream) {
+}
+
+static int gate_bwd_impl(const float* dy32, const void* dy, const void* dy2, const float* x32, const void* pos, const float* u,
+                         const float* gamma, const float* a, const float* mean, const float* rstd, const float* ws, float* ws2,
+                         float* dx32, void* dx16, float* du, float* dgamma, float* dbeta, int64_t B, int64_t L, int64_t D, int64_t H,
+                         int dtype, void* stream) {
     if ((!dy32 && !dy && !dy2) || !x32 || !pos || !u || !gamma || !a || !mean || !rstd || !ws || !ws2 || !dx32 || !du ||
         !dgamma || !dbeta)
         return SVOL_E_INVALID;
@@ -808,9 +817,9 @@
             det_fold(det_gb, (int)g1, 2 * D, dgamma, D, s);                                                                 \
             det_fold(det_gb + D, (int)g1, 2 * D, dbeta, D, s);                                                              \
         }                                                                                                                   \
-        if (np_ == 1) hipLaunchKernelGGL((gate_bwd_apply_kernel<TT, 1>), g3, dim3(256), 0, s, x32, (const TT*)pos, u, scores, mx, sm, da, cc, dx32, du, (int)L, (int)D, (int)H, rpw3, det_du); \
-        else if (np_ == 2) hipLaunchKernelGGL((gate_bwd_apply_kernel<TT, 2>), g3, dim3(256), 0, s, x32, (const TT*)pos, u, scores, mx, sm, da, cc, dx32, du, (int)L, (int)D, (int)H, rpw3, det_du); \
-        else hipLaunchKernelGGL((gate_bwd_apply_kernel<TT, 4>), g3, dim3(256), 0, s, x32, (const TT*)pos, u, scores, mx, sm, da, cc, dx32, du, (int)L, (int)D, (int)H, rpw3, det_du); \
+        if (np_ == 1) hipLaunchKernelGGL((gate_bwd_apply_kernel<TT, 1>), g3, dim3(256), 0, s, x32, (const TT*)pos, u, scores, mx, sm, da, cc, dx32, du, (int)L, (int)D, (int)H, rpw3, det_du, (TT*)dx16); \
+        else if (np_ == 2) hipLaunchKernelGGL((gate_bwd_apply_kernel<TT, 2>), g3, dim3(256), 0, s, x32, (const TT*)pos, u, scores, mx, sm, da, cc, dx32, du, (int)L, (int)D, (int)H, rpw3, det_du, (TT*)dx16); \
+        else hipLaunchKernelGGL((gate_bwd_apply_kernel<TT, 4>), g3, dim3(256), 0, s, x32, (const TT*)pos, u, scores, mx, sm, da, cc, dx32, du, (int)L, (int)D, (int)H, rpw3, det_du, (TT*)dx16); \
     } while (0)
     if (dtype == SVOL_BF16) SVOL_GATE_BWD(bf16_t);
     else if (dtype == SVOL_F16) SVOL_GATE_BWD(f16_t);
@@ -819,6 +828,25 @@
     if (det_mode) det_fold(det_du, (int)g3.x, H * D, du, H * D, s, (int)B, (int64_t)g3.x * H * D, H * D);
     SVOL_CHECK_LAUNCH();
     return SVOL_OK;
+}
+
+extern "C" {
+
+int svol_gate_bwd(const float* dy32, const void* dy, const void* dy2, const float* x32, const void* pos, const float* u,
+                  const float* gamma, const float* a, const float* mean, const float* rstd, const float* ws, float* ws2,
+                  float* dx32, float* du, float* dgamma, float* dbeta, int64_t B, int64_t L, int64_t D, int64_t H, int dtype,
+                  void* stream) {
+    return gate_bwd_impl(dy32, dy, dy2, x32, pos, u, gamma, a, mean, rstd, ws, ws2, dx32, nullptr, du, dgamma, dbeta, B, L, D, H, dtype,
+                         stream);
+}
+
+int svol_gate_bwd_twin(const float* dy32, const void* dy, const void* dy2, const float* x32, const void* pos, const float* u,
+                       const float* gamma, const float* a, const float* mean, const float* rstd, const float* ws, float* ws2,
+                       float* dx32, void* dx16, float* du, float* dgamma, float* dbeta, int64_t B, int64_t L, int64_t D, int64_t H,
+                       int dtype, void* stream) {
+    if (dx16 && !svol_is16(dtype)) return SVOL_E_INVALID;
+    return gate_bwd_impl(dy32, dy, dy2, x32, pos, u, gamma, a, mean, rstd, ws, ws2, dx32, dx16, du, dgamma, dbeta, B, L, D, H, dtype,
+                         stream);
 }
 
 int svol_gate_vectors_fwd(const float* skch, const float* W_in, const float* b_in, float* q_out, float* u_out, int64_t B, int64_t D,
diff --git a/svol_amd/csrc/norm.hip b/svol_amd/csrc/norm.hip
--- a/svol_amd/csrc/norm.hip
+++ b/svol_amd/csrc/norm.hip
@@ -82,7 +82,7 @@
                                                      T* __restrict__ dx, float* __restrict__ dgamma,
                                                      float* __restrict__ dbeta, float* __restrict__ dxsum, int64_t M, int D,
                                                      float p, float inv_keep, uint64_t seed0, const int64_t* __restrict__ soff, int rows_per_wave,
-                                                     float* __restrict__ det_part) {
+                                                     float* __restrict__ det_part, int flags) {
     const uint64_t seed = seed0 + (soff ? ((uint64_t)soff[0] << 8) : 0ull);
     const int lane = threadIdx.x & 63;
     const int64_t wave_id = (int64_t)blockIdx.x * 4 + (threadIdx.x >> 6);
@@ -136,6 +136,7 @@
                 }
             }
         }
+        if (flags & SVOL_LN_NO_DX) { cur = nxt; continue; }
         s1 = wave_sum(s1) / (float)D;
         s2 = wave_sum(s2) / (float)D;
 #pragma unroll
@@ -146,7 +147,8 @@
                 Vec4<float> o32;
 #pragma unroll
                 for (int e = 0; e < 4; ++e) {
-                    const float r = rs * (g[j][e] - s1 - xh[j][e] * s2);
+                    float r = rs * (g[j][e] - s1 - xh[j][e] * s2);
+                    if ((flags & SVOL_LN_RELU_MASK) && !(cur.xv[j].get(e) > 0.f)) r = 0.f;
                     dxs[j][e] += r;
                     o.set(e, r);
                     o32.set(e, r);
@@ -307,12 +309,14 @@
     return SVOL_OK;
 }
 
-int svol_layernorm_bwd(const float* dy32, const void* dy, const void* dy2, const void* x, int x_f32, const float* gamma,
-                       const float* mean, const float* rstd, float* dx32, void* dx, float* dgamma, float* dbeta,
-                       float* dx_colsum, int64_t M, int64_t D, float dropout_p, uint64_t seed, const int64_t* seed_offset_dev,
-                       int dtype, void* stream) {
-    if ((!dy32 && !dy && !dy2) || !x || !gamma || !mean || !rstd || (!dx && !dx32) || !dgamma || !dbeta || M < 0 || D <= 0)
-        return SVOL_E_INVALID;
+}
+
+static int layernorm_bwd_impl(const float* dy32, const void* dy, const void* dy2, const void* x, int x_f32, const float* gamma,
+                              const float* mean, const float* rstd, float* dx32, void* dx, float* dgamma, float* dbeta,
+                              float* dx_colsum, int64_t M, int64_t D, float dropout_p, uint64_t seed, const int64_t* seed_offset_dev,
+                              int dtype, int flags, void* stream) {
+    if ((!dy32 && !dy && !dy2) || !x || !gamma || !mean || !rstd || !dgamma || !dbeta || M < 0 || D <= 0) return SVOL_E_INVALID;
+    if (((flags & SVOL_LN_NO_DX) != 0) != (!dx && !dx32)) return SVOL_E_INVALID;
     if (D % 4 || D > LN_MAX_PASSES * 256) return SVOL_E_UNSUPPORTED;
     if (dropout_p < 0.f || dropout_p >= 1.f) return SVOL_E_INVALID;
     if (!svol_is16(dtype) && dtype != SVOL_F32) return SVOL_E_INVALID;
@@ -329,7 +333,7 @@
 #define SVOL_LNB(TT, TXX, NPP)                                                                                                      \
     hipLaunchKernelGGL((ln_bwd_kernel<TT, TXX, NPP>), dim3(grid), dim3(256), 0, s, dy32, (const TT*)dy, (const TT*)dy2, (const TXX*)x, \
                        gamma, mean, rstd, dx32, (TT*)dx, dgamma, dbeta, dx_colsum, M, (int)D, dropout_p, inv_keep, seed,              \
-                       seed_offset_dev, (int)rpw, det.p)
+                       seed_offset_dev, (int)rpw, det.p, flags)
 #define SVOL_LNB_NP(TT, TXX)                  \
     do {                                      \
         if (D <= 256) SVOL_LNB(TT, TXX, 1);   \
@@ -352,6 +356,25 @@
     return SVOL_OK;
 }
 
+extern "C" {
+
+int svol_layernorm_bwd(const float* dy32, const void* dy, const void* dy2, const void* x, int x_f32, const float* gamma,
+                       const float* mean, const float* rstd, float* dx32, void* dx, float* dgamma, float* dbeta,
+                       float* dx_colsum, int64_t M, int64_t D, float dropout_p, uint64_t seed, const int64_t* seed_offset_dev,
+                       int dtype, void* stream) {
+    return layernorm_bwd_impl(dy32, dy, dy2, x, x_f32, gamma, mean, rstd, dx32, dx, dgamma, dbeta, dx_colsum, M, D, dropout_p, seed,
+                              seed_offset_dev, dtype, 0, stream);
+}
+
+int svol_layernorm_bwd_ex(const float* dy32, const void* dy, const void* dy2, const void* x, int x_f32, const float* gamma,
+                          const float* mean, const float* rstd, float* dx32, void* dx, float* dgamma, float* dbeta, int64_t M, int64_t D,
+                          float dropout_p, uint64_t seed, const int64_t* seed_offset_dev, int flags, int dtype, void* stream) {
+    if (flags & ~(SVOL_LN_RELU_MASK | SVOL_LN_NO_DX)) return SVOL_E_INVALID;
+    if ((flags & SVOL_LN_RELU_MASK) && (flags & SVOL_LN_NO_DX)) return SVOL_E_INVALID;
+    return layernorm_bwd_impl(dy32, dy, dy2, x, x_f32, gamma, mean, rstd, dx32, dx, dgamma, dbeta, nullptr, M, D, dropout_p, seed,
+                              seed_offset_dev, dtype, flags, stream);
+}
+
 int svol_dropout(const void* x, void* y, int64_t n, int64_t row_len, float p, uint64_t seed, int dtype, void* stream) {
     if (!x || !y || n < 0 || row_len <= 0 || row_len > 0xffffffffll || !(p >= 0.f && p < 1.f)) return SVOL_E_INVALID;
     if (n == 0) return SVOL_OK;
diff --git a/svol_amd/modeling/cross_modal_transformer.py b/svol_amd/modeling/cross_modal_transformer.py
--- a/svol_amd/modeling/cross_modal_transformer.py
+++ b/svol_amd/modeling/cross_modal_transformer.py
@@ -163,10 +163,10 @@
         m32, m, mpos = self.video_half(mem32, skch32, pos, u)
         return m32, self.query_half(out, m, mpos, qpos, kbias)
 
-    def video_half(self, mem32, skch32, pos, u=None, u_next=None, sc_in=None):
+    def video_half(self, mem32, skch32, pos, u=None, u_next=None, sc_in=None, want_m32=True):
         if blocks.ENABLED:
             uu = self.gate_vectors(skch32) if u is None else u
-            m32, m, mpos, sc = blocks.video_half(self, mem32, pos, uu, pos.dtype, u_next, sc_in)
+            m32, m, mpos, sc = blocks.video_half(self, mem32, pos, uu, pos.dtype, u_next, sc_in, want_m32)
             return (m32, m, mpos) if u_next is None else (m32, m, mpos, sc)
         assert sc_in is None
         h = self.nhead
@@ -241,15 +241,16 @@
         with torch.cuda.stream(side):
             out = initial_queries()
         sc = None
+        last = len(self.layers) - 1
         for li, (layer, u) in enumerate(zip(self.layers, us)):
             with torch.cuda.stream(side):
                 out_sa = layer.query_self(out, qpos, vid_pos.dtype)
             if blocks.ENABLED and blocks.GATE_SCORES_FUSE and li + 1 < len(us):
                 m32, m, mpos, sc = layer.video_half(mem32, src_skch32, vid_pos, u, us[li + 1], sc)
             elif sc is not None:
-                m32, m, mpos = layer.video_half(mem32, src_skch32, vid_pos, u, None, sc)
+                m32, m, mpos = layer.video_half(mem32, src_skch32, vid_pos, u, None, sc, li < last)
             else:
-                m32, m, mpos = layer.video_half(mem32, src_skch32, vid_pos, u)
+                m32, m, mpos = layer.video_half(mem32, src_skch32, vid_pos, u, None, None, li < last)
             side.wait_stream(main)
             m.record_stream(side)
             mpos.record_stream(side)
diff --git a/svol_amd/modeling/svanet.py b/svol_amd/modeling/svanet.py
--- a/svol_amd/modeling/svanet.py
+++ b/svol_amd/modeling/svanet.py
@@ -5,7 +5,7 @@
 import torch
 from torch import nn
 
-from .. import ops
+from .. import blocks, ops
 from . import cross_modal_transformer as cmt
 from .cross_modal_transformer import build_cross_modal_transformer
 from .position_encoding import build_position_encoding
@@ -93,6 +93,14 @@
                       seed_dev=self.step_dev)
         return x
 
+    def _proj32(self, seq, x32, salt):
+        dt = self.compute_dtype
+        if blocks.ENABLED and blocks.input_proj_fusable(seq, x32, dt):
+            seed = (self.base_seed << 32) + (self._step << 8) + salt * 16
+            p = [layer.p if layer.training else 0.0 for layer in seq]
+            return blocks.input_proj(seq, x32, dt, p[0], seed, p[1], seed + 1, self.step_dev)
+        return self._proj(seq, ops.cast_ag(x32, dt), salt)
+
     def forward(self, src_sketch, src_sketch_mask, src_video, src_video_mask):
         if not src_video.is_cuda:
             raise RuntimeError('svol_amd.SVANet runs on the MI355X HIP kernels only; move the module and its '
@@ -107,7 +115,7 @@
         def mask_side(with_us):
             mask_f = src_video_mask.to(torch.float32)
             pos_video = self.video_position_embed(mask_f, d, dt)
-            skch = self._proj(self.input_sketch_proj, ops.cast_ag(src_sketch.float(), dt), 1)
+            skch = self._proj32(self.input_sketch_proj, src_sketch.float(), 1)
             skch = skch.reshape(skch.shape[0], -1)
             kbias = torch.zeros_like(mask_f).masked_fill_(mask_f == 0, float('-inf'))
             us = cmt.all_gate_vectors(list(self.transformer.layers), skch) if with_us else None
@@ -120,16 +128,17 @@
             with torch.cuda.stream(side):
                 ops.weights.new_epoch()
                 casts_done = side.record_event()
-            xv = ops.cast_ag(src_video.float(), dt)
+            fused = blocks.ENABLED and blocks.input_proj_fusable(self.input_video_proj, src_video.float(), dt)
+            xv = None if fused else ops.cast_ag(src_video.float(), dt)
             with torch.cuda.stream(side):
                 pos_video, skch, kbias, us = mask_side(True)
             main.wait_event(casts_done)
-            vid = self._proj(self.input_video_proj, xv, 0)
+            vid = self._proj32(self.input_video_proj, src_video.float(), 0) if fused else self._proj(self.input_video_proj, xv, 0)
             main.wait_stream(side)
             for t in [pos_video, skch, kbias] + list(us or []):
                 t.record_stream(main)
         else:
-            vid = self._proj(self.input_video_proj, ops.cast_ag(src_video.float(), dt), 0)
+            vid = self._proj32(self.input_video_proj, src_video.float(), 0)
             pos_video, skch, kbias, us = mask_side(False)
         hs = (self.transformer(vid, skch, kbias, pos_video, self.query_embed.weight, us) if us is not None else
               self.transformer(vid, skch, kbias, pos_video, self.query_embed.weight))
```

Result: no change. 15270, median of 6 (+0.9%).
